# spyglass-search/memex

Hardware: AMD Instinct MI355X
Metric: queries/sec, exact cosine top-10 (recall@10 = 1.0) on 10M x 384-d f32 (higher is better)
Workload: dtype f32 corpus; int8 MFMA filter (exact integer sums, measured-residual certificate) -> f32 rescoring -> f64 DistCosine on the survivors (results bit-identical to all-f64)

## Files before the change

memex_amd/csrc/index.hip:

```cpp
#include <dlfcn.h>
#include <sys/stat.h>
#include <unistd.h>

#include <algorithm>
#include <atomic>
#include <cmath>
#include <condition_variable>
#include <cstdlib>
#include <chrono>
#include <ctime>
#include <cstring>
#include <deque>
#include <map>
#include <memory>
#include <mutex>
#include <string>
#include <thread>
#include <vector>

#include "index_kernels.h"
#include "mx_common.h"
#include "mx_debug.h"
#include "mx_filter_bits.h"
#include "shard_pool.h"

namespace mx {

std::string &last_error_slot() {
    static thread_local std::string slot;
    return slot;
}

namespace {

constexpr int kFlagWords = 4 * kMaxBatch;
constexpr int kAutoI8MaxDim = 1024;
constexpr int kSumWords = 5;

struct Scratch {
    void *qfrag = nullptr;
    float *qpad = nullptr;
    double *qnorm2 = nullptr;
    float *theta = nullptr, *theta_retry = nullptr;
    uint32_t *todo = nullptr;
    uint32_t *dev_flags = nullptr;
    uint32_t *host_flags = nullptr;
    uint32_t *host_sum = nullptr;
    bool out_on_host = false;
    uint32_t *done_ctr = nullptr;
    uint32_t flag_seq = 0;
    uint32_t *overflow = nullptr, *cand_cnt = nullptr, *qflags = nullptr;
    float *e1 = nullptr;
    float *lane_rec = nullptr;
    uint32_t *lane_tile = nullptr;
    uint32_t *lane_cnt = nullptr;
    float *lane_max = nullptr;
    float *qstage = nullptr;
    float *qscale = nullptr;
    float *qa = nullptr, *qb = nullptr;
    float *qmean = nullptr;
    uint64_t *out_ids = nullptr;
    float *out_scores = nullptr;
    float *out_dists = nullptr;
    int32_t *out_nfound = nullptr;
    int kcap = 0;
    void *exact_scratch = nullptr;
    size_t exact_bytes = 0;
    float *max_err = nullptr;
    float *h_q = nullptr;
    uint64_t *h_ids = nullptr;
    float *h_scores = nullptr, *h_dists = nullptr;
    int32_t *h_nf = nullptr;
    uint32_t *rlim = nullptr;
    uint64_t *out_nrange = nullptr;
    uint64_t *h_nr = nullptr;
    bool ready = false;
};

struct LaneBufs {
    float *rec = nullptr;
    uint32_t *tile = nullptr, *cnt = nullptr;
    float *max = nullptr;
    int nwg = 0;
    int groups = 1;
};
constexpr int kMaxDevices = 64;
struct LanePool {
    std::mutex mu;
    std::vector<LaneBufs> idle;
    int open_indexes = 0;
};
LanePool g_lanes[kMaxDevices];

void lane_free(LaneBufs &b) {
    if (b.rec) (void)hipFree(b.rec);
    if (b.tile) (void)hipFree(b.tile);
    if (b.cnt) (void)hipFree(b.cnt);
    if (b.max) (void)hipFree(b.max);
    b = LaneBufs{};
}

struct Rccl {
    void *lib = nullptr;
    int (*CommInitAll)(void **, int, const int *) = nullptr;
    int (*CommDestroy)(void *) = nullptr;
    int (*AllGather)(const void *, void *, size_t, int, void *, hipStream_t) = nullptr;
    int (*GroupStart)() = nullptr;
    int (*GroupEnd)() = nullptr;
    const char *(*GetErrorString)(int) = nullptr;
    bool ok = false;
};

}
}

using namespace mx;

struct mx_filter;

struct SearchReq {
    const float *q;
    int B, k;
    uint64_t *ids;
    float *scores, *dists;
    int32_t *n_found;
    const std::vector<std::pair<uint64_t, uint64_t>> *filt = nullptr;
    mx_filter *res = nullptr;
    const uint32_t *dlim = nullptr;
    uint64_t *n_in_range = nullptr;
    int rc = MX_OK;
    std::string err;
    bool done = false;
};

struct mx_index {
    std::string key;
    int dim = 0, ds = 0, kc = 0, device = 0;
    int refs = 1;
    std::mutex mu;
    std::mutex cmu;
    std::condition_variable ccv;
    std::deque<SearchReq *> pending;
    bool leader = false;
    hipStream_t stream = nullptr;
    float *x = nullptr;
    float *scale = nullptr;
    void *xh = nullptr;
    bool want_filter = true;
    bool filter_i8 = false;
    bool filter_auto = true;
    bool pooled = false;
    uint32_t i8_batches = 0, i8_retry_batches = 0;
    uint64_t plain_bf16_rows = 0;
    uint64_t demoted_at_rows = 0;
    float *tsc = nullptr;
    float *amean = nullptr;
    float *mean = nullptr;
    float *msum = nullptr;
    bool centred = false;
    bool compressed = false;
    bool raw_ingest = false;
    float *xs = nullptr, *ss = nullptr;
    uint64_t xs_rows = 0;
    uint64_t n = 0, cap = 0;
    IdMap idmap{0, 0, 1, 0};
    uint32_t *flags = nullptr;
    uint64_t wild_rows = 0;
    uint32_t *zero_rows = nullptr;
    uint64_t n_zero = 0;
    uint32_t *wild_list = nullptr;
    uint64_t n_wild = 0;
    int mode = MX_SEARCH_AUTO;
    bool profiling = false;
    int n_cu = 0, nwg = 0;
    bool scan8_pair = true;
    Scratch s;
    mx_index_stats stats{};
    hipEvent_t ev0 = nullptr, ev1 = nullptr, ev_wait = nullptr;
    double wait_ema_us[4] = {0.0, 0.0, 0.0, 0.0};
    uint64_t *dead = nullptr;
    std::vector<uint64_t> dead_h;
    uint64_t n_dead = 0;
    std::vector<uint64_t> dead_log;
    uint64_t disk_dead = 0;
    uint64_t gen = 0;
    bool failed = false;
    uint64_t *filt = nullptr;
    size_t filt_words = 0;
    uint64_t *filt_ranges = nullptr;
    size_t filt_ranges_cap = 0;
    uint32_t *subset_rows = nullptr;
    bool last_subset = false;
    uint64_t row_epoch = 0;
    uint64_t dead_ver = 0;
    uint32_t *mmr_rows = nullptr;
    float *mmr_stage = nullptr;
    size_t mmr_stage_bytes = 0;
    uint64_t *mmr_ids = nullptr, *mmr_h_ids = nullptr;
    float *mmr_scores = nullptr, *mmr_dists = nullptr;
    int32_t *mmr_nf = nullptr, *mmr_h_nf = nullptr;
    uint32_t *mmr_pos = nullptr;
    int mmr_fcap = 0;
    uint32_t *byid_rows = nullptr;
    float *byid_stage = nullptr;
    float *byid_q = nullptr;
    uint64_t *byid_ids = nullptr, *byid_nr = nullptr, *byid_own = nullptr;
    float *byid_scores = nullptr, *byid_dists = nullptr;
    int32_t *byid_nf = nullptr;
    uint32_t *byid_src = nullptr, *byid_dlim = nullptr;
    int byid_cap = 0;
    std::string disk_dir;
    uint64_t disk_rows = 0;
    off_t disk_size = 0;
    struct timespec disk_mtime {};
    std::vector<mx_index *> shards;
    uint64_t block_rows = 0;
    uint64_t total = 0;
    bool use_rccl = false;
    std::vector<void *> comms;
    std::vector<void *> sh_block;
    std::vector<void *> sh_gather;
    std::vector<float *> sh_q, sh_scores;
    std::vector<int32_t *> sh_nf;
    int sh_kcap = 0;
    std::unique_ptr<ShardPool> pool;
    bool composite() const { return !shards.empty(); }
};

struct FilterShard {
    int device = 0;
    uint64_t *bits = nullptr;
    size_t words = 0;
    std::vector<uint64_t> bits_h;
    uint64_t *stage = nullptr;
    size_t stage_words = 0;
    uint32_t *list = nullptr;
    bool cached = false, list_ok = false;
    uint64_t cached_dead = 0;
    uint64_t n_allowed = 0, n_live = 0;
    uint64_t row_lo = 0, row_hi = 0;
};
struct mx_filter {
    mx_index *idx = nullptr;
    uint64_t epoch = 0;
    std::vector<FilterShard> sh;
};

namespace {

std::mutex g_reg_mu;
std::map<std::string, mx_index *> g_registry;
std::once_flag g_scan_once;
hipError_t g_scan_setup_err = hipSuccess;
std::mutex g_rccl_mu;
Rccl g_rccl;
std::atomic<bool> g_rccl_broken{false};

bool load_rccl() {
    std::lock_guard<std::mutex> lk(g_rccl_mu);
    if (g_rccl.lib) return g_rccl.ok;
    for (const char *name : {"librccl.so.1", "librccl.so", "/opt/rocm/lib/librccl.so.1"}) {
        g_rccl.lib = dlopen(name, RTLD_NOW | RTLD_GLOBAL);
        if (g_rccl.lib) break;
    }
    if (!g_rccl.lib) return false;
    auto sym = [&](const char *n) { return dlsym(g_rccl.lib, n); };
    g_rccl.CommInitAll = reinterpret_cast<int (*)(void **, int, const int *)>(sym("ncclCommInitAll"));
    g_rccl.CommDestroy = reinterpret_cast<int (*)(void *)>(sym("ncclCommDestroy"));
    g_rccl.AllGather = reinterpret_cast<int (*)(const void *, void *, size_t, int, void *, hipStream_t)>(sym("ncclAllGather"));
    g_rccl.GroupStart = reinterpret_cast<int (*)()>(sym("ncclGroupStart"));
    g_rccl.GroupEnd = reinterpret_cast<int (*)()>(sym("ncclGroupEnd"));
    g_rccl.GetErrorString = reinterpret_cast<const char *(*)(int)>(sym("ncclGetErrorString"));
    g_rccl.ok = g_rccl.CommInitAll && g_rccl.CommDestroy && g_rccl.AllGather && g_rccl.GroupStart && g_rccl.GroupEnd;
    return g_rccl.ok;
}

void free_composite_buffers(mx_index *idx) {
    for (size_t g = 0; g < idx->shards.size(); ++g) {
        DeviceGuard dg(idx->shards[g]->device);
        auto F = [](void *p) {
            if (p) (void)hipFree(p);
        };
        if (g < idx->sh_block.size()) F(idx->sh_block[g]);
        if (g < idx->sh_gather.size()) F(idx->sh_gather[g]);
        if (g < idx->sh_q.size()) F(idx->sh_q[g]);
        if (g < idx->sh_scores.size()) F(idx->sh_scores[g]);
        if (g < idx->sh_nf.size()) F(idx->sh_nf[g]);
    }
    idx->sh_block.clear(); idx->sh_gather.clear(); idx->sh_q.clear(); idx->sh_scores.clear(); idx->sh_nf.clear();
    idx->sh_kcap = 0;
}

int free_index(mx_index *idx) {
    {
        std::lock_guard<std::mutex> lk(idx->mu);
    }
    if (idx->composite()) {
        idx->pool.reset();
        for (mx_index *sh : idx->shards) {
            DeviceGuard dg(sh->device);
            if (sh->stream) (void)hipStreamSynchronize(sh->stream);
        }
        free_composite_buffers(idx);
        for (void *c : idx->comms)
            if (c && g_rccl.ok) (void)g_rccl.CommDestroy(c);
        for (mx_index *sh : idx->shards) free_index(sh);
        idx->shards.clear();
    }
    DeviceGuard g(idx->device);
    if (idx->stream) (void)hipStreamSynchronize(idx->stream);
    auto F = [](void *p) {
        if (p) (void)hipFree(p);
    };
    F(idx->x); F(idx->scale); F(idx->xh); F(idx->tsc); F(idx->flags); F(idx->xs); F(idx->ss); F(idx->zero_rows); F(idx->wild_list);
    F(idx->amean); F(idx->mean); F(idx->msum); F(idx->dead); F(idx->filt); F(idx->filt_ranges); F(idx->subset_rows);
    F(idx->mmr_rows); F(idx->mmr_stage); F(idx->mmr_ids); F(idx->mmr_scores); F(idx->mmr_dists); F(idx->mmr_nf); F(idx->mmr_pos);
    if (idx->mmr_h_ids) (void)hipHostFree(idx->mmr_h_ids);
    if (idx->mmr_h_nf) (void)hipHostFree(idx->mmr_h_nf);
    F(idx->byid_rows); F(idx->byid_stage); F(idx->byid_q); F(idx->byid_ids); F(idx->byid_nr); F(idx->byid_own); F(idx->byid_scores);
    F(idx->byid_dists); F(idx->byid_nf); F(idx->byid_src); F(idx->byid_dlim);
    Scratch &s = idx->s;
    F(s.qfrag); F(s.qpad); F(s.qnorm2); F(s.theta); F(s.theta_retry); F(s.todo); F(s.dev_flags); F(s.done_ctr);
    if (s.host_flags) (void)hipHostFree(s.host_flags);
    if (s.host_sum) (void)hipHostFree(s.host_sum);
    for (void *hp : {(void *)s.h_q, (void *)s.h_ids, (void *)s.h_scores, (void *)s.h_dists, (void *)s.h_nf, (void *)s.h_nr})
        if (hp) (void)hipHostFree(hp);
    F(s.rlim); F(s.out_nrange);
    F(s.qstage); F(s.qscale); F(s.qa); F(s.qb); F(s.qmean); F(s.out_ids); F(s.out_scores); F(s.out_dists); F(s.out_nfound);
    F(s.exact_scratch); F(s.max_err);
    if (idx->ev0) (void)hipEventDestroy(idx->ev0);
    if (idx->ev1) (void)hipEventDestroy(idx->ev1);
    if (idx->ev_wait) (void)hipEventDestroy(idx->ev_wait);
    if (idx->stream) (void)hipStreamDestroy(idx->stream);
    if (idx->pooled && idx->device >= 0 && idx->device < kMaxDevices) {
        LanePool &lp = g_lanes[idx->device];
        std::lock_guard<std::mutex> lk(lp.mu);
        if (--lp.open_indexes <= 0) {
            lp.open_indexes = 0;
            for (LaneBufs &b : lp.idle) lane_free(b);
            lp.idle.clear();
        }
    }
    delete idx;
    return MX_OK;
}

struct LaneLease {
    mx_index *idx = nullptr;
    LaneBufs b;
    int take(mx_index *i, int groups) {
        if (i->device < 0 || i->device >= kMaxDevices) return fail(MX_EDEVICE, "device %d out of range", i->device);
        idx = i;
        LanePool &lp = g_lanes[i->device];
        {
            std::lock_guard<std::mutex> lk(lp.mu);
            for (size_t j = 0; j < lp.idle.size(); ++j)
                if (lp.idle[j].nwg == i->nwg && lp.idle[j].groups == groups) {
                    b = lp.idle[j];
                    lp.idle.erase(lp.idle.begin() + (long)j);
                    break;
                }
        }
        if (!b.rec) {
            b.nwg = i->nwg;
            b.groups = groups;
            const size_t lanes = (size_t)i->nwg * kScanThreads * (size_t)groups;
            hipError_t e = hipMalloc(reinterpret_cast<void **>(&b.rec), lanes * kRecCap * 16 * sizeof(float));
            if (e == hipSuccess) e = hipMalloc(reinterpret_cast<void **>(&b.tile), lanes * kRecCap * sizeof(uint32_t));
            if (e == hipSuccess) e = hipMalloc(reinterpret_cast<void **>(&b.cnt), lanes * sizeof(uint32_t));
            if (e == hipSuccess) e = hipMalloc(reinterpret_cast<void **>(&b.max), lanes * sizeof(float));
            if (e != hipSuccess) {
                lane_free(b);
                idx = nullptr;
                return fail(MX_ENOMEM, "hipMalloc(lane buffers): %s", hipGetErrorString(e));
            }
        }
        Scratch &s = i->s;
        s.lane_rec = b.rec;
        s.lane_tile = b.tile;
        s.lane_cnt = b.cnt;
        s.lane_max = b.max;
        return MX_OK;
    }
    void drop() {
        if (!idx) return;
        Scratch &s = idx->s;
        s.lane_rec = nullptr;
        s.lane_tile = nullptr;
        s.lane_cnt = nullptr;
        s.lane_max = nullptr;
        LanePool &lp = g_lanes[idx->device];
        std::lock_guard<std::mutex> lk(lp.mu);
        if (lp.open_indexes > 0) lp.idle.push_back(b);
        else lane_free(b);
        idx = nullptr;
        b = LaneBufs{};
    }
    ~LaneLease() { drop(); }
};

int ensure_scratch(mx_index *idx) {
    Scratch &s = idx->s;
    if (s.ready) return MX_OK;
    const size_t ds = (size_t)idx->ds;
    MX_HIP(hipMalloc(&s.qfrag, (size_t)kMaxBatch * ds * 2));
    MX_HIP(hipMalloc(&s.qpad, (size_t)kMaxBatch * ds * 4));
    MX_HIP(hipMalloc(&s.qnorm2, kMaxBatch * sizeof(double)));
    MX_HIP(hipMalloc(&s.theta, kMaxBatch * sizeof(float)));
    MX_HIP(hipMalloc(&s.theta_retry, kMaxBatch * sizeof(float)));
    MX_HIP(hipMalloc(&s.todo, kMaxBatch * sizeof(uint32_t)));
    MX_HIP(hipMalloc(&s.dev_flags, kFlagWords * sizeof(uint32_t)));
    MX_HIP(hipMemsetAsync(s.dev_flags, 0, kFlagWords * sizeof(uint32_t), idx->stream));
    s.overflow = s.dev_flags;
    s.cand_cnt = s.dev_flags + kMaxBatch;
    s.e1 = reinterpret_cast<float *>(s.dev_flags + 2 * kMaxBatch);
    s.qflags = s.dev_flags + 3 * kMaxBatch;
    MX_HIP(hipHostMalloc(reinterpret_cast<void **>(&s.host_flags), kFlagWords * sizeof(uint32_t), hipHostMallocDefault));
    MX_HIP(hipHostMalloc(reinterpret_cast<void **>(&s.host_sum), kSumWords * sizeof(uint32_t), hipHostMallocMapped | hipHostMallocCoherent));
    memset(s.host_sum, 0, kSumWords * sizeof(uint32_t));
    MX_HIP(hipMalloc(&s.done_ctr, sizeof(uint32_t)));
    MX_HIP(hipMemsetAsync(s.done_ctr, 0, sizeof(uint32_t), idx->stream));
    MX_HIP(hipMalloc(&s.qstage, (size_t)kMaxBatch * idx->dim * sizeof(float)));
    MX_HIP(hipMalloc(&s.qscale, kMaxBatch * sizeof(float)));
    MX_HIP(hipMalloc(&s.qa, kMaxBatch * sizeof(float)));
    MX_HIP(hipMalloc(&s.qb, kMaxBatch * sizeof(float)));
    MX_HIP(hipMalloc(&s.qmean, kMaxBatch * sizeof(float)));
    MX_HIP(hipMemsetAsync(s.qmean, 0, kMaxBatch * sizeof(float), idx->stream));
    MX_HIP(hipHostMalloc(reinterpret_cast<void **>(&s.h_q), (size_t)kMaxBatch * idx->dim * sizeof(float), hipHostMallocMapped | hipHostMallocCoherent));
    MX_HIP(hipHostMalloc(reinterpret_cast<void **>(&s.h_nf), kMaxBatch * sizeof(int32_t), hipHostMallocMapped | hipHostMallocCoherent));
    MX_HIP(hipMalloc(&s.max_err, sizeof(float)));
    MX_HIP(hipMalloc(&s.rlim, kMaxBatch * sizeof(uint32_t)));
    MX_HIP(hipMalloc(&s.out_nrange, kMaxBatch * sizeof(uint64_t)));
    MX_HIP(hipHostMalloc(reinterpret_cast<void **>(&s.h_nr), kMaxBatch * sizeof(uint64_t), hipHostMallocMapped | hipHostMallocCoherent));
    MX_HIP(hipMemsetAsync(s.max_err, 0, sizeof(float), idx->stream));
    s.ready = true;
    return MX_OK;
}

int ensure_out(mx_index *idx, int k) {
    Scratch &s = idx->s;
    if (k <= s.kcap) return MX_OK;
    auto F = [](void *p) {
        if (p) (void)hipFree(p);
    };
    F(s.out_ids); F(s.out_scores); F(s.out_dists); F(s.out_nfound);
    s.out_ids = nullptr; s.out_scores = nullptr; s.out_dists = nullptr; s.out_nfound = nullptr;
    for (void *hp : {(void *)s.h_ids, (void *)s.h_scores, (void *)s.h_dists})
        if (hp) (void)hipHostFree(hp);
    s.h_ids = nullptr; s.h_scores = nullptr; s.h_dists = nullptr;
    s.kcap = 0;
    const int kc = std::max(k, 16);
    MX_HIP(hipMalloc(&s.out_ids, (size_t)kMaxBatch * kc * sizeof(uint64_t)));
    MX_HIP(hipMalloc(&s.out_scores, (size_t)kMaxBatch * kc * sizeof(float)));
    MX_HIP(hipMalloc(&s.out_dists, (size_t)kMaxBatch * kc * sizeof(float)));
    MX_HIP(hipMalloc(&s.out_nfound, kMaxBatch * sizeof(int32_t)));
    MX_HIP(hipHostMalloc(reinterpret_cast<void **>(&s.h_ids), (size_t)kMaxBatch * kc * sizeof(uint64_t), hipHostMallocMapped | hipHostMallocCoherent));
    MX_HIP(hipHostMalloc(reinterpret_cast<void **>(&s.h_scores), (size_t)kMaxBatch * kc * sizeof(float), hipHostMallocMapped | hipHostMallocCoherent));
    MX_HIP(hipHostMalloc(reinterpret_cast<void **>(&s.h_dists), (size_t)kMaxBatch * kc * sizeof(float), hipHostMallocMapped | hipHostMallocCoherent));
    s.kcap = kc;
    return MX_OK;
}

int ensure_exact(mx_index *idx, int k, int *gcap) {
    Scratch &s = idx->s;
    for (int g = *gcap;; g /= 2) {
        const size_t need = exact_group_scratch_bytes(idx->n, k, g);
        if (s.exact_bytes >= need) {
            *gcap = g;
            return MX_OK;
        }
        if (s.exact_scratch) {
            MX_HIP(hipStreamSynchronize(idx->stream));
            (void)hipFree(s.exact_scratch);
        }
        s.exact_scratch = nullptr;
        s.exact_bytes = 0;
        const size_t want = need + need / 4;
        if (hipMalloc(&s.exact_scratch, want) == hipSuccess) {
            s.exact_bytes = want;
        } else {
            (void)hipGetLastError();
            if (hipMalloc(&s.exact_scratch, need) == hipSuccess) s.exact_bytes = need;
            else (void)hipGetLastError();
        }
        if (s.exact_bytes >= need) {
            *gcap = g;
            return MX_OK;
        }
        if (g <= 4) return fail(MX_ENOMEM, "hipMalloc(EXACT-path scratch, %zu bytes) failed", need);
    }
}

struct DevBuf {
    void *p = nullptr;
    ~DevBuf() {
        if (p) (void)hipFree(p);
    }
    void *release() {
        void *r = p;
        p = nullptr;
        return r;
    }
};

int grow_dead(mx_index *idx, uint64_t cap) {
    if (!idx->dead) return MX_OK;
    const size_t words = (size_t)(cap / kTile8Rows), have = idx->dead_h.size();
    if (words <= have) return MX_OK;
    DevBuf nd;
    MX_HIP(hipMalloc(&nd.p, words * sizeof(uint64_t)));
    MX_HIP(hipMemcpyAsync(nd.p, idx->dead, have * sizeof(uint64_t), hipMemcpyDeviceToDevice, idx->stream));
    MX_HIP(hipMemsetAsync(static_cast<uint64_t *>(nd.p) + have, 0, (words - have) * sizeof(uint64_t), idx->stream));
    MX_HIP(hipStreamSynchronize(idx->stream));
    (void)hipFree(idx->dead);
    idx->dead = static_cast<uint64_t *>(nd.release());
    idx->dead_h.resize(words, 0);
    return MX_OK;
}

int ensure_capacity(mx_index *idx, uint64_t rows) {
    if (rows <= idx->cap) return MX_OK;
    uint64_t want = std::max<uint64_t>(rows, idx->cap + idx->cap / 2);
    want = round_up(std::max<uint64_t>(want, 1024), kTile8Rows);
    if (int rc = grow_dead(idx, want); rc != MX_OK) return rc;
    if (idx->compressed) {
        DevBuf nh2;
        const size_t hb = (size_t)want * idx->ds * 2;
        MX_HIP(hipMalloc(&nh2.p, hb));
        const size_t used = idx->xh ? (size_t)round_up(idx->n, kTileRows) * idx->ds * 2 : 0;
        if (used) MX_HIP(hipMemcpyAsync(nh2.p, idx->xh, used, hipMemcpyDeviceToDevice, idx->stream));
        MX_HIP(hipMemsetAsync(static_cast<char *>(nh2.p) + used, 0, hb - used, idx->stream));
        MX_HIP(hipStreamSynchronize(idx->stream));
        if (idx->xh) (void)hipFree(idx->xh);
        idx->xh = nh2.release();
        idx->cap = want;
        return MX_OK;
    }
    DevBuf nx, nsc, nh, nts, nam;
    const size_t rowb = (size_t)idx->ds * sizeof(float);
    MX_HIP(hipMalloc(&nx.p, want * rowb));
    MX_HIP(hipMalloc(&nsc.p, want * sizeof(float)));
    float *fx = static_cast<float *>(nx.p), *fsc = static_cast<float *>(nsc.p);
    if (idx->n) {
        MX_HIP(hipMemcpyAsync(fx, idx->x, idx->n * rowb, hipMemcpyDeviceToDevice, idx->stream));
        MX_HIP(hipMemcpyAsync(fsc, idx->scale, idx->n * sizeof(float), hipMemcpyDeviceToDevice, idx->stream));
    }
    MX_HIP(hipMemsetAsync(fx + idx->n * (size_t)idx->ds, 0, (want - idx->n) * rowb, idx->stream));
    MX_HIP(hipMemsetAsync(fsc + idx->n, 0, (want - idx->n) * sizeof(float), idx->stream));
    if (idx->want_filter && idx->kc <= kMaxKC16) {
        const size_t eb = idx->filter_i8 ? 1 : 2;
        const size_t hb = (size_t)want * idx->ds * eb, tb = (size_t)(want / kTile8Rows) * kTscaleFloats * sizeof(float);
        if (hipMalloc(&nh.p, hb) != hipSuccess || (idx->filter_i8 && hipMalloc(&nts.p, tb) != hipSuccess)) {
            (void)hipGetLastError();
            if (nh.p) (void)hipFree(nh.release());
            nh.p = nullptr;
        } else {
            const uint64_t used_rows = idx->xh ? round_up(idx->n, kTile8Rows) : 0;
            const size_t used = (size_t)used_rows * idx->ds * eb;
            if (used) MX_HIP(hipMemcpyAsync(nh.p, idx->xh, used, hipMemcpyDeviceToDevice, idx->stream));
            MX_HIP(hipMemsetAsync(static_cast<char *>(nh.p) + used, 0, hb - used, idx->stream));
            if (idx->filter_i8) {
                const size_t tused = (size_t)(used_rows / kTile8Rows) * kTscaleFloats * sizeof(float);
                if (tused) MX_HIP(hipMemcpyAsync(nts.p, idx->tsc, tused, hipMemcpyDeviceToDevice, idx->stream));
                MX_HIP(hipMemsetAsync(static_cast<char *>(nts.p) + tused, 0, tb - tused, idx->stream));
                if (idx->centred && idx->xh && idx->amean) {
                    if (hipMalloc(&nam.p, want * sizeof(float)) == hipSuccess) {
                        const size_t aused = (size_t)used_rows * sizeof(float);
                        MX_HIP(hipMemcpyAsync(nam.p, idx->amean, std::min(aused, (size_t)idx->cap * sizeof(float)), hipMemcpyDeviceToDevice, idx->stream));
                        if (want * sizeof(float) > aused) MX_HIP(hipMemsetAsync(static_cast<char *>(nam.p) + aused, 0, want * sizeof(float) - aused, idx->stream));
                    } else {
                        (void)hipGetLastError();
                        if (idx->n) {
// ... 297 lines not shown
int build_filter_mask(mx_index *idx, const Ranges &r, std::vector<uint64_t> &flat) {
    const size_t words = (size_t)(idx->cap / kTile8Rows);
    if (int rc = ensure_mask_words(idx, words); rc != MX_OK) return rc;
    if (idx->filt_ranges_cap < std::max<size_t>(r.size(), 1)) {
        if (idx->filt_ranges) (void)hipFree(idx->filt_ranges);
        idx->filt_ranges = nullptr;
        idx->filt_ranges_cap = 0;
        const size_t want = std::max<size_t>(r.size() + r.size() / 2, 64);
        MX_HIP(hipMalloc(reinterpret_cast<void **>(&idx->filt_ranges), want * 2 * sizeof(uint64_t)));
        idx->filt_ranges_cap = want;
    }
    flat.resize(2 * r.size());
    for (size_t i = 0; i < r.size(); ++i) {
        flat[2 * i] = r[i].first;
        flat[2 * i + 1] = r[i].second;
    }
    if (!flat.empty())
        MX_HIP(hipMemcpyAsync(idx->filt_ranges, flat.data(), flat.size() * sizeof(uint64_t), hipMemcpyHostToDevice, idx->stream));
    MX_HIP(launch_filter_mask(idx->stream, idx->n_dead ? idx->dead : nullptr, idx->filt_ranges, (uint32_t)r.size(), words, idx->filt));
    return MX_OK;
}

bool subset_pays(const mx_index *idx, int B, uint64_t m, uint64_t span_rows, int bytes_per_elem) {
    if (m > (uint64_t)kSubsetCap || idx->ds > kMaxKC16 * kChunkFloats) return false;
    const int force = debug_flag("filt_subset", -1);
    if (force == 0 || force == 1) return force == 1;
    const double w = (double)idx->ds / 384.0;
    const double subset_us = (double)((B + kPassBatch - 1) / kPassBatch) * (43.0 + 0.053 * w * (double)m);
    const double masked_us = 75.0 + (double)span_rows * w * bytes_per_elem * (B <= 128 ? 0.065e-3 : 0.10e-3);
    return subset_us <= masked_us;
}

struct FilterArg {
    const Ranges *ranges = nullptr;
    mx_filter *res = nullptr;
    int shard = 0;
};

void refresh_filter_shard(const mx_index *t, FilterShard &fs) {
    if (fs.cached && fs.cached_dead == t->dead_ver) return;
    fs.n_allowed = fs.n_live = 0;
    fs.row_lo = fs.row_hi = 0;
    const bool dead = t->n_dead != 0;
    for (size_t w = 0; w < fs.bits_h.size(); ++w) {
        const uint64_t b = fs.bits_h[w];
        if (!b) continue;
        if (!fs.n_allowed) fs.row_lo = (uint64_t)w * 64 + (uint64_t)__builtin_ctzll(b);
        fs.row_hi = (uint64_t)w * 64 + 64 - (uint64_t)__builtin_clzll(b);
        fs.n_allowed += (uint64_t)__builtin_popcountll(b);
        fs.n_live += (uint64_t)__builtin_popcountll(dead && w < t->dead_h.size() ? b & ~t->dead_h[w] : b);
    }
    fs.cached = true;
    fs.cached_dead = t->dead_ver;
    fs.list_ok = false;
}

int ensure_mask_words(mx_index *idx, size_t words) {
    if (idx->filt_words >= words) return MX_OK;
    if (idx->filt) (void)hipFree(idx->filt);
    idx->filt = nullptr;
    idx->filt_words = 0;
    MX_HIP(hipMalloc(reinterpret_cast<void **>(&idx->filt), words * sizeof(uint64_t)));
    idx->filt_words = words;
    return MX_OK;
}

int apply_filter_mask(mx_index *idx, const FilterShard &fs) {
    const size_t words = (size_t)(idx->cap / kTile8Rows);
    if (int rc = ensure_mask_words(idx, words); rc != MX_OK) return rc;
    MX_HIP(launch_filter_apply(idx->stream, idx->n_dead ? idx->dead : nullptr, fs.bits, std::min(fs.words, words), words, idx->filt));
    return MX_OK;
}

int await_finish(mx_index *idx, int B, uint32_t seq) {
    Scratch &s = idx->s;
    static const bool no_spin = [] {
        const char *sp = getenv("MEMEX_HIP_SPIN");
        return !(sp && sp[0] == '1');
    }();
    const auto t0 = std::chrono::steady_clock::now();
    double &ema = idx->wait_ema_us[B <= 32 ? 0 : B <= 128 ? 1 : B <= 256 ? 2 : 3];
    bool overslept = false;
    if (no_spin && ema > 150.0) {
        const double nap_us = 0.8 * ema - 60.0;
        if (nap_us > 50.0) {
            struct timespec ts;
            ts.tv_sec = (time_t)(nap_us / 1e6);
            ts.tv_nsec = (long)((nap_us - (double)ts.tv_sec * 1e6) * 1e3);
            (void)clock_nanosleep(CLOCK_MONOTONIC, 0, &ts, nullptr);
            overslept = __atomic_load_n(&s.host_sum[4], __ATOMIC_ACQUIRE) == seq;
        }
    }
    bool done = false;
    for (unsigned spins = 1;; ++spins) {
        if (__atomic_load_n(&s.host_sum[4], __ATOMIC_ACQUIRE) == seq) {
            done = true;
            break;
        }
        if ((spins & 0xfff) == 0 && std::chrono::steady_clock::now() - t0 > std::chrono::seconds(2)) break;
        __builtin_ia32_pause();
    }
    if (done) {
        const double us = std::chrono::duration<double, std::micro>(std::chrono::steady_clock::now() - t0).count();
        ema = overslept ? 0.5 * ema : ema > 0.0 ? 0.75 * ema + 0.25 * us : us;
        return MX_OK;
    }
    MX_HIP(hipStreamSynchronize(idx->stream));
    if (__atomic_load_n(&s.host_sum[4], __ATOMIC_ACQUIRE) == seq) return MX_OK;
    return fail(MX_EDEVICE, "finish_kernel did not signal completion");
}

enum class BatchKind { kTopK, kRange };
struct BatchPlan {
    bool filt8;
    bool wide;
    bool fast;
    bool centred8;
    bool centred;
    bool x2;
    bool pair;
    int nwg;
    int lanes;
    Scan8Geom geom;
    int split;
    uint64_t trows;
    int bytes_per_elem;
};

BatchPlan plan_batch(const mx_index *idx, int B, int k_or_cap, BatchKind kind, bool trivial) {
    BatchPlan pl;
    pl.filt8 = idx->xh != nullptr && idx->filter_i8 && !idx->compressed;
    pl.wide = idx->kc > kMaxKC && !pl.filt8;
    pl.fast = !trivial && idx->mode == MX_SEARCH_AUTO && (idx->kc > kMaxKC ? idx->xh != nullptr && idx->kc <= kMaxKC16 : true) &&
              (!idx->compressed || idx->wild_rows == 0) && (kind == BatchKind::kRange || k_or_cap <= 256) &&
              idx->n_zero <= (uint64_t)kZeroCap && idx->n_wild <= (uint64_t)kWildCap;
    pl.centred8 = idx->centred && pl.filt8 && idx->amean && idx->mean && idx->kc <= kMaxKC;
    const bool two_groups = pl.fast && pl.filt8 && !pl.centred8 && idx->kc <= kMaxKC8x2;
    pl.x2 = two_groups && B > kPassBatch;
    pl.pair = two_groups && B > kPassBatch / 2 && B <= kPassBatch && idx->scan8_pair;
    pl.centred = pl.centred8 || (idx->centred && idx->xh && !pl.filt8 && !pl.wide && !idx->compressed && idx->amean && idx->mean && idx->kc <= kMaxKC);
    pl.nwg = pl.pair ? 2 * idx->nwg : idx->nwg;
    pl.lanes = pl.x2 || pl.pair ? 2 : 1;
    pl.geom = pl.pair ? Scan8Geom::kPair : pl.x2 ? Scan8Geom::k512 : Scan8Geom::k256;
    pl.split = B > kPassBatch && !pl.x2 && !(pl.fast && pl.wide) ? kPassBatch : pl.fast && pl.wide && B > kWideBatch ? kWideBatch : 0;
    pl.trows = pl.filt8 ? kTile8Rows : kTileRows;
    pl.bytes_per_elem = pl.filt8 ? 1 : idx->xh ? 2 : 4;
    return pl;
}

int prep_queries(mx_index *idx, const BatchPlan &pl, const float *d_q, int B) {
    Scratch &s = idx->s;
    MX_HIP(launch_prep_queries(idx->stream, d_q, B, idx->dim, idx->ds, s.qfrag, s.qpad, s.qnorm2, s.theta, s.e1,
                               idx->xh ? idx->flags + 2 : nullptr, s.overflow, s.qflags, s.qa, s.qb, pl.filt8, s.qscale,
                               pl.centred ? idx->mean : nullptr, s.qmean, pl.centred8 ? idx->flags + 5 : nullptr));
    return MX_OK;
}

void fill_scan_params(ScanParams &p, const mx_index *idx, const BatchPlan &pl, int B, const uint64_t *mask) {
    const Scratch &s = idx->s;
    p.x = idx->x;
    p.xh = idx->xh;
    p.scale = idx->scale;
    p.qfrag = s.qfrag;
    p.theta = s.theta;
    p.n_rows = idx->n;
    p.ds = (uint32_t)idx->ds;
    p.wave_mask = (1u << ((B + 31) / 32)) - 1u;
    p.lane_rec = s.lane_rec;
    p.lane_tile = s.lane_tile;
    p.lane_cnt = s.lane_cnt;
    p.lane_max = s.lane_max;
    p.overflow = s.overflow;
    p.tscale = idx->tsc;
    p.qscale = s.qscale;
    p.qa = s.qa;
    p.qb = s.qb;
    p.amean = pl.centred ? idx->amean : nullptr;
    p.qmean = s.qmean;
    p.dead = mask;
}

hipError_t launch_scan_for(const mx_index *idx, const BatchPlan &pl, bool collect, const ScanParams &p) {
    if (pl.filt8) return launch_scan8(idx->stream, idx->kc, collect, pl.nwg, p, pl.geom);
    if (pl.wide) return launch_scan16w(idx->stream, idx->kc, collect, pl.nwg, p);
    return idx->xh ? launch_scan16(idx->stream, idx->kc, collect, pl.nwg, p) : launch_scan(idx->stream, idx->kc, collect, pl.nwg, p);
}

void fill_finish_params(FinishParams &fp, const mx_index *idx, const BatchPlan &pl, int B, int k, const uint64_t *mask, uint64_t n_live,
                        uint64_t *d_ids, float *d_scores, float *d_dists, int32_t *d_nfound) {
    const Scratch &s = idx->s;
    fp.k = k;
    fp.ds = idx->ds;
    fp.nwg = pl.nwg;
    fp.x = idx->compressed ? nullptr : idx->x;
    fp.xh = idx->xh;
    fp.scale = idx->scale;
    fp.n_rows = idx->n;
    fp.idmap = idx->idmap;
    fp.qpad = s.qpad;
    fp.qnorm2 = s.qnorm2;
    fp.e1 = s.e1;
    fp.qa = s.qa;
    fp.qb = s.qb;
    fp.terr = pl.filt8 ? idx->tsc : nullptr;
    fp.e2 = (float)(idx->ds + 8) * 5.9604645e-8f + 1e-6f;
    fp.lane_rec = s.lane_rec;
    fp.lane_tile = s.lane_tile;
    fp.lane_cnt = s.lane_cnt;
    fp.theta = s.theta;
    fp.zero_rows = idx->zero_rows;
    fp.n_zero = (uint32_t)std::min<uint64_t>(idx->n_zero, kZeroCap);
    fp.wild_rows = idx->wild_list;
    fp.n_wild = (uint32_t)std::min<uint64_t>(idx->n_wild, kWildCap);
    fp.dead = mask;
    fp.n_live = n_live;
    fp.overflow = s.overflow;
    fp.todo = nullptr;
    fp.theta_retry = s.theta_retry;
    fp.cand_cnt = s.cand_cnt;
    fp.ids = d_ids;
    fp.scores = d_scores;
    fp.dists = d_dists;
    fp.n_found = d_nfound;
    fp.max_err = nullptr;
    fp.done_ctr = s.done_ctr;
    fp.dev_flags = s.dev_flags;
    fp.host_flags = s.host_sum;
    fp.n_queries = B;
    fp.host_out = s.out_on_host ? 1 : 0;
}

int fetch_flags(mx_index *idx) {
    MX_HIP(hipMemcpyAsync(idx->s.host_flags, idx->s.dev_flags, kFlagWords * sizeof(uint32_t), hipMemcpyDeviceToHost, idx->stream));
    MX_HIP(hipStreamSynchronize(idx->stream));
    return MX_OK;
}

void drop_large_exact_scratch(mx_index *idx) {
    if (idx->mode != MX_SEARCH_AUTO || idx->s.exact_bytes <= kExactKeepBytes) return;
    (void)hipFree(idx->s.exact_scratch);
    idx->s.exact_scratch = nullptr;
    idx->s.exact_bytes = 0;
}

int search_batch(mx_index *idx, const float *d_q, int B, int k, uint64_t *d_ids, float *d_scores, float *d_dists,
                 int32_t *d_nfound, const FilterArg *filt = nullptr) {
    int rc = ensure_scratch(idx);
    if (rc != MX_OK) return rc;
    Scratch &s = idx->s;
    hipStream_t st = idx->stream;
    Ranges fr;
    uint64_t n_allow = 0, span_lo = 0, span_hi = 0;
    FilterShard *res = filt && filt->res ? &filt->res->sh[(size_t)filt->shard] : nullptr;
    if (res) {
        refresh_filter_shard(idx, *res);
        n_allow = res->n_live;
        span_lo = res->row_lo;
        span_hi = res->row_hi;
    } else if (filt) {
        for (const auto &x : *filt->ranges)
            if (x.first < std::min(x.second, idx->n)) fr.emplace_back(x.first, std::min(x.second, idx->n));
        n_allow = count_allowed(idx, fr);
        if (!fr.empty()) {
            span_lo = fr.front().first;
            span_hi = fr.back().second;
        }
    }
    idx->last_subset = false;
    const bool trivial = idx->n == 0 || k == 0 || (filt && n_allow == 0);
    if (idx->compressed && idx->kc > kMaxKC16 && !trivial)
        return fail(MX_EUNSUPPORTED, "a compressed corpus supports dim <= %d", kMaxKC16 * kChunkFloats);
    const BatchPlan pl = plan_batch(idx, B, k, BatchKind::kTopK, trivial);
    if (pl.split) {
        rc = search_batch(idx, d_q, pl.split, k, d_ids, d_scores, d_dists, d_nfound, filt);
        if (rc != MX_OK) return rc;
        const size_t o = (size_t)pl.split * k;
        return search_batch(idx, d_q + (size_t)pl.split * idx->dim, B - pl.split, k, d_ids + o, d_scores + o,
                            d_dists ? d_dists + o : nullptr, d_nfound + pl.split, filt);
    }
    const uint32_t *h_ovf = s.host_flags, *h_qfl = s.host_flags + 3 * kMaxBatch;
    auto any_bad_query = [&] {
        uint32_t bad = 0;
        for (int b = 0; b < B; ++b) bad |= h_qfl[b];
        return bad != 0;
    };
    if (filt && !trivial && subset_pays(idx, B, n_allow, span_hi - span_lo, pl.bytes_per_elem)) {
        std::vector<uint32_t> list;
        const uint32_t *rows_list = nullptr;
        if (res) {
            if (!res->list) MX_HIP(hipMalloc(reinterpret_cast<void **>(&res->list), (size_t)kSubsetCap * sizeof(uint32_t)));
            if (!res->list_ok) {
                MX_HIP(hipMemsetAsync(res->list, 0, (size_t)kSubsetCap * sizeof(uint32_t), st));
                MX_HIP(launch_filter_list(st, idx->n_dead ? idx->dead : nullptr, res->bits, span_lo >> 6, (span_hi + 63) >> 6, res->list,
                                          (uint32_t)kSubsetCap));
                res->list_ok = true;
            }
            rows_list = res->list;
        } else {
            list.reserve((size_t)n_allow);
            for (const auto &x : fr)
                for (uint64_t r = x.first; r < x.second; ++r)
                    if (!idx->n_dead || !((idx->dead_h[r >> 6] >> (r & 63)) & 1ull)) list.push_back((uint32_t)r);
            if (!idx->subset_rows) MX_HIP(hipMalloc(reinterpret_cast<void **>(&idx->subset_rows), (size_t)kSubsetCap * sizeof(uint32_t)));
            MX_HIP(hipMemcpyAsync(idx->subset_rows, list.data(), list.size() * sizeof(uint32_t), hipMemcpyHostToDevice, st));
            rows_list = idx->subset_rows;
        }
        if ((rc = prep_queries(idx, pl, d_q, B)) != MX_OK) return rc;
        MX_HIP(launch_subset_topk(st, B, k, idx->ds, idx->compressed ? nullptr : idx->x, idx->xh, rows_list, (uint32_t)n_allow,
                                  idx->idmap, s.qpad, s.qnorm2, d_ids, d_scores, d_dists, d_nfound));
        if ((rc = fetch_flags(idx)) != MX_OK) return rc;
        if (any_bad_query()) return fail(MX_EINVAL, "a query contains non-finite values");
        idx->last_subset = true;
        idx->stats.searches += 1;
        idx->stats.queries += (uint64_t)B;
        idx->stats.filtered_queries += (uint64_t)B;
        idx->stats.subset_queries += (uint64_t)B;
        return MX_OK;
    }
    std::vector<uint64_t> flat_ranges;
    if (filt && !trivial && (rc = res ? apply_filter_mask(idx, *res) : build_filter_mask(idx, fr, flat_ranges)) != MX_OK) return rc;
    const uint64_t *mask = filt ? idx->filt : idx->n_dead ? idx->dead : nullptr;
    const uint64_t n_live = filt ? n_allow : idx->n - idx->n_dead;
    LaneLease lease;
    if ((rc = lease.take(idx, pl.lanes)) != MX_OK) return rc;
    if ((rc = prep_queries(idx, pl, d_q, B)) != MX_OK) return rc;
    bool timed = false;

    FinishParams fp;
    fill_finish_params(fp, idx, pl, B, k, mask, n_live, d_ids, d_scores, d_dists, d_nfound);
    if (trivial) fp.n_rows = fp.n_live = 0;
    fp.max_err = idx->profiling ? s.max_err : nullptr;
    auto finish_and_wait = [&]() -> int {
        fp.seq = ++s.flag_seq;
        MX_HIP(launch_finish(st, B, fp));
        return await_finish(idx, B, fp.seq);
    };
    std::vector<int> exact;
    if (trivial) {
        fp.seq = ++s.flag_seq;
        MX_HIP(launch_finish(st, B, fp));
    } else if (pl.fast) {
        const uint64_t tiles = (idx->n + pl.trows - 1) / pl.trows, full = idx->n / pl.trows;
        const uint64_t ts0 = filt ? span_lo / pl.trows : 0, ts1 = filt ? (span_hi + pl.trows - 1) / pl.trows : tiles;
        const uint64_t full1 = std::min(ts1, full);
        ScanParams p;
        fill_scan_params(p, idx, pl, B, mask);
        auto collect = [&](bool first) -> int {
            p.tile_begin = (uint32_t)ts0;
            p.tile_end = (uint32_t)ts1;
            p.tile_stride = 1;
            if (first && idx->profiling) MX_HIP(hipEventRecord(idx->ev0, st));
            MX_HIP(launch_scan_for(idx, pl, true, p));
            if (first && idx->profiling) {
                MX_HIP(hipEventRecord(idx->ev1, st));
                timed = true;
            }
            if (first) {
                idx->stats.scan_launches += 1;
                idx->stats.scan_bytes += (ts1 - ts0) * pl.trows * idx->ds * (uint64_t)pl.bytes_per_elem;
            }
            return MX_OK;
        };
        if (ts1 - ts0 > 2ull * idx->nwg) {
            p.tile_begin = (uint32_t)ts0;
            p.tile_end = (uint32_t)full1;
            p.tile_stride = sample_stride(full1 - ts0, pl.nwg, k, pl.filt8, idx->ds, pl.centred8);
            MX_HIP(launch_scan_for(idx, pl, false, p));
            MX_HIP(launch_theta(st, B, k, pl.nwg, s.lane_max, s.qa, !pl.filt8, s.theta));
        }
        if ((rc = collect(true)) != MX_OK) return rc;
        if ((rc = finish_and_wait()) != MX_OK) return rc;
        if (timed) {
            float ms = 0.f;
            MX_HIP(hipEventElapsedTime(&ms, idx->ev0, idx->ev1));
            idx->stats.scan_ms += ms;
            timed = false;
        }
        if (s.host_sum[2]) return fail(MX_EINVAL, "a query contains non-finite values");
        idx->stats.candidates += s.host_sum[1];
        if (s.host_sum[0]) {
            if ((rc = fetch_flags(idx)) != MX_OK) return rc;
            int retry = 0;
            for (int b = 0; b < B; ++b) {
                if (h_ovf[b] == 1) ++retry;
                else if (h_ovf[b] >= 2) exact.push_back(b);
            }
            if (pl.filt8 && !filt) idx->i8_retry_batches += 1;
            const bool habitual = pl.filt8 && idx->i8_batches >= 8 && idx->i8_retry_batches * 4 > idx->i8_batches;
            if (pl.filt8 && !filt && idx->filter_auto && ((size_t)(retry + (int)exact.size()) * 16 > (size_t)std::max(B, 16) || habitual)) {
                if (!idx->centred && idx->kc <= kMaxKC && idx->n >= 256) {
                    const std::string keep = last_error_slot();
                    if (build_filter_copy(idx, true) == MX_OK && idx->centred) {
                        lease.drop();
                        return search_batch(idx, d_q, B, k, d_ids, d_scores, d_dists, d_nfound);
                    }
                    last_error_slot() = keep;
                }
                const int drc = demote_filter(idx);
                if (drc == MX_OK) {
                    idx->stats.filter_demotions += 1;
                    lease.drop();
                    return search_batch(idx, d_q, B, k, d_ids, d_scores, d_dists, d_nfound);
                }
                if (drc != MX_ENOMEM) return drc;
            }
            if (retry) {
                idx->stats.retry_queries += (uint64_t)retry;
                p.wave_mask = 0;
                for (int b = 0; b < B; ++b)
                    if (h_ovf[b] == 1) p.wave_mask |= 1u << (b >> 5);
                MX_HIP(launch_retry_setup(st, s.theta, s.theta_retry, s.overflow, s.todo));
                if ((rc = collect(false)) != MX_OK) return rc;
                fp.todo = s.todo;
                if ((rc = finish_and_wait()) != MX_OK) return rc;
                exact.clear();
                if (s.host_sum[0]) {
                    if ((rc = fetch_flags(idx)) != MX_OK) return rc;
                    for (int b = 0; b < B; ++b)
                        if (h_ovf[b] != 0) exact.push_back(b);
                }
            }
        }
        idx->stats.fallback_queries += exact.size();
    } else {
        if ((rc = fetch_flags(idx)) != MX_OK) return rc;
        if (any_bad_query()) return fail(MX_EINVAL, "a query contains non-finite values");
        for (int b = 0; b < B; ++b) exact.push_back(b);
    }
    if (!exact.empty() || trivial || !pl.fast) {
        rc = run_exact(idx, exact, k, d_ids, d_scores, d_dists, d_nfound, mask, n_live);
        if (rc != MX_OK) return rc;
        MX_HIP(hipStreamSynchronize(st));
        drop_large_exact_scratch(idx);
    }
    idx->stats.searches += 1;
    idx->stats.queries += (uint64_t)B;
    if (filt) idx->stats.filtered_queries += (uint64_t)B;
    if (pl.filt8 && pl.fast && !filt) idx->i8_batches += 1;
    return MX_OK;
}

float host_score_from_dist(float d) {
    const volatile float t = 1.0f / d;
    const volatile float u = 1.0f / t;
    return 1.0f - u;
}

uint32_t range_dist_limit(float t) {
    if (!(t <= 1.0f)) return 0;
    uint32_t lo = 0, hi = 0x40800000u;
    if (host_score_from_dist(4.0f) >= t) return hi + 1;
    while (hi - lo > 1) {
        const uint32_t mid = lo + (hi - lo) / 2;
        float d;
        memcpy(&d, &mid, sizeof d);
        if (host_score_from_dist(d) >= t) lo = mid;
        else hi = mid;
    }
    return lo + 1;
}

constexpr float kRangeEps = 9.5367431640625e-7f;

int run_exact_range(mx_index *idx, const std::vector<int> &qs, int cap, uint64_t *d_ids, float *d_scores, float *d_dists,
                    int32_t *d_nfound, uint64_t *d_nrange, const uint64_t *mask, uint64_t n_live) {
    if (qs.empty()) return MX_OK;
    int gcap = qs.size() <= 4 ? 4 : qs.size() <= 8 ? 8 : qs.size() <= 16 ? 16 : kExactGroup;
    int rc = ensure_exact(idx, cap, &gcap);
    if (rc != MX_OK) return rc;
    Scratch &s = idx->s;
    for (size_t g0 = 0; g0 < qs.size(); g0 += (size_t)gcap) {
        ExactGroup grp{};
        grp.n = (int)std::min<size_t>((size_t)gcap, qs.size() - g0);
        for (int j = 0; j < grp.n; ++j) grp.q[j] = qs[g0 + j];
        MX_HIP(launch_exact_range_group(idx->stream, cap, idx->ds, idx->compressed ? nullptr : idx->x, idx->xh, idx->n, idx->idmap, s.qpad,
                                        s.qnorm2, grp, s.exact_scratch, s.rlim, d_ids, d_scores, d_dists, d_nfound, d_nrange, mask, n_live));
    }
    return MX_OK;
}

int range_batch(mx_index *idx, const float *d_q, int B, int cap, const uint32_t *dlim, uint64_t *d_ids, float *d_scores, float *d_dists,
                int32_t *d_nfound, uint64_t *d_nrange) {
    int rc = ensure_scratch(idx);
    if (rc != MX_OK) return rc;
    Scratch &s = idx->s;
    hipStream_t st = idx->stream;
    const uint64_t n_live = idx->n - idx->n_dead;
    const bool trivial = idx->n == 0 || n_live == 0;
    if (idx->compressed && idx->kc > kMaxKC16 && !trivial)
        return fail(MX_EUNSUPPORTED, "a compressed corpus supports dim <= %d", kMaxKC16 * kChunkFloats);
    const BatchPlan pl = plan_batch(idx, B, cap, BatchKind::kRange, trivial);
    if (pl.split) {
        rc = range_batch(idx, d_q, pl.split, cap, dlim, d_ids, d_scores, d_dists, d_nfound, d_nrange);
        if (rc != MX_OK) return rc;
        const size_t o = (size_t)pl.split * cap;
        return range_batch(idx, d_q + (size_t)pl.split * idx->dim, B - pl.split, cap, dlim + pl.split, d_ids + o, d_scores + o,
                           d_dists ? d_dists + o : nullptr, d_nfound + pl.split, d_nrange + pl.split);
    }
    const uint32_t *h_ovf = s.host_flags, *h_qfl = s.host_flags + 3 * kMaxBatch;
    const uint64_t *mask = idx->n_dead ? idx->dead : nullptr;
    LaneLease lease;
    if (pl.fast && (rc = lease.take(idx, pl.lanes)) != MX_OK) return rc;
    MX_HIP(hipMemcpyAsync(s.rlim, dlim, (size_t)B * sizeof(uint32_t), hipMemcpyHostToDevice, st));
    if ((rc = prep_queries(idx, pl, d_q, B)) != MX_OK) return rc;
    std::vector<int> exact;
    if (pl.fast) {
        MX_HIP(launch_range_theta(st, B, s.rlim, kRangeEps, s.qa, s.theta));
        const uint64_t tiles = (idx->n + pl.trows - 1) / pl.trows;
        ScanParams p;
        fill_scan_params(p, idx, pl, B, mask);
        p.tile_begin = 0;
        p.tile_end = (uint32_t)tiles;
        p.tile_stride = 1;
        MX_HIP(launch_scan_for(idx, pl, true, p));
        idx->stats.scan_launches += 1;
        idx->stats.scan_bytes += tiles * pl.trows * idx->ds * (uint64_t)pl.bytes_per_elem;

        RangeParams rp;
        FinishParams &fp = rp.f;
        fill_finish_params(fp, idx, pl, B, cap, mask, n_live, d_ids, d_scores, d_dists, d_nfound);
        fp.seq = ++s.flag_seq;
        rp.dlim = s.rlim;
        rp.eps = kRangeEps;
        rp.n_in_range = d_nrange;
        MX_HIP(launch_range_finish(st, B, rp));
        if ((rc = await_finish(idx, B, fp.seq)) != MX_OK) return rc;
        if (s.host_sum[2]) return fail(MX_EINVAL, "a query contains non-finite values");
        idx->stats.candidates += s.host_sum[1];
        if (s.host_sum[0]) {
            if ((rc = fetch_flags(idx)) != MX_OK) return rc;
            for (int b = 0; b < B; ++b)
                if (h_ovf[b] != 0) exact.push_back(b);
        }
        idx->stats.fallback_queries += exact.size();
    } else {
        if ((rc = fetch_flags(idx)) != MX_OK) return rc;
        for (int b = 0; b < B; ++b)
            if (h_qfl[b]) return fail(MX_EINVAL, "a query contains non-finite values");
        for (int b = 0; b < B && !trivial; ++b) exact.push_back(b);
        if (trivial) {
            MX_HIP(hipMemsetAsync(s.rlim, 0, (size_t)B * sizeof(uint32_t), st));
            RangeParams rp{};
            rp.f.k = cap;
            rp.f.ds = idx->ds;
            rp.f.x = idx->x;
            rp.f.ids = d_ids;
            rp.f.scores = d_scores;
            rp.f.dists = d_dists;
            rp.f.n_found = d_nfound;
            rp.f.cand_cnt = s.cand_cnt;
            rp.dlim = s.rlim;
            rp.n_in_range = d_nrange;
            MX_HIP(launch_range_finish(st, B, rp));
        }
    }
    if (!exact.empty() || trivial) {
        rc = run_exact_range(idx, exact, cap, d_ids, d_scores, d_dists, d_nfound, d_nrange, mask, n_live);
        if (rc != MX_OK) return rc;
        MX_HIP(hipStreamSynchronize(st));
        drop_large_exact_scratch(idx);
    }
    idx->stats.searches += 1;
    idx->stats.queries += (uint64_t)B;
    return MX_OK;
}

void sync_shard_streams(mx_index *idx) {
    for (mx_index *sh : idx->shards) {
        DeviceGuard dg(sh->device);
        if (sh->stream) (void)hipStreamSynchronize(sh->stream);
    }
}

bool sync_shard_streams_within(mx_index *idx, double seconds) {
    const auto t_end = std::chrono::steady_clock::now() + std::chrono::duration<double>(seconds);
    for (mx_index *sh : idx->shards) {
        DeviceGuard dg(sh->device);
        if (!sh->stream) continue;
        for (;;) {
            const hipError_t e = hipStreamQuery(sh->stream);
            if (e == hipSuccess) break;
            if (e != hipErrorNotReady) {
                (void)hipGetLastError();
                return false;
            }
            if (std::chrono::steady_clock::now() > t_end) return false;
            std::this_thread::sleep_for(std::chrono::microseconds(200));
        }
    }
    return true;
}

int ensure_composite_buffers(mx_index *idx, int k) {
    if (k <= idx->sh_kcap) return MX_OK;
    sync_shard_streams(idx);
    free_composite_buffers(idx);
    const int kc = std::max(k, 16);
    const size_t G = idx->shards.size();
    const size_t blk = (size_t)kMaxBatch * kc * 12 + kMaxBatch * sizeof(uint64_t);
    idx->sh_block.assign(G, nullptr); idx->sh_gather.assign(G, nullptr); idx->sh_q.assign(G, nullptr);
    idx->sh_scores.assign(G, nullptr); idx->sh_nf.assign(G, nullptr);
    for (size_t g = 0; g < G; ++g) {
        DeviceGuard dg(idx->shards[g]->device);
        MX_HIP(hipMalloc(&idx->sh_block[g], blk));
        if (g == 0 || idx->use_rccl) MX_HIP(hipMalloc(&idx->sh_gather[g], blk * G));
        MX_HIP(hipMalloc(reinterpret_cast<void **>(&idx->sh_q[g]), (size_t)kMaxBatch * idx->dim * sizeof(float)));
        MX_HIP(hipMalloc(reinterpret_cast<void **>(&idx->sh_scores[g]), (size_t)kMaxBatch * kc * sizeof(float)));
        MX_HIP(hipMalloc(reinterpret_cast<void **>(&idx->sh_nf[g]), kMaxBatch * sizeof(int32_t)));
    }
    idx->sh_kcap = kc;
    return MX_OK;
}

uint64_t shard_rows(uint64_t total, uint64_t R, uint64_t G, uint64_t g) {
    const uint64_t full_blocks = total / R, tail = total % R;
    uint64_t rows = (full_blocks / G) * R + (g < full_blocks % G ? R : 0);
    if (full_blocks % G == g) rows += tail;
    return rows;
}

void enable_peer_access(mx_index *idx) {
    for (size_t g = 1; g < idx->shards.size(); ++g) {
        if (idx->shards[g]->device == idx->shards[0]->device) continue;
        int can = 0;
        (void)hipDeviceCanAccessPeer(&can, idx->shards[0]->device, idx->shards[g]->device);
        if (can) {
            DeviceGuard dg(idx->shards[0]->device);
            (void)hipDeviceEnablePeerAccess(idx->shards[g]->device, 0);
            (void)hipGetLastError();
            DeviceGuard d2(idx->shards[g]->device);
            (void)hipDeviceEnablePeerAccess(idx->shards[0]->device, 0);
            (void)hipGetLastError();
        }
    }
}

bool rccl_selftest(mx_index *idx, double seconds) {
    const int G = (int)idx->shards.size();
    std::vector<hipStream_t> st(G, nullptr);
    std::vector<unsigned char *> snd(G, nullptr), rcv(G, nullptr);
    bool ok = true;
    for (int g = 0; g < G && ok; ++g) {
        DeviceGuard dg(idx->shards[g]->device);
        ok = hipStreamCreateWithFlags(&st[g], hipStreamNonBlocking) == hipSuccess && hipMalloc(&snd[g], 64) == hipSuccess &&
             hipMalloc(&rcv[g], 64 * (size_t)G) == hipSuccess && hipMemsetAsync(snd[g], g + 1, 64, st[g]) == hipSuccess &&
             hipMemsetAsync(rcv[g], 0, 64 * (size_t)G, st[g]) == hipSuccess;
    }
    bool hung = false;
    if (ok) {
        int e = g_rccl.GroupStart();
        for (int g = 0; g < G && e == 0; ++g) e = g_rccl.AllGather(snd[g], rcv[g], 64, 1 , idx->comms[g], st[g]);
        const int e2 = g_rccl.GroupEnd();
        ok = e == 0 && e2 == 0;
        const auto t0 = std::chrono::steady_clock::now();
        for (int g = 0; g < G && ok && !hung; ++g) {
            DeviceGuard dg(idx->shards[g]->device);
            for (;;) {
                const hipError_t q = hipStreamQuery(st[g]);
                if (q == hipSuccess) break;
                if (q != hipErrorNotReady) {
                    ok = false;
                    break;
                }
                if (std::chrono::duration<double>(std::chrono::steady_clock::now() - t0).count() > seconds) {
                    hung = true;
                    break;
                }
                struct timespec ts = {0, 200 * 1000};
                (void)clock_nanosleep(CLOCK_MONOTONIC, 0, &ts, nullptr);
            }
        }
        if (ok && !hung) {
            std::vector<unsigned char> h(64 * (size_t)G);
            DeviceGuard dg(idx->shards[0]->device);
            ok = hipMemcpy(h.data(), rcv[0], h.size(), hipMemcpyDeviceToHost) == hipSuccess;
            for (int g = 0; g < G && ok; ++g) ok = h[64 * (size_t)g] == (unsigned char)(g + 1) && h[64 * (size_t)g + 63] == (unsigned char)(g + 1);
        }
// ... 707 lines not shown
            rc = fail(MX_EIO, "%s: entry %zu names row %llu of a store of %llu rows", path.c_str(), i, (unsigned long long)(*rows)[i],
                      (unsigned long long)n_rows);
    if (rc != MX_OK) rows->clear();
    return rc;
}

int save_dead_file(mx_index *idx, const char *dir, bool in_sync) {
    const std::string path = dead_file(dir);
    const uint64_t total = idx->dead_log.size();
    struct stat sb;
    const bool exists = stat(path.c_str(), &sb) == 0;
    if (total == 0) {
        if (exists && unlink(path.c_str()) != 0) return fail(MX_EIO, "cannot remove %s", path.c_str());
        idx->disk_dead = 0;
        return MX_OK;
    }
    const long hb = dead_header_bytes(idx->gen);
    if (in_sync && exists && idx->disk_dead <= total && (uint64_t)sb.st_size == (uint64_t)hb + 8 * idx->disk_dead) {
        if (idx->disk_dead == total) return MX_OK;
        FILE *f = fopen(path.c_str(), "r+b");
        if (!f) return fail(MX_EIO, "cannot open %s for appending", path.c_str());
        const size_t m = (size_t)(total - idx->disk_dead);
        int rc = fseek(f, hb + (long)(8 * idx->disk_dead), SEEK_SET) == 0 &&
                         fwrite(idx->dead_log.data() + idx->disk_dead, sizeof(uint64_t), m, f) == m
                     ? MX_OK : fail(MX_EIO, "write to %s failed", path.c_str());
        if (rc == MX_OK && (fflush(f) != 0 || fseek(f, 8, SEEK_SET) != 0 || fwrite(&total, sizeof(total), 1, f) != 1))
            rc = fail(MX_EIO, "write to %s failed", path.c_str());
        if (fclose(f) != 0 && rc == MX_OK) rc = fail(MX_EIO, "write to %s failed", path.c_str());
        if (rc == MX_OK) idx->disk_dead = total;
        return rc;
    }
    const std::string tmp = path + ".tmp";
    FILE *f = fopen(tmp.c_str(), "wb");
    if (!f) return fail(MX_EIO, "cannot open %s for writing", tmp.c_str());
    int rc = fwrite(idx->gen ? kDeadMagic2 : kDeadMagic, 1, 8, f) == 8 && fwrite(&total, sizeof(total), 1, f) == 1 &&
                     (!idx->gen || fwrite(&idx->gen, sizeof(idx->gen), 1, f) == 1) &&
                     fwrite(idx->dead_log.data(), sizeof(uint64_t), (size_t)total, f) == (size_t)total
                 ? MX_OK : fail(MX_EIO, "write to %s failed", tmp.c_str());
    if (fclose(f) != 0 && rc == MX_OK) rc = fail(MX_EIO, "write to %s failed", tmp.c_str());
    if (rc == MX_OK && rename(tmp.c_str(), path.c_str()) != 0) rc = fail(MX_EIO, "cannot rename %s", tmp.c_str());
    if (rc != MX_OK) {
        unlink(tmp.c_str());
        return rc;
    }
    idx->disk_dead = total;
    return MX_OK;
}

int clear_locked(mx_index *idx) {
    if (idx->composite()) {
        for (mx_index *sh : idx->shards) {
            std::lock_guard<std::mutex> lk(sh->mu);
            clear_locked(sh);
        }
        idx->total = 0;
    } else {
        idx->n = 0;
        idx->centred = false;
        idx->plain_bf16_rows = 0;
        idx->wild_rows = 0;
        idx->n_zero = 0;
        idx->n_wild = 0;
        if (idx->dead) {
            DeviceGuard dg(idx->device);
            (void)hipMemsetAsync(idx->dead, 0, idx->dead_h.size() * sizeof(uint64_t), idx->stream);
            std::fill(idx->dead_h.begin(), idx->dead_h.end(), 0);
        }
        for (double &w : idx->wait_ema_us) w = 0.0;
        if (idx->flags) {
            DeviceGuard dg(idx->device);
            (void)hipMemsetAsync(idx->flags + 2, 0, 4 * sizeof(uint32_t), idx->stream);
        }
    }
    idx->n_dead = 0;
    idx->dead_ver += 1;
    idx->row_epoch += 1;
    idx->dead_log.clear();
    idx->disk_dead = 0;
    idx->disk_dir.clear();
    idx->failed = false;
    return MX_OK;
}

int add_host_locked(mx_index *idx, const float *rows, uint64_t n, uint64_t *first_id) {
    if (idx->composite()) return composite_add(idx, rows, n, first_id, false);
    DeviceGuard g(idx->device);
    if (n == 0) return add_device_locked(idx, nullptr, 0, first_id);
    const size_t total = (size_t)n * idx->dim;
    for (size_t i = 0; i < total; ++i)
        if (!std::isfinite(rows[i])) return fail(MX_EINVAL, "row %zu contains a non-finite value; nothing inserted", i / idx->dim);
    const uint64_t chunk_rows = std::max<uint64_t>(1, (64ull << 20) / ((uint64_t)idx->dim * 4));
    float *stage = nullptr;
    MX_HIP(hipMalloc(&stage, (size_t)std::min(chunk_rows, n) * idx->dim * sizeof(float)));
    int rc = MX_OK;
    uint64_t first = 0;
    const RowMark mark = mark_rows(idx);
    for (uint64_t done = 0; done < n && rc == MX_OK; done += chunk_rows) {
        const uint64_t m = std::min(chunk_rows, n - done);
        hipError_t e = hipMemcpyAsync(stage, rows + (size_t)done * idx->dim, (size_t)m * idx->dim * sizeof(float),
                                      hipMemcpyHostToDevice, idx->stream);
        if (e != hipSuccess) {
            rc = fail(MX_EDEVICE, "hipMemcpy H2D: %s", hipGetErrorString(e));
            break;
        }
        uint64_t f = 0;
        rc = add_device_locked(idx, stage, m, &f);
        if (done == 0) first = f;
    }
    (void)hipFree(stage);
    if (rc != MX_OK) rollback_rows(idx, mark);
    if (rc == MX_OK && first_id) *first_id = first;
    return rc;
}

int open_plain(const std::string &k, int dim, int device, mx_index **out) {
    int ndev = 0;
    hipError_t e = hipGetDeviceCount(&ndev);
    if (e != hipSuccess || ndev <= 0)
        return fail(MX_EDEVICE, "no HIP device available (%s)", e == hipSuccess ? "count 0" : hipGetErrorString(e));
    if (device < 0 || device >= ndev) return fail(MX_EDEVICE, "device %d out of range (have %d)", device, ndev);
    if (device >= kMaxDevices) return fail(MX_EUNSUPPORTED, "device %d: at most %d devices per process", device, kMaxDevices);
    DeviceGuard g(device);
    if (!g.ok) return fail(MX_EDEVICE, "hipSetDevice(%d) failed", device);
    std::call_once(g_scan_once, [] {
        g_scan_setup_err = scan_setup();
        if (g_scan_setup_err == hipSuccess) g_scan_setup_err = scan16_setup();
        if (g_scan_setup_err == hipSuccess) g_scan_setup_err = scan16w_setup();
        if (g_scan_setup_err == hipSuccess) g_scan_setup_err = scan8_setup();
        if (g_scan_setup_err == hipSuccess) g_scan_setup_err = finish_setup();
        if (g_scan_setup_err == hipSuccess) g_scan_setup_err = subset_setup();
        if (g_scan_setup_err == hipSuccess) g_scan_setup_err = range_setup();
    });
    if (g_scan_setup_err != hipSuccess)
        return fail(MX_EDEVICE, "scan kernel setup failed: %s (is this a gfx950 device?)", hipGetErrorString(g_scan_setup_err));
    std::unique_ptr<mx_index> idx(new mx_index());
    idx->key = k;
    idx->dim = dim;
    idx->ds = (int)round_up((uint64_t)dim, dim > kMaxKC * kChunkFloats ? 2 * kChunkFloats : kChunkFloats);
    idx->kc = idx->ds / kChunkFloats;
    {
        const char *fk = getenv("MEMEX_HIP_FILTER");
        idx->filter_auto = !(fk && fk[0]);
        idx->filter_i8 = idx->filter_auto ? idx->ds <= kAutoI8MaxDim : (fk[0] == 'i' || fk[0] == '8');
    }
    idx->device = device;
    hipDeviceProp_t prop;
    MX_HIP(hipGetDeviceProperties(&prop, device));
    idx->n_cu = prop.multiProcessorCount;
    idx->nwg = std::max(1, std::min(idx->n_cu, kMaxScanCUs));
    {
        const char *pv = getenv("MEMEX_HIP_SCAN8_PAIR");
        idx->scan8_pair = !(pv && pv[0] == '0');
    }
    MX_HIP(hipStreamCreateWithFlags(&idx->stream, hipStreamNonBlocking));
    MX_HIP(hipEventCreate(&idx->ev0));
    MX_HIP(hipEventCreate(&idx->ev1));
    MX_HIP(hipEventCreateWithFlags(&idx->ev_wait, hipEventDisableTiming));
    MX_HIP(hipMalloc(&idx->flags, 6 * sizeof(uint32_t)));
    MX_HIP(hipMemset(idx->flags, 0, 6 * sizeof(uint32_t)));
    MX_HIP(hipMalloc(&idx->zero_rows, kZeroCap * sizeof(uint32_t)));
    MX_HIP(hipMalloc(&idx->wild_list, kWildCap * sizeof(uint32_t)));
    if (device < kMaxDevices) {
        std::lock_guard<std::mutex> lk(g_lanes[device].mu);
        g_lanes[device].open_indexes += 1;
        idx->pooled = true;
    }
    *out = idx.release();
    return MX_OK;
}

bool row_removed(const mx_index *t, uint64_t r) {
    return t->dead && (r >> 6) < t->dead_h.size() && ((t->dead_h[r >> 6] >> (r & 63)) & 1ull);
}
bool global_removed(const mx_index *idx, uint64_t r) {
    if (!idx->composite()) return row_removed(idx, r);
    const uint64_t R = idx->block_rows, G = idx->shards.size(), b = r / R;
    return row_removed(idx->shards[b % G], (b / G) * R + r % R);
}

int release_capacity(mx_index *idx) {
    const uint64_t want = round_up(std::max<uint64_t>(idx->n, 1024), kTile8Rows);
    if (want >= idx->cap) return MX_OK;
    const size_t ds = (size_t)idx->ds;
    const size_t eb = idx->compressed ? 2 : idx->filter_i8 ? 1 : 2;
    DevBuf nx, nsc, nh, nts, nam;
    auto get = [](DevBuf &b, size_t bytes) {
        if (hipMalloc(&b.p, bytes) == hipSuccess) return true;
        (void)hipGetLastError();
        b.p = nullptr;
        return false;
    };
    bool ok = idx->compressed || (get(nx, want * ds * 4) && get(nsc, want * sizeof(float)));
    if (ok && idx->xh) ok = get(nh, want * ds * eb);
    if (ok && idx->tsc) ok = get(nts, (want / kTile8Rows) * kTscaleFloats * sizeof(float));
    if (ok && idx->amean) ok = get(nam, want * sizeof(float));
    if (!ok) return MX_OK;
    const uint64_t used = round_up(idx->n, kTile8Rows);
    hipStream_t st = idx->stream;
    auto move = [&](DevBuf &b, const void *old, size_t used_bytes, size_t all_bytes) -> hipError_t {
        hipError_t e = used_bytes ? hipMemcpyAsync(b.p, old, used_bytes, hipMemcpyDeviceToDevice, st) : hipSuccess;
        if (e == hipSuccess && all_bytes > used_bytes) e = hipMemsetAsync(static_cast<char *>(b.p) + used_bytes, 0, all_bytes - used_bytes, st);
        return e;
    };
    if (!idx->compressed) {
        MX_HIP(move(nx, idx->x, used * ds * 4, want * ds * 4));
        MX_HIP(move(nsc, idx->scale, used * sizeof(float), want * sizeof(float)));
    }
    if (nh.p) MX_HIP(move(nh, idx->xh, used * ds * eb, want * ds * eb));
    if (nts.p) MX_HIP(move(nts, idx->tsc, (used / kTile8Rows) * kTscaleFloats * sizeof(float), (want / kTile8Rows) * kTscaleFloats * sizeof(float)));
    if (nam.p) MX_HIP(move(nam, idx->amean, used * sizeof(float), want * sizeof(float)));
    MX_HIP(hipStreamSynchronize(st));
    auto swap = [](auto *&dst, DevBuf &b) {
        if (!b.p) return;
        if (dst) (void)hipFree(dst);
        dst = static_cast<std::remove_reference_t<decltype(dst)>>(b.release());
    };
    swap(idx->x, nx);
    swap(idx->scale, nsc);
    if (nh.p) {
        (void)hipFree(idx->xh);
        idx->xh = nh.release();
    }
    swap(idx->tsc, nts);
    swap(idx->amean, nam);
    idx->cap = want;
    return MX_OK;
}

int compact_plain(mx_index *idx, bool *moved) {
    *moved = false;
    DeviceGuard dg(idx->device);
    hipStream_t st = idx->stream;
    const uint64_t n = idx->n, tiles = (n + kTile8Rows - 1) / kTile8Rows, ds = (uint64_t)idx->ds;
    if (!idx->dead || idx->dead_h.size() < tiles) return fail(MX_EDEVICE, "removal mask smaller than the index");
    std::vector<uint64_t> hp((size_t)tiles + 1, 0);
    uint64_t t_first = tiles;
    for (uint64_t t = 0; t < tiles; ++t) {
        const uint64_t r0 = t * kTile8Rows;
        const uint64_t valid = n - r0 >= (uint64_t)kTile8Rows ? ~0ull : (1ull << (n - r0)) - 1ull;
        const uint64_t live = ~idx->dead_h[t] & valid;
        if (live != valid && t_first == tiles) t_first = t;
        hp[t + 1] = hp[t] + (uint64_t)__builtin_popcountll(live);
    }
    const uint64_t n_live = hp[tiles];
    if (n_live != n - idx->n_dead) return fail(MX_EDEVICE, "removal bookkeeping out of step (%llu live rows counted, %llu expected)",
                                               (unsigned long long)n_live, (unsigned long long)(n - idx->n_dead));
    if (idx->compressed) t_first = 0;
    const uint32_t nb = compact_count_blocks(tiles);
    DevBuf tb, bo, stage, wa, wb;
    MX_HIP(hipMalloc(&tb.p, std::max<uint64_t>(tiles, 1) * sizeof(uint32_t)));
    MX_HIP(hipMalloc(&bo.p, ((size_t)nb + 1) * sizeof(uint32_t)));
    uint32_t *tile_base = static_cast<uint32_t *>(tb.p), *blk_off = static_cast<uint32_t *>(bo.p);
    const uint64_t stage_tiles = std::max<uint64_t>(1, (64ull << 20) / (kTile8Rows * ds * 4));
    constexpr uint64_t kWinTiles = 16384 / kTile8Rows;
    if (idx->compressed) {
        MX_HIP(hipMalloc(&wa.p, (size_t)kWinTiles * kTile8Rows * idx->dim * sizeof(float)));
        MX_HIP(hipMalloc(&wb.p, (size_t)kWinTiles * kTile8Rows * idx->dim * sizeof(float)));
        if (!idx->xs) {
            MX_HIP(hipMalloc(reinterpret_cast<void **>(&idx->xs), (size_t)(65536 + kTileRows) * idx->ds * sizeof(float)));
            MX_HIP(hipMalloc(reinterpret_cast<void **>(&idx->ss), (size_t)(65536 + kTileRows) * sizeof(float)));
            idx->xs_rows = 65536 + kTileRows;
        }
    } else {
        MX_HIP(hipMalloc(&stage.p, (size_t)stage_tiles * kTile8Rows * (ds + 1) * sizeof(float)));
    }
    MX_HIP(launch_compact_prefix(st, idx->dead, n, tile_base, blk_off));
    uint32_t dev_live = 0;
    MX_HIP(hipMemcpyAsync(&dev_live, blk_off + nb, sizeof(dev_live), hipMemcpyDeviceToHost, st));
    MX_HIP(hipStreamSynchronize(st));
    if (dev_live != n_live) return fail(MX_EDEVICE, "device removal mask out of step (%u live rows, %llu expected)", dev_live,
                                        (unsigned long long)n_live);

    *moved = true;
    if (!idx->compressed) {
        float *sx = static_cast<float *>(stage.p), *ss = sx + stage_tiles * kTile8Rows * ds;
        for (uint64_t t = t_first; t < tiles;) {
            const uint64_t lag = t * kTile8Rows - hp[t];
            uint64_t c;
            if (lag >= stage_tiles * kTile8Rows) {
                c = std::min(tiles - t, lag / kTile8Rows);
                MX_HIP(launch_compact_gather(st, idx->dead, n, t, c, tile_base, blk_off, idx->x + t * kTile8Rows * ds, idx->scale + t * kTile8Rows,
                                             (int)ds, 0, idx->x, idx->scale));
            } else {
                c = std::min(tiles - t, stage_tiles);
                MX_HIP(launch_compact_gather(st, idx->dead, n, t, c, tile_base, blk_off, idx->x + t * kTile8Rows * ds, idx->scale + t * kTile8Rows,
                                             (int)ds, hp[t], sx, ss));
                const uint64_t m = hp[t + c] - hp[t];
                if (m) {
                    MX_HIP(hipMemcpyAsync(idx->x + hp[t] * ds, sx, m * ds * sizeof(float), hipMemcpyDeviceToDevice, st));
                    MX_HIP(hipMemcpyAsync(idx->scale + hp[t], ss, m * sizeof(float), hipMemcpyDeviceToDevice, st));
                }
            }
            t += c;
        }
        const uint64_t z1 = std::min<uint64_t>(round_up(n, kTile8Rows), idx->cap);
        MX_HIP(hipMemsetAsync(idx->x + n_live * ds, 0, (z1 - n_live) * ds * sizeof(float), st));
        MX_HIP(hipMemsetAsync(idx->scale + n_live, 0, (z1 - n_live) * sizeof(float), st));
        MX_HIP(hipMemsetAsync(idx->flags, 0, 2 * sizeof(uint32_t), st));
        MX_HIP(hipMemsetAsync(idx->flags + 3, 0, 2 * sizeof(uint32_t), st));
        MX_HIP(launch_relist(st, idx->x, idx->scale, n_live, idx->ds, idx->flags, idx->zero_rows, idx->wild_list));
        idx->n = n_live;
        idx->n_zero = 0;
        idx->n_wild = 0;
        uint32_t fl[5] = {0, 0, 0, 0, 0};
        if (int rc = commit_ingest(idx, fl); rc != MX_OK) return rc;
        if (idx->xh) {
            MX_HIP(hipMemsetAsync(idx->flags + 2, 0, sizeof(uint32_t), st));
            MX_HIP(hipMemsetAsync(idx->flags + 5, 0, sizeof(uint32_t), st));
            const bool ctr = idx->centred && idx->amean && idx->mean && idx->msum;
            if (ctr && n_live) MX_HIP(launch_mean_dir(st, idx->x, idx->scale, n_live, idx->ds, idx->msum, idx->mean));
            const uint32_t t1 = (uint32_t)((n_live + kTileRows - 1) / kTileRows);
            if (n_live) {
                if (idx->filter_i8)
                    MX_HIP(launch_shadow8(st, idx->x, idx->scale, idx->ds, 0, (uint32_t)round_up(t1, 2), n_live, idx->xh, idx->tsc, idx->flags + 2,
                                          ctr ? idx->mean : nullptr, ctr ? idx->amean : nullptr, ctr ? idx->flags + 5 : nullptr));
                else
                    MX_HIP(launch_shadow(st, idx->x, idx->scale, idx->ds, 0, t1, idx->xh, idx->flags + 2, 0, 0, ~0ull, ctr ? idx->mean : nullptr,
                                         ctr ? idx->amean : nullptr));
            }
        }
    } else {
        float *wa_f = static_cast<float *>(wa.p), *wb_f = static_cast<float *>(wb.p);
        MX_HIP(hipMemsetAsync(idx->flags + 2, 0, 3 * sizeof(uint32_t), st));
        idx->n = 0;
        idx->n_zero = 0;
        idx->n_wild = 0;
        idx->wild_rows = 0;
        idx->raw_ingest = true;
        int rc = MX_OK;
        for (uint64_t t = 0; t < tiles && rc == MX_OK; t += kWinTiles) {
            const uint64_t c = std::min(kWinTiles, tiles - t), r0 = t * kTile8Rows, rows = std::min(c * kTile8Rows, n - r0);
            hipError_t e = launch_unshadow(st, idx->xh, idx->ds, idx->dim, r0, rows, wa_f);
            if (e == hipSuccess) e = launch_compact_gather(st, idx->dead, n, t, c, tile_base, blk_off, wa_f, nullptr, idx->dim, hp[t], wb_f, nullptr);
            if (e != hipSuccess) rc = fail(MX_EDEVICE, "compaction of the bf16 rows: %s", hipGetErrorString(e));
            else rc = add_device_locked(idx, wb_f, hp[t + c] - hp[t], nullptr);
        }
        idx->raw_ingest = false;
        if (rc != MX_OK) return rc;
        const uint64_t z1 = round_up(n_live, kTileRows);
        if (z1 > n_live) {
            MX_HIP(hipMemsetAsync(idx->xs, 0, (size_t)kTileRows * ds * sizeof(float), st));
            MX_HIP(hipMemsetAsync(idx->ss, 0, (size_t)kTileRows * sizeof(float), st));
            const uint32_t tl = (uint32_t)(n_live / kTileRows);
            MX_HIP(launch_shadow(st, idx->xs, idx->ss, idx->ds, tl, tl + 1, idx->xh, idx->flags + 2, tl, n_live, z1));
        }
    }
    MX_HIP(hipStreamSynchronize(st));
    (void)hipFree(idx->dead);
    idx->dead = nullptr;
    idx->dead_h.clear();
    idx->dead_h.shrink_to_fit();
    idx->n_dead = 0;
    auto rescale = [&](uint64_t &v) {
        if (v) v = std::max<uint64_t>(1, (uint64_t)((double)v * (double)n_live / (double)std::max<uint64_t>(n, 1)));
    };
    rescale(idx->demoted_at_rows);
    rescale(idx->plain_bf16_rows);
    return release_capacity(idx);
}

int compact_composite(mx_index *idx) {
    const uint64_t R = idx->block_rows, G = idx->shards.size(), total = idx->total;
    std::unique_ptr<mx_index> fresh(new mx_index());
    fresh->dim = idx->dim;
    fresh->block_rows = R;
    auto drop_fresh = [&] {
        for (mx_index *sh : fresh->shards) free_index(sh);
        fresh->shards.clear();
    };
    for (uint64_t g = 0; g < G; ++g) {
        mx_index *old = idx->shards[g], *sh = nullptr;
        int rc = open_plain("", idx->dim, old->device, &sh);
        if (rc != MX_OK) {
            drop_fresh();
            return rc;
        }
        sh->idmap = old->idmap;
        sh->mode = old->mode;
        sh->profiling = old->profiling;
        sh->scan8_pair = old->scan8_pair;
        sh->want_filter = old->want_filter;
        sh->filter_i8 = old->filter_i8;
        sh->filter_auto = old->filter_auto;
        sh->compressed = old->compressed;
        sh->raw_ingest = old->compressed;
        fresh->shards.push_back(sh);
    }
    const uint64_t chunk = std::max<uint64_t>(kTile8Rows, (32ull << 20) / ((uint64_t)idx->dim * 4));
    std::vector<float> buf((size_t)std::min<uint64_t>(chunk, std::max<uint64_t>(total, 1)) * idx->dim), tmpv;
    int rc = MX_OK;
    for (uint64_t r0 = 0; r0 < total && rc == MX_OK; r0 += chunk) {
        const uint64_t m = std::min(chunk, total - r0);
        rc = fetch_rows(idx, r0, m, buf.data(), tmpv);
        uint64_t k = 0;
        for (uint64_t i = 0; i < m && rc == MX_OK; ++i) {
            if (global_removed(idx, r0 + i)) continue;
            if (k != i) memmove(buf.data() + k * idx->dim, buf.data() + i * idx->dim, (size_t)idx->dim * sizeof(float));
            ++k;
        }
        if (rc == MX_OK && k) rc = composite_add(fresh.get(), buf.data(), k, nullptr, false);
    }
    for (mx_index *sh : fresh->shards) sh->raw_ingest = false;
    if (rc != MX_OK) {
        drop_fresh();
        return rc;
    }
    std::swap(idx->shards, fresh->shards);
    drop_fresh();
    idx->total = fresh->total;
    idx->n_dead = 0;
    return MX_OK;
}

int usable(mx_index *idx) {
    if (!idx->failed) return MX_OK;
    return fail(MX_EDEVICE, "this index is unusable: a compaction failed after rows had moved (mx_index_clear or mx_index_load resets it)");
}

}

extern "C" {

const char *mx_last_error(void) { return last_error_slot().c_str(); }
const char *mx_version(void) { return "memex-hip 0.6.0 (gfx950)"; }
size_t mx_index_stats_size(void) { return sizeof(mx_index_stats); }

int mx_device_count(int *n) try {
    if (!n) return fail(MX_EINVAL, "null argument");
    int c = 0;
    hipError_t e = hipGetDeviceCount(&c);
    if (e != hipSuccess) {
        *n = 0;
        return fail(MX_EDEVICE, "hipGetDeviceCount: %s", hipGetErrorString(e));
    }
    *n = c;
    return MX_OK;
} catch (...) {
    return guard_exception();
}

int mx_index_open(const char *key, int dim, int device, mx_index **out) try {
    if (!out) return fail(MX_EINVAL, "out is null");
    *out = nullptr;
    if (dim < 1 || dim > (1 << 16)) return fail(MX_EINVAL, "dim %d out of range", dim);
    const std::string k = key ? key : "";
    std::lock_guard<std::mutex> lk(g_reg_mu);
    if (!k.empty()) {
        auto it = g_registry.find(k);
        if (it != g_registry.end()) {
            mx_index *idx = it->second;
            if (idx->dim != dim) return fail(MX_EINVAL, "index '%s' is open with dim %d, not %d", k.c_str(), idx->dim, dim);
            if (!idx->composite() && idx->device != device)
                return fail(MX_EINVAL, "index '%s' lives on device %d, not %d", k.c_str(), idx->device, device);
            idx->refs += 1;
            *out = idx;
            return MX_OK;
        }
    }
    mx_index *raw = nullptr;
    int rc = open_plain(k, dim, device, &raw);
    if (rc != MX_OK) return rc;
    if (!k.empty()) g_registry[k] = raw;
    *out = raw;
    return MX_OK;
} catch (...) {
    return guard_exception();
}

int mx_index_open_sharded(const char *key, int dim, int n_dev, const int *devices, uint64_t block_rows, mx_index **out) try {
    if (!out) return fail(MX_EINVAL, "out is null");
    *out = nullptr;
    if (dim < 1 || dim > (1 << 16)) return fail(MX_EINVAL, "dim %d out of range", dim);
    if (n_dev < 1 || n_dev > 64) return fail(MX_EINVAL, "n_dev %d out of range", n_dev);
    const std::string k = key ? key : "";
    std::lock_guard<std::mutex> lk(g_reg_mu);
    if (!k.empty()) {
        auto it = g_registry.find(k);
        if (it != g_registry.end()) {
            mx_index *idx = it->second;
            if (idx->dim != dim) return fail(MX_EINVAL, "index '%s' is open with dim %d, not %d", k.c_str(), idx->dim, dim);
            if ((int)idx->shards.size() != n_dev) return fail(MX_EINVAL, "index '%s' is open with %zu shards, not %d", k.c_str(), idx->shards.size(), n_dev);
            idx->refs += 1;
            *out = idx;
            return MX_OK;
        }
    }
    std::unique_ptr<mx_index> idx(new mx_index());
    idx->key = k;
    idx->dim = dim;
    idx->block_rows = round_up(block_rows ? block_rows : 65536, kTileRows);
    bool distinct = n_dev > 1;
    for (int g = 0; g < n_dev; ++g) {
        const int dev = devices ? devices[g] : g;
        mx_index *sh = nullptr;
        int rc = open_plain("", dim, dev, &sh);
        if (rc != MX_OK) {
            for (mx_index *s2 : idx->shards) free_index(s2);
            return rc;
        }
        sh->idmap = IdMap{0, (uint32_t)idx->block_rows, (uint32_t)n_dev, (uint32_t)g};
        idx->shards.push_back(sh);
        for (int h = 0; h < g; ++h) distinct = distinct && idx->shards[h]->device != dev;
    }
    idx->device = idx->shards[0]->device;
    const char *ex = getenv("MEMEX_HIP_EXCHANGE");
    const bool want_rccl = ex ? strcmp(ex, "rccl") == 0 : distinct;
    const bool forbid_rccl = ex && strcmp(ex, "p2p") == 0;
    if (want_rccl && !forbid_rccl && (distinct || n_dev == 1)) {
        std::string why;
        if (g_rccl_broken) {
            why = "an earlier RCCL initialisation of this process hung";
        } else if (!load_rccl()) {
            why = "librccl.so.1 cannot be loaded";
        } else {
            struct Init {
                std::mutex mu;
                std::condition_variable cv;
                bool done = false;
                int rc = -1;
                std::vector<void *> comms;
                std::vector<int> devs;
            };
            auto init = std::make_shared<Init>();
            for (mx_index *sh : idx->shards) init->devs.push_back(sh->device);
            init->comms.assign(n_dev, nullptr);
            std::thread([init, n_dev] {
                const int rc = g_rccl.CommInitAll(init->comms.data(), n_dev, init->devs.data());
                std::lock_guard<std::mutex> l2(init->mu);
                init->rc = rc;
                init->done = true;
                init->cv.notify_all();
            }).detach();
            const char *tv = getenv("MEMEX_HIP_RCCL_TIMEOUT");
// ... 1410 lines not shown
```

memex_amd/csrc/index_kernels.h:

```cpp
#pragma once
#include <hip/hip_runtime.h>

#include <cstdint>

namespace mx {

constexpr int kScanThreads = 512;
constexpr int kScanWaves = 8;
constexpr int kTileRows = 32;
constexpr int kChunkFloats = 128;
constexpr int kSlotBytes = kTileRows * kChunkFloats * 4;
constexpr int kNumSlots = 8;
constexpr int kPrefetch = 8;
constexpr int kScaleRing = 16;
constexpr int kScanLdsBytes = kNumSlots * kSlotBytes + 2 * kTileRows * (kChunkFloats * 2 + 16) + kScaleRing * kTileRows * 4;
constexpr int kMaxKC = 6;

constexpr int kSlot16Bytes = kTileRows * kChunkFloats * 2;
constexpr int kRing16 = 16;
constexpr int kMeanRing16 = 32;
constexpr int kScan16LdsBytes = kRing16 * kSlot16Bytes + kMeanRing16 * 256 + 1024;
constexpr int kMaxKC16 = 12;
constexpr int kWideBatch = 128;
constexpr int kScan16WideLdsBytes = kRing16 * kSlot16Bytes + 4 * 64 * 16 * 4;

constexpr int kPassBatch = 256;
constexpr int kMaxBatch = 512;
constexpr int kMaxKC8x2 = 4;
constexpr int kRecCap = 64;
constexpr int kMaxScanCUs = 256;
constexpr int kMaxScanWGs = 2 * kMaxScanCUs;
constexpr int kCandCap = 16384;
constexpr int kZeroCap = 1024;
constexpr int kWildCap = 64;

constexpr float kApproxErr = 0.0081f;
constexpr float kAccSlack = 2.7e-4f;

struct Cand {
    float score;
    uint32_t row;
};

struct IdMap {
    uint64_t id_offset;
    uint32_t block_rows, n_shards, shard;
    __host__ __device__ uint64_t id_of(uint32_t row) const {
        const uint64_t r = block_rows ? ((uint64_t)(row / block_rows) * n_shards + shard) * block_rows + row % block_rows
                                      : (uint64_t)row;
        return id_offset + r + 1;
    }
};

struct ScanParams {
    const float *x;
    const void *xh;
    const float *scale;
    const void *qfrag;
    const float *theta;
    uint64_t n_rows;
    uint32_t tile_begin;
    uint32_t tile_end;
    uint32_t tile_stride;
    uint32_t ds;
    uint32_t wave_mask = 0xff;
    float *lane_rec;
    uint32_t *lane_tile;
    uint32_t *lane_cnt;
    float *lane_max;
    uint32_t *overflow;
    const float *tscale = nullptr;
    const float *qscale = nullptr;
    const float *qa = nullptr, *qb = nullptr;
    const float *amean = nullptr;
    const float *qmean = nullptr;
    const uint64_t *dead = nullptr;
};

__device__ __forceinline__ uint32_t lane_dead16(uint32_t half, uint32_t h) {
    const uint32_t w = half >> (4u * h);
    return (w & 0xfu) | ((w >> 4) & 0xf0u) | ((w >> 8) & 0xf00u) | ((w >> 12) & 0xf000u);
}
__device__ __forceinline__ uint32_t dead_half(const uint64_t *dead, uint32_t t) { return (uint32_t)(dead[t >> 1] >> (32u * (t & 1u))); }

hipError_t scan_setup();
hipError_t scan16_setup();
hipError_t launch_scan(hipStream_t s, int kc, bool collect, int nwg, const ScanParams &p);
hipError_t launch_scan16(hipStream_t s, int kc, bool collect, int nwg, const ScanParams &p);
constexpr int kTile8Rows = 64;
constexpr int kTscaleFloats = 8;
constexpr float kMinStep8 = 1.0f / 32768.0f;
constexpr int kScaleRing8 = 32;
constexpr int kScale8Entry = 512;
constexpr int kScan8LdsBytes = kRing16 * kSlot16Bytes + kScaleRing8 * kScale8Entry + 256;
constexpr int kScan8PairWaves = 4;
constexpr int kScan8PairRing = 8;
constexpr int kScan8PairScaleRing = 16;
constexpr int kScan8PairEntry = 256;
constexpr int kScan8PairLdsBytes = kScan8PairRing * kSlot16Bytes + kScan8PairScaleRing * kScan8PairEntry;
static_assert(2 * kScan8PairLdsBytes <= 160 * 1024, "two workgroups of the pair form must fit one CU's LDS");
enum class Scan8Geom {
    k256,
    k512,
    kPair,
};
hipError_t scan8_setup();
hipError_t launch_scan8(hipStream_t s, int kc, bool collect, int nwg, const ScanParams &p, Scan8Geom geom = Scan8Geom::k256);
hipError_t launch_shadow8(hipStream_t s, const float *x, const float *scale, int ds, uint32_t half0, uint32_t half1,
                          uint64_t row_hi, void *x8, float *tscale, uint32_t *ec_max, const float *mean = nullptr,
                          float *amean = nullptr, uint32_t *rc_max = nullptr);
hipError_t scan16w_setup();
hipError_t launch_scan16w(hipStream_t s, int kc, bool collect, int nwg, const ScanParams &p);

hipError_t launch_shadow(hipStream_t s, const float *x, const float *scale, int ds, uint32_t tile0, uint32_t tile1,
                         void *xh, uint32_t *ec_max, uint32_t src_tile0 = 0, uint64_t row_lo = 0, uint64_t row_hi = ~0ull,
                         const float *mean = nullptr, float *amean = nullptr);
hipError_t launch_mean_dir(hipStream_t s, const float *x, const float *scale, uint64_t n, int ds, float *msum, float *mean);
hipError_t launch_unshadow(hipStream_t s, const void *xh, int ds, int d, uint64_t row0, uint64_t n, float *out);

hipError_t launch_ingest(hipStream_t s, const float *src, uint64_t n, int d, float *x, float *scale,
                         uint64_t first, int ds, uint32_t *flags, int raw, uint32_t *zero_rows, uint32_t *wild_rows, uint64_t row_base);

hipError_t launch_prep_queries(hipStream_t s, const float *q, int B, int d, int ds, void *qfrag,
                               float *qpad, double *qnorm2, float *theta, float *e1, const uint32_t *ec_max,
                               uint32_t *overflow, uint32_t *flags, float *qa, float *qb, bool filt8 = false,
                               float *qscale = nullptr, const float *mean = nullptr, float *qmean = nullptr,
                               const uint32_t *rc_max = nullptr);

hipError_t launch_theta(hipStream_t s, int B, int k, int nwg, const float *lane_max, const float *qa, bool raw, float *theta);

struct FinishParams {
    int k, ds, nwg;
    const float *x;
    const void *xh;
    const float *scale;
    uint64_t n_rows;
    IdMap idmap;
    const float *qpad;
    const double *qnorm2;
    const float *e1;
    const float *qa, *qb;
    const float *terr;
    float e2;
    const float *lane_rec;
    const uint32_t *lane_tile;
    const uint32_t *lane_cnt;
    const float *theta;
    const uint32_t *zero_rows;
    uint32_t n_zero;
    const uint32_t *wild_rows;
    uint32_t n_wild;
    const uint64_t *dead;
    uint64_t n_live;
    uint32_t *overflow;
    const uint32_t *todo;
    float *theta_retry;
    uint32_t *cand_cnt;
    uint64_t *ids;
    float *scores, *dists;
    int32_t *n_found;
    float *max_err;
    uint32_t *done_ctr;
    const uint32_t *dev_flags;
    uint32_t *host_flags;
    int n_queries;
    int host_out;
    uint32_t seq;
};
hipError_t finish_setup();
hipError_t launch_finish(hipStream_t s, int B, const FinishParams &p);
hipError_t launch_retry_setup(hipStream_t s, float *theta, const float *theta_retry, uint32_t *overflow, uint32_t *todo);

hipError_t launch_range_theta(hipStream_t s, int B, const uint32_t *dlim, float eps, const float *qa, float *theta);
struct RangeParams {
    FinishParams f;
    const uint32_t *dlim;
    float eps;
    uint64_t *n_in_range;
};
hipError_t range_setup();
hipError_t launch_range_finish(hipStream_t s, int B, const RangeParams &rp);

constexpr int kExactGroup = 32;
constexpr int kExactSlices = 256;
struct ExactGroup {
    int n;
    int q[kExactGroup];
};
size_t exact_group_scratch_bytes(uint64_t n_rows, int k, int gcap);
hipError_t launch_exact_group(hipStream_t s, int k, int ds, const float *x, const void *xh, uint64_t n_rows, const IdMap &idmap,
                              const float *qpad, const double *qnorm2, const ExactGroup &grp, void *scratch, uint64_t *ids,
                              float *scores, float *dists, int32_t *n_found, const uint64_t *dead = nullptr, uint64_t n_live = ~0ull);

constexpr int kCompactTilesPerBlock = 1024;
uint32_t compact_count_blocks(uint64_t tiles);
hipError_t launch_compact_prefix(hipStream_t s, const uint64_t *dead, uint64_t n, uint32_t *tile_base, uint32_t *blk_off);
hipError_t launch_compact_gather(hipStream_t s, const uint64_t *dead, uint64_t n, uint64_t tile0, uint64_t tiles, const uint32_t *tile_base,
                                 const uint32_t *blk_off, const float *src, const float *src_scale, int W, uint64_t dst0, float *dst,
                                 float *dst_scale);
hipError_t launch_relist(hipStream_t s, const float *x, const float *scale, uint64_t n, int ds, uint32_t *flags, uint32_t *zero_rows,
                         uint32_t *wild_rows);

hipError_t launch_filter_mask(hipStream_t s, const uint64_t *dead, const uint64_t *ranges, uint32_t n_ranges, uint64_t words,
                              uint64_t *mask);
constexpr int kSubsetCap = 16384;
hipError_t subset_setup();
hipError_t launch_subset_topk(hipStream_t s, int B, int k, int ds, const float *x, const void *xh, const uint32_t *rows, uint32_t m,
                              const IdMap &idmap, const float *qpad, const double *qnorm2, uint64_t *ids, float *scores, float *dists,
                              int32_t *n_found);

hipError_t launch_filter_range_edit(hipStream_t s, const uint64_t *ranges, uint32_t n_ranges, uint64_t w0, uint64_t w1, bool allow,
                                    uint64_t *bits);
hipError_t launch_filter_id_edit(hipStream_t s, const uint64_t *ids, uint64_t n_ids, uint64_t total, const IdMap &idmap, bool allow,
                                 uint64_t *bits, uint64_t bit_words);
hipError_t launch_filter_apply(hipStream_t s, const uint64_t *dead, const uint64_t *bits, uint64_t bit_words, uint64_t words,
                               uint64_t *mask);
hipError_t launch_filter_list(hipStream_t s, const uint64_t *dead, const uint64_t *bits, uint64_t w0, uint64_t w1, uint32_t *rows,
                              uint32_t cap);

hipError_t launch_fill_nfound(hipStream_t s, int32_t *nf, int B, int32_t v);
hipError_t launch_exact_range_group(hipStream_t s, int cap, int ds, const float *x, const void *xh, uint64_t n_rows, const IdMap &idmap,
                                    const float *qpad, const double *qnorm2, const ExactGroup &grp, void *scratch, const uint32_t *dlim,
                                    uint64_t *ids, float *scores, float *dists, int32_t *n_found, uint64_t *n_in_range,
                                    const uint64_t *dead = nullptr, uint64_t n_live = ~0ull);
hipError_t launch_range_sum(hipStream_t s, const void *counts, size_t stride, int G, int B, int cap, uint64_t *n_in_range, int32_t *n_found);
hipError_t launch_merge(hipStream_t s, const void *ids, size_t ids_stride, const void *dists, size_t dists_stride,
                        int G, int B, int k, uint64_t *out_ids, float *out_dists, float *out_scores);

constexpr int kMmrMaxFetch = 1024;
constexpr int kMmrMaxDs = 8192;
constexpr size_t kMmrStageBytes = 64u << 20;
hipError_t launch_mmr_gather(hipStream_t s, int ds, const float *x, const void *xh, const uint32_t *rows, uint32_t n, float *stage);
hipError_t launch_mmr_select(hipStream_t s, int B, int k, int fetch, int ds, float lambda, const float *stage, const uint32_t *pos,
                             const uint64_t *cand_ids, const float *cand_scores, const float *cand_dists, const int32_t *cand_nf,
                             uint64_t *ids, float *scores, float *dists, int32_t *n_found);

constexpr uint32_t kByIdNone = 0xffffffffu;
hipError_t launch_byid_gather(hipStream_t s, int dim, int ds, const float *x, const void *xh, const uint32_t *rows, uint32_t n, float *q);
struct ByIdDrop {
    int B, k, kk, exclude, dim;
    const uint32_t *src;
    const uint64_t *own;
    const uint64_t *in_ids;
    const float *in_scores, *in_dists;
    const int32_t *in_nfound;
    const uint64_t *in_nrange;
    const uint32_t *dlim;
    const float *q;
    uint64_t *ids;
    float *scores, *dists;
    int32_t *n_found;
    uint64_t *n_in_range;
};
hipError_t launch_byid_drop_self(hipStream_t s, const ByIdDrop &p);

}
```

memex_amd/csrc/index_kernels.hip:

```cpp
#include <cmath>

#include "index_kernels.h"
#include "mx_rotate.h"

namespace mx {

typedef __attribute__((ext_vector_type(4))) float f32x4;

__device__ __forceinline__ uint32_t f32_key(float f) {
    const uint32_t u = __float_as_uint(f);
    return (u & 0x80000000u) ? ~u : (u | 0x80000000u);
}
__device__ __forceinline__ float key_f32(uint32_t k) {
    const uint32_t u = (k & 0x80000000u) ? (k & 0x7fffffffu) : ~k;
    return __uint_as_float(u);
}
__device__ __forceinline__ float score_from_dist(float d) {
    const float t = __fdiv_rn(1.0f, d);
    const float u = __fdiv_rn(1.0f, t);
    return __fsub_rn(1.0f, u);
}
__device__ __forceinline__ float dist_from_sums(double dot, double na, double nb) {
    if (na > 0.0 && nb > 0.0) {
        double d = __dsub_rn(1.0, __ddiv_rn(dot, __dsqrt_rn(__dmul_rn(na, nb))));
        if (d < 0.0) d = 0.0;
        return (float)d;
    }
    return 0.0f;
}

__device__ __forceinline__ uint32_t block_sum_256(uint32_t v, uint32_t *lds4) {
#pragma unroll
    for (int o = 32; o > 0; o >>= 1) v += __shfl_xor(v, o);
    __syncthreads();
    if ((threadIdx.x & 63) == 0) lds4[threadIdx.x >> 6] = v;
    __syncthreads();
    return lds4[0] + lds4[1] + lds4[2] + lds4[3];
}


template <int PER>
__device__ __forceinline__ uint32_t block_kth_largest(const uint32_t (&key)[PER], const bool (&valid)[PER], uint32_t k,
                                                      uint32_t *hist, uint32_t *s_pick) {
    const int tid = threadIdx.x;
    uint32_t kmax = 0, kmin = 0xffffffffu;
#pragma unroll
    for (int e = 0; e < PER; ++e)
        if (valid[e]) {
            kmax = key[e] > kmax ? key[e] : kmax;
            kmin = key[e] < kmin ? key[e] : kmin;
        }
#pragma unroll
    for (int o = 32; o > 0; o >>= 1) {
        const uint32_t a = __shfl_xor(kmax, o), b = __shfl_xor(kmin, o);
        kmax = a > kmax ? a : kmax;
        kmin = b < kmin ? b : kmin;
    }
    __syncthreads();
    if ((tid & 63) == 0) {
        hist[tid >> 6] = kmax;
        hist[16 + (tid >> 6)] = kmin;
    }
    __syncthreads();
    const int nw = (int)(blockDim.x >> 6);
    for (int w = 0; w < nw; ++w) {
        kmax = hist[w] > kmax ? hist[w] : kmax;
        kmin = hist[16 + w] < kmin ? hist[16 + w] : kmin;
    }
    const uint32_t diff = kmax ^ kmin;
    if (diff == 0) return kmax;
    int hi = 31 - __clz((int)diff);
    uint32_t mask = hi == 31 ? 0u : ~((2u << hi) - 1u);
    uint32_t prefix = kmax & mask;
#pragma unroll 1
    while (hi >= 0) {
        const int lo = hi >= 7 ? hi - 7 : 0;
        const uint32_t dmask = (1u << (hi - lo + 1)) - 1u;
        __syncthreads();
        for (int i = tid; i < 256; i += blockDim.x) hist[i] = 0;
        __syncthreads();
#pragma unroll
        for (int e = 0; e < PER; ++e)
            if (valid[e] && (key[e] & mask) == prefix) atomicAdd(&hist[(key[e] >> lo) & dmask], 1u);
        __syncthreads();
        if (tid < 64) {
            const uint32_t b0 = hist[4 * tid], b1 = hist[4 * tid + 1], b2 = hist[4 * tid + 2], b3 = hist[4 * tid + 3];
            const uint32_t mine = b0 + b1 + b2 + b3;
            uint32_t inc = mine;
#pragma unroll
            for (int o = 1; o < 64; o <<= 1) {
                const uint32_t t = __shfl_down(inc, o);
                if (tid + o < 64) inc += t;
            }
            const uint32_t above = inc - mine;
            if (above < k && k <= inc) {
                uint32_t a = above;
                int dg;
                if (a + b3 >= k) dg = 3;
                else if ((a += b3) + b2 >= k) dg = 2;
                else if ((a += b2) + b1 >= k) dg = 1;
                else { a += b1; dg = 0; }
                s_pick[0] = (uint32_t)(4 * tid + dg);
                s_pick[1] = k - a;
            }
        }
        __syncthreads();
        prefix |= s_pick[0] << lo;
        mask |= dmask << lo;
        k = s_pick[1];
        hi = lo - 1;
    }
    return prefix;
}

__global__ __launch_bounds__(256) void ingest_kernel(const float *__restrict__ src, uint64_t n, int d,
                                                     float *__restrict__ x, float *__restrict__ scale,
                                                     uint64_t first, int ds, uint32_t *flags, int raw,
                                                     uint32_t *__restrict__ zero_rows, uint32_t *__restrict__ wild_rows,
                                                     uint64_t row_base) {
    const int lane = threadIdx.x & 63;
    const uint64_t wave0 = (uint64_t)blockIdx.x * 4 + (threadIdx.x >> 6);
    const uint64_t nwaves = (uint64_t)gridDim.x * 4;
    for (uint64_t r = wave0; r < n; r += nwaves) {
        const float *s = src + r * (uint64_t)d;
        float *o = x + (first + r) * (uint64_t)ds;
        double acc = 0.0;
        bool bad = false;
        for (int c = lane; c < ds; c += 64) {
            const float v = c < d ? s[c] : 0.0f;
            o[c] = v;
            bad |= !isfinite(v);
            acc += (double)v * (double)v;
        }
#pragma unroll
        for (int off = 32; off > 0; off >>= 1) acc += __shfl_xor(acc, off);
        const bool anybad = __builtin_amdgcn_ballot_w64(bad) != 0;
        if (lane == 0) {
            float sc;
            const bool wild = acc > 0.0 && (acc < 1e-30 || acc > 1e30) && isfinite(acc);
            if (wild) atomicAdd(&flags[1], 1u);
            if (wild && (raw & 2) && !anybad) {
                sc = 0.0f;
                const uint32_t at = atomicAdd(&flags[4], 1u);
                if (at < (uint32_t)kWildCap) wild_rows[at] = (uint32_t)(row_base + r);
            } else if (acc > 0.0) {
                sc = (raw & 1) ? 1.0f : (float)(1.0 / sqrt(acc));
            } else {
                sc = 0.0f;
                if (!anybad && acc == 0.0) {
                    const uint32_t at = atomicAdd(&flags[3], 1u);
                    if (at < (uint32_t)kZeroCap) zero_rows[at] = (uint32_t)(row_base + r);
                }
            }
            if (anybad || !isfinite(acc)) atomicAdd(&flags[0], 1u);
            scale[first + r] = sc;
        }
    }
}

hipError_t launch_ingest(hipStream_t s, const float *src, uint64_t n, int d, float *x, float *scale,
                         uint64_t first, int ds, uint32_t *flags, int raw, uint32_t *zero_rows, uint32_t *wild_rows, uint64_t row_base) {
    if (n == 0) return hipSuccess;
    uint64_t blocks = (n + 3) / 4;
    if (blocks > 8192) blocks = 8192;
    hipLaunchKernelGGL(ingest_kernel, dim3((unsigned)blocks), dim3(256), 0, s, src, n, d, x, scale, first, ds, flags, raw, zero_rows, wild_rows, row_base);
    return hipGetLastError();
}

__global__ __launch_bounds__(256) void prep_queries_kernel(const float *__restrict__ q, int B, int d, int ds,
                                                           __bf16 *__restrict__ qfrag, float *__restrict__ qpad,
                                                           double *__restrict__ qnorm2, float *__restrict__ theta,
                                                           float *__restrict__ e1, const uint32_t *__restrict__ ec_max,
                                                           uint32_t *__restrict__ overflow, uint32_t *__restrict__ flags,
                                                           int filt8, float *__restrict__ qscale,
                                                           float *__restrict__ qa, float *__restrict__ qb,
                                                           const float *__restrict__ mean, float *__restrict__ qmean,
                                                           const uint32_t *__restrict__ rc_max) {
    extern __shared__ __attribute__((aligned(16))) char psm[];
    float *s_row = reinterpret_cast<float *>(psm);
    __shared__ float s_inv;
    __shared__ uint32_t s_red[4];
    __shared__ uint32_t s_bad[4];
    __shared__ double s_dot[4];
    __shared__ float s_rq[4];
    const int b = blockIdx.x;
    const int tid = threadIdx.x;
    const bool live = b < B;
    bool bad = false;
    for (int i = tid; i < d; i += 256) {
        const float v = live ? q[(size_t)b * d + i] : 0.0f;
        s_row[i] = v;
        bad |= !isfinite(v);
    }
    __syncthreads();
    if (tid == 0) {
        double na = 0.0;
        for (int i = 0; i < d; ++i) {
            const float v = s_row[i];
            na += (double)__fmul_rn(v, v);
        }
        qnorm2[b] = na;
        const bool usable = live && na > 0.0 && isfinite(na);
        s_inv = usable ? (float)(1.0 / sqrt(na)) : 0.0f;
        theta[b] = usable ? -INFINITY : INFINITY;
        overflow[b] = 0;
    }
    __syncthreads();
    const float inv = s_inv;
    const int w = b >> 5, col = b & 31;
    float r2 = 0.0f;
    if (filt8) {
        float *rin = s_row + d, *rot = rin + ds, *mixq = rot + ds;
        float aq8 = 0.0f, rq2 = 0.0f;
        if (mean) {
            double dp = 0.0;
            for (int dim = tid; dim < d; dim += 256) dp += (double)(s_row[dim] * inv) * (double)mean[dim];
#pragma unroll
            for (int o = 32; o > 0; o >>= 1) dp += __shfl_xor(dp, o);
            if ((tid & 63) == 0) s_dot[tid >> 6] = dp;
            __syncthreads();
            aq8 = (float)(s_dot[0] + s_dot[1] + s_dot[2] + s_dot[3]);
            if (tid == 0) qmean[b] = aq8;
        }
        for (int dim = tid; dim < ds; dim += 256) {
            float vn = dim < d ? s_row[dim] * inv : 0.0f;
            if (mean && dim < d) vn = __builtin_fmaf(-aq8, mean[dim], vn);
            rin[dim] = vn;
            rq2 += vn * vn;
        }
        if (mean) {
#pragma unroll
            for (int o = 32; o > 0; o >>= 1) rq2 += __shfl_xor(rq2, o);
            if ((tid & 63) == 0) s_rq[tid >> 6] = rq2;
        }
        rot_fill_mix(mixq, ds >> 7, tid, 256);
        __syncthreads();
        if (tid < 64) rot_wave(rin, rot, ds >> 7, tid, mixq);
        __syncthreads();
        float mx = 0.0f;
        for (int dim = tid; dim < ds; dim += 256) mx = fmaxf(mx, fabsf(rot[dim]));
#pragma unroll
        for (int o = 32; o > 0; o >>= 1) mx = fmaxf(mx, __shfl_xor(mx, o));
        if ((tid & 63) == 0) s_red[tid >> 6] = __float_as_uint(mx);
        __syncthreads();
        mx = fmaxf(fmaxf(__uint_as_float(s_red[0]), __uint_as_float(s_red[1])), fmaxf(__uint_as_float(s_red[2]), __uint_as_float(s_red[3])));
        __syncthreads();
        const bool floored = mean && inv > 0.0f;
        const float sq = floored ? fmaxf(mx / 127.0f, kMinStep8) : mx / 127.0f;
        const float qinv = floored ? 1.0f / sq : (mx > 0.0f ? 127.0f / mx : 0.0f);
        if (tid == 0) qscale[b] = sq;
        const int ksteps = ds / 32;
        int8_t *q8 = reinterpret_cast<int8_t *>(qfrag);
        for (int dim = tid; dim < ds; dim += 256) {
            const float v = dim < d ? s_row[dim] : 0.0f;
            qpad[(size_t)b * ds + dim] = v;
            const int ks = dim >> 5, hh = (dim >> 4) & 1, i = dim & 15;
            const int lane = hh * 32 + col;
            const float vn = rot[dim];
            const float qv = fminf(fmaxf(rintf(vn * qinv), -127.0f), 127.0f);
            q8[(((size_t)w * ksteps + ks) * 64 + lane) * 16 + i] = (int8_t)(int)qv;
            const float r = qv * sq - vn;
            r2 += r * r;
        }
    } else {
        float aq = 0.0f;
        if (mean) {
            double dp = 0.0;
            for (int dim = tid; dim < d; dim += 256) dp += (double)(s_row[dim] * inv) * (double)mean[dim];
#pragma unroll
            for (int o = 32; o > 0; o >>= 1) dp += __shfl_xor(dp, o);
            if ((tid & 63) == 0) s_dot[tid >> 6] = dp;
            __syncthreads();
            aq = (float)(s_dot[0] + s_dot[1] + s_dot[2] + s_dot[3]);
            if (tid == 0) qmean[b] = aq;
        }
        const int ksteps = ds / 16;
        float rq2 = 0.0f;
        for (int dim = tid; dim < ds; dim += 256) {
            const float v = dim < d ? s_row[dim] : 0.0f;
            qpad[(size_t)b * ds + dim] = v;
            const int ks = dim >> 4, hh = (dim >> 3) & 1, i = dim & 7;
            const int lane = hh * 32 + col;
            float vn = v * inv;
            if (mean && dim < d) vn = __builtin_fmaf(-aq, mean[dim], vn);
            const __bf16 vb = (__bf16)vn;
            qfrag[(((size_t)w * ksteps + ks) * 64 + lane) * 8 + i] = vb;
            const float r = (float)vb - vn;
            r2 += r * r;
            rq2 += vn * vn;
        }
        if (mean) {
#pragma unroll
            for (int o = 32; o > 0; o >>= 1) rq2 += __shfl_xor(rq2, o);
            if ((tid & 63) == 0) s_rq[tid >> 6] = rq2;
        }
    }
#pragma unroll
    for (int o = 32; o > 0; o >>= 1) r2 += __shfl_xor(r2, o);
    const bool anybad = __builtin_amdgcn_ballot_w64(bad) != 0;
    if ((tid & 63) == 0) {
        s_red[tid >> 6] = __float_as_uint(r2);
        s_bad[tid >> 6] = anybad ? 1u : 0u;
    }
    __syncthreads();
    if (tid == 0) {
        flags[b] = live ? (s_bad[0] | s_bad[1] | s_bad[2] | s_bad[3]) : 0u;
        const float eq = sqrtf(__uint_as_float(s_red[0]) + __uint_as_float(s_red[1]) + __uint_as_float(s_red[2]) +
                               __uint_as_float(s_red[3])) * 1.01f + 1e-6f;
        float e = kApproxErr;
        if (ec_max) {
            const float ec = __uint_as_float(*ec_max) * 1.01f + 1e-6f;
            e = ec + eq + ec * eq + kAccSlack;
            if (!filt8) e = fminf(kApproxErr + ec * ec, e);
            if (mean && !filt8) {
                const float rq = sqrtf(s_rq[0] + s_rq[1] + s_rq[2] + s_rq[3]) * 1.001f + 1e-6f;
                e = fminf(e, rq * ec + eq * 1.0001f + ec * eq + kAccSlack);
            }
        }
        float a8 = eq + kAccSlack, b8 = 1.0f + eq;
        if (mean && filt8) {
            const float rq = sqrtf(s_rq[0] + s_rq[1] + s_rq[2] + s_rq[3]) * 1.001f + 1e-6f;
            const float rc = rc_max ? fminf(__uint_as_float(*rc_max) * 1.001f + 1e-6f, 1.0f + 1e-6f) : 1.0f + 1e-6f;
            a8 = eq * rc * 1.0001f + kAccSlack;
            b8 = rq + eq;
            if (ec_max) e = a8 + b8 * (__uint_as_float(*ec_max) * 1.01f + 1e-6f);
        }
        e1[b] = e;
        qa[b] = filt8 ? a8 : e;
        qb[b] = filt8 ? b8 : 0.0f;
    }
}

hipError_t launch_prep_queries(hipStream_t s, const float *q, int B, int d, int ds, void *qfrag, float *qpad,
                               double *qnorm2, float *theta, float *e1, const uint32_t *ec_max, uint32_t *overflow,
                               uint32_t *flags, float *qa, float *qb, bool filt8, float *qscale, const float *mean, float *qmean,
                               const uint32_t *rc_max) {
    if (!qmean) mean = nullptr;
    hipLaunchKernelGGL(prep_queries_kernel, dim3(B > kPassBatch ? kMaxBatch : kPassBatch), dim3(256),
                       sizeof(float) * ((size_t)d + (filt8 ? 2 * (size_t)ds + kRotMaxBlocks * kRotMaxBlocks : 0)), s, q, B, d, ds,
                       (__bf16 *)qfrag, qpad, qnorm2, theta, e1, ec_max, overflow, flags, filt8 ? 1 : 0, qscale, qa, qb, mean, qmean, rc_max);
    return hipGetLastError();
}

__global__ __launch_bounds__(256) void mean_sum_kernel(const float *__restrict__ x, const float *__restrict__ scale, uint64_t n, int ds,
                                                       float *__restrict__ msum) {
    const uint64_t per = (n + gridDim.x - 1) / gridDim.x;
    const uint64_t r0 = (uint64_t)blockIdx.x * per, r1 = r0 + per < n ? r0 + per : n;
    for (int c = threadIdx.x; c < ds; c += 256) {
        float acc = 0.0f;
        for (uint64_t r = r0; r < r1; ++r) acc = __builtin_fmaf(x[r * (uint64_t)ds + c], scale[r], acc);
        atomicAdd(&msum[c], acc);
    }
}

__global__ __launch_bounds__(256) void mean_norm_kernel(float *__restrict__ msum, int ds, float *__restrict__ mean) {
    __shared__ double s_p[4];
    double p = 0.0;
    for (int c = threadIdx.x; c < ds; c += 256) p += (double)msum[c] * (double)msum[c];
#pragma unroll
    for (int o = 32; o > 0; o >>= 1) p += __shfl_xor(p, o);
    if ((threadIdx.x & 63) == 0) s_p[threadIdx.x >> 6] = p;
    __syncthreads();
    const double n2 = s_p[0] + s_p[1] + s_p[2] + s_p[3];
    const double inv = n2 > 1e-30 && n2 < 1e30 ? 1.0 / sqrt(n2) : 0.0;
    for (int c = threadIdx.x; c < ds; c += 256) mean[c] = (float)((double)msum[c] * inv);
    __syncthreads();
    if (threadIdx.x == 0) msum[ds] = (float)sqrt(n2);
}

hipError_t launch_mean_dir(hipStream_t s, const float *x, const float *scale, uint64_t n, int ds, float *msum, float *mean) {
    hipError_t e = hipMemsetAsync(msum, 0, (size_t)ds * sizeof(float), s);
    if (e != hipSuccess) return e;
    if (n > 0) {
        const unsigned blocks = (unsigned)(n < 2048 ? n : 2048);
        hipLaunchKernelGGL(mean_sum_kernel, dim3(blocks), dim3(256), 0, s, x, scale, n, ds, msum);
    }
    hipLaunchKernelGGL(mean_norm_kernel, dim3(1), dim3(256), 0, s, msum, ds, mean);
    return hipGetLastError();
}

template <int PER>
__global__ __launch_bounds__(256) void theta_kernel(int k, int nwg, const float *__restrict__ lane_max,
                                                    const float *__restrict__ qa, int raw, float *__restrict__ theta) {
    __shared__ uint32_t s_hist[256];
    __shared__ uint32_t s_pick[2];
    __shared__ uint32_t s_nvalid[4];
    const int q = blockIdx.x;
    const int tid = threadIdx.x;
    const int n = 2 * nwg;
    const uint32_t t0 = (uint32_t)(q >> 5) * 64 + (uint32_t)(q & 31);
    uint32_t key[PER];
    bool valid[PER];
#pragma unroll
    for (int e = 0; e < PER; ++e) {
        const int i = e * 256 + tid;
        float v = -INFINITY;
        if (i < n) {
            const int hh = i / nwg, w = i - hh * nwg;
            v = lane_max[(size_t)(t0 + 32 * hh) * nwg + w];
        }
        valid[e] = v > -INFINITY;
        key[e] = f32_key(v);
    }
    uint32_t nv = 0;
#pragma unroll
    for (int e = 0; e < PER; ++e) nv += (uint32_t)__popcll(__builtin_amdgcn_ballot_w64(valid[e]));
    if ((tid & 63) == 0) s_nvalid[tid >> 6] = nv;
    __syncthreads();
    nv = s_nvalid[0] + s_nvalid[1] + s_nvalid[2] + s_nvalid[3];
    float kth = -8.0f;
    if (nv >= (uint32_t)k && k > 0) kth = key_f32(block_kth_largest<PER>(key, valid, (uint32_t)k, s_hist, s_pick));
    if (tid == 0 && theta[q] != INFINITY) theta[q] = kth - (raw ? 2.0f : 1.0f) * qa[q];
}

hipError_t launch_theta(hipStream_t s, int B, int k, int nwg, const float *lane_max, const float *qa, bool raw, float *theta) {
    if (B <= 0) return hipSuccess;
    if (nwg > kMaxScanWGs) return hipErrorInvalidValue;
    if (nwg <= 256)
        hipLaunchKernelGGL(theta_kernel<2>, dim3(B), dim3(256), 0, s, k, nwg, lane_max, qa, raw ? 1 : 0, theta);
    else
        hipLaunchKernelGGL(theta_kernel<4>, dim3(B), dim3(256), 0, s, k, nwg, lane_max, qa, raw ? 1 : 0, theta);
    return hipGetLastError();
}

__global__ void retry_setup_kernel(float *theta, const float *theta_retry, uint32_t *overflow, uint32_t *todo) {
    const int q = threadIdx.x;
    const bool again = overflow[q] == 1;
    todo[q] = again ? 1u : 0u;
    theta[q] = again ? theta_retry[q] : INFINITY;
    if (again) overflow[q] = 0;
}

hipError_t launch_retry_setup(hipStream_t s, float *theta, const float *theta_retry, uint32_t *overflow, uint32_t *todo) {
    hipLaunchKernelGGL(retry_setup_kernel, dim3(1), dim3(kMaxBatch), 0, s, theta, theta_retry, overflow, todo);
    return hipGetLastError();
}

template <bool CMP>
__device__ __forceinline__ float4 row_load4(const float *__restrict__ x, const void *__restrict__ xh, int ds, uint32_t row,
                                            int c4) {
    if (!CMP) return reinterpret_cast<const float4 *>(x + (size_t)row * ds)[c4];
    const uint32_t t = row >> 5, ks = (uint32_t)c4 >> 2, hh = ((uint32_t)c4 >> 1) & 1u, l = (row & 31u) + 32u * hh;
    const uint2 v = reinterpret_cast<const uint2 *>(xh)[(((size_t)t * (uint32_t)(ds >> 4) + ks) * 64 + l) * 2 + (c4 & 1)];
    float4 f;
    f.x = __uint_as_float(v.x << 16);
    f.y = __uint_as_float(v.x & 0xffff0000u);
    f.z = __uint_as_float(v.y << 16);
    f.w = __uint_as_float(v.y & 0xffff0000u);
    f.x = f.x == f.x ? f.x : 0.0f;
    f.y = f.y == f.y ? f.y : 0.0f;
    f.z = f.z == f.z ? f.z : 0.0f;
    f.w = f.w == f.w ? f.w : 0.0f;
    return f;
}

template <bool CMP>
__device__ __forceinline__ float exact_dist_stored(const float *__restrict__ qv, const float *__restrict__ x,
                                                   const void *__restrict__ xh, int ds, uint32_t row, double na) {
    double dot = 0.0, nb = 0.0;
#pragma unroll 8
    for (int i = 0; i < ds / 4; ++i) {
        const float4 c = row_load4<CMP>(x, xh, ds, row, i);
        const float4 a = *reinterpret_cast<const float4 *>(qv + 4 * i);
        dot += (double)__fmul_rn(a.x, c.x); nb += (double)__fmul_rn(c.x, c.x);
        dot += (double)__fmul_rn(a.y, c.y); nb += (double)__fmul_rn(c.y, c.y);
        dot += (double)__fmul_rn(a.z, c.z); nb += (double)__fmul_rn(c.z, c.z);
        dot += (double)__fmul_rn(a.w, c.w); nb += (double)__fmul_rn(c.w, c.w);
    }
    return dist_from_sums(dot, na, nb);
}

__device__ __forceinline__ float exact_dist_row(const float *__restrict__ qv, const float *__restrict__ row, int ds,
                                                double na, double *cos_out) {
    double dot = 0.0, nb = 0.0;
    const float4 *r4 = reinterpret_cast<const float4 *>(row);
#pragma unroll 8
    for (int i = 0; i < ds / 4; ++i) {
        const float4 c = r4[i];
        const float4 a = *reinterpret_cast<const float4 *>(qv + 4 * i);
        dot += (double)__fmul_rn(a.x, c.x); nb += (double)__fmul_rn(c.x, c.x);
        dot += (double)__fmul_rn(a.y, c.y); nb += (double)__fmul_rn(c.y, c.y);
        dot += (double)__fmul_rn(a.z, c.z); nb += (double)__fmul_rn(c.z, c.z);
        dot += (double)__fmul_rn(a.w, c.w); nb += (double)__fmul_rn(c.w, c.w);
    }
    if (cos_out) *cos_out = (na > 0.0 && nb > 0.0) ? dot / sqrt(na * nb) : 1.0;
    return dist_from_sums(dot, na, nb);
}

constexpr int kFinThreads = 1024;
constexpr int kFinishTailBytes = 128 + (2 * kMaxScanWGs + 1 + 3) * 4;
constexpr int kFinWaves = kFinThreads / 64;
constexpr int kFinPer = kCandCap / kFinThreads;
static_assert(kCandCap % kFinThreads == 0, "candidate capacity must divide over the block");

__device__ __forceinline__ uint32_t block_scan_1024(uint32_t v, uint32_t *lds_w, uint32_t *total) {
    const int lane = threadIdx.x & 63, wave = threadIdx.x >> 6;
    uint32_t inc = v;
#pragma unroll
    for (int o = 1; o < 64; o <<= 1) {
        const uint32_t t = __shfl_up(inc, o);
        if (lane >= o) inc += t;
    }
    __syncthreads();
    if (lane == 63) lds_w[wave] = inc;
    __syncthreads();
    uint32_t base = 0, tot = 0;
#pragma unroll
    for (int w = 0; w < kFinWaves; ++w) {
        const uint32_t c = lds_w[w];
        base += w < wave ? c : 0u;
        tot += c;
    }
    *total = tot;
    return base + inc - v;
}

template <bool CMP>
__device__ __forceinline__ void finish_query(const FinishParams &p) {
    extern __shared__ __attribute__((aligned(16))) char fsm[];
    Cand *ent = reinterpret_cast<Cand *>(fsm);
    uint64_t *keys = reinterpret_cast<uint64_t *>(fsm);
    float *qv = reinterpret_cast<float *>(fsm + sizeof(Cand) * (size_t)kCandCap);
    __shared__ uint32_t s_w[kFinWaves];
    __shared__ uint32_t s_sel[2][kFinWaves];
    __shared__ uint32_t s_hist[256];
    __shared__ uint32_t s_pick[2];
    __shared__ uint32_t s_cnt;

    const int q = blockIdx.x;
    const int tid = threadIdx.x;
    const int lane = tid & 63, wave = tid >> 6;
    if (p.todo && !p.todo[q]) return;
    const int k = p.k, ds = p.ds;
    const uint64_t want64 = p.n_live < (uint64_t)k ? p.n_live : (uint64_t)k;
    const int want = (int)want64;
    uint64_t *oid = p.ids + (size_t)q * k;
    float *osc = p.scores + (size_t)q * k;
    float *odi = p.dists ? p.dists + (size_t)q * k : nullptr;
    if (tid == 0) {
        p.n_found[q] = want;
        p.cand_cnt[q] = 0;
    }
    for (int j = tid; j < k; j += kFinThreads) {
        oid[j] = 0;
        osc[j] = 0.0f;
        if (odi) odi[j] = INFINITY;
    }
    if (want == 0) return;
    const double na = p.qnorm2[q];
    if (!(na > 0.0)) {
        if (!p.dead) {
            for (int j = tid; j < want; j += kFinThreads) {
                oid[j] = p.idmap.id_of((uint32_t)j);
                osc[j] = 1.0f;
                if (odi) odi[j] = 0.0f;
            }
        } else {
            uint32_t found = 0;
            for (uint64_t w0 = 0; found < (uint32_t)want && w0 * 64 < p.n_rows; w0 += kFinThreads) {
                const uint64_t w = w0 + (uint64_t)tid;
                uint64_t live = 0;
                if (w * 64 < p.n_rows) {
                    live = ~p.dead[w];
                    const uint64_t rem = p.n_rows - w * 64;
                    if (rem < 64) live &= (1ull << rem) - 1ull;
                }
                uint32_t tot;
                uint32_t j = found + block_scan_1024((uint32_t)__popcll(live), s_w, &tot);
                for (; live && j < (uint32_t)want; ++j) {
                    const uint64_t row = w * 64 + (uint64_t)__builtin_ctzll(live);
                    live &= live - 1;
                    oid[j] = p.idmap.id_of((uint32_t)row);
                    osc[j] = 1.0f;
                    if (odi) odi[j] = 0.0f;
                }
                found += tot;
            }
        }
        return;
    }
    const uint32_t lane_ovf = p.overflow[q];
    const float qa = p.qa[q], qb = p.qb[q];
    auto resid = [&](uint32_t row) { return p.terr ? p.terr[kTscaleFloats * (size_t)(row >> 6) + 2 + ((row >> 5) & 1u)] : 0.0f; };
    for (int i = tid; i < ds; i += kFinThreads) qv[i] = p.qpad[(size_t)q * ds + i];

    const int nwg = p.nwg;
    const float th = p.theta[q];
    const uint32_t nz = p.n_zero;
    const uint32_t nw = p.n_wild;
    auto in_list = [&](const uint32_t *list, uint32_t n, uint32_t row) {
        uint32_t lo = 0, hi = n;
        while (lo < hi) {
            const uint32_t mid = (lo + hi) >> 1;
            if (list[mid] < row) lo = mid + 1;
            else hi = mid;
        }
        return lo < n && list[lo] == row;
    };
    auto is_zero_row = [&](uint32_t row) { return (nz && in_list(p.zero_rows, nz, row)) || (nw && in_list(p.wild_rows, nw, row)); };
    auto is_dead = [&](uint32_t row) { return p.dead && ((p.dead[row >> 6] >> (row & 63u)) & 1ull) != 0; };
    uint32_t *s_off = reinterpret_cast<uint32_t *>(qv + ds) + 32;
    uint32_t nrec = 0;
    if (tid < 2 * nwg) {
        const uint32_t hh0 = (uint32_t)(tid / nwg);
        const int w = tid - (int)hh0 * nwg;
        nrec = p.lane_cnt[(size_t)((uint32_t)(q >> 5) * 64 + (uint32_t)(q & 31) + 32u * hh0) * nwg + w];
        nrec = nrec > (uint32_t)kRecCap ? (uint32_t)kRecCap : nrec;
    }
    uint32_t R;
    const uint32_t roff = block_scan_1024(nrec, s_w, &R);
    if (tid < 2 * nwg) s_off[tid] = roff;
    if (tid == 0) s_off[2 * nwg] = R;
    if (tid == 0) s_cnt = 0;
    __syncthreads();
    auto put = [&](uint32_t at, float sc, uint32_t row) {
        if (at < (uint32_t)kCandCap) {
            Cand cd;
            cd.score = sc;
            cd.row = row;
            ent[at] = cd;
        }
    };
    for (uint32_t j0 = 0; j0 < R; j0 += kFinThreads) {
        const uint32_t j = j0 + tid;
        uint32_t mask = 0, rowb = 0;
        float v[16];
        if (j < R) {
            uint32_t lo = 0, hi = (uint32_t)(2 * nwg) - 1;
            while (lo < hi) {
                const uint32_t mid = (lo + hi + 1) >> 1;
                if (s_off[mid] <= j) lo = mid;
                else hi = mid - 1;
            }
            const uint32_t e = j - s_off[lo], hh = lo / (uint32_t)nwg, w = lo - hh * (uint32_t)nwg;
            const size_t l = (size_t)((uint32_t)(q >> 5) * 64 + (uint32_t)(q & 31) + 32u * hh) * nwg + w;
            const f32x4 *rec = reinterpret_cast<const f32x4 *>(p.lane_rec + l * (kRecCap * 16)) + e * 4;
            const uint32_t t32 = p.lane_tile[l * kRecCap + e];
            rowb = t32 * kTileRows + 4u * hh;
            const uint32_t dm = p.dead ? lane_dead16(dead_half(p.dead, t32), hh) : 0u;
            const f32x4 a = rec[0], b = rec[1], c = rec[2], d = rec[3];
#pragma unroll
            for (int r = 0; r < 4; ++r) v[r] = a[r], v[4 + r] = b[r], v[8 + r] = c[r], v[12 + r] = d[r];
            const float er = resid(rowb);
            const float thr = fmaf(-qb, er, th), eb = fmaf(qb, er, qa);
#pragma unroll
            for (int r = 0; r < 16; ++r) {
                const uint32_t row = rowb + (r & 3) + 8 * (r >> 2);
                const bool pass = v[r] >= thr && (uint64_t)row < p.n_rows && !(v[r] == 0.0f && (nz | nw) && is_zero_row(row)) && !((dm >> r) & 1u);
                mask |= pass ? (1u << r) : 0u;
                v[r] -= eb;
            }
        }
        const uint32_t cnt = (uint32_t)__popc(mask);
        uint32_t inc = cnt;
#pragma unroll
        for (int o = 1; o < 64; o <<= 1) {
            const uint32_t t = __shfl_up(inc, o);
            if (lane >= o) inc += t;
        }
        uint32_t wbase = 0;
        if (lane == 63 && inc) wbase = atomicAdd(&s_cnt, inc);
        wbase = __shfl(wbase, 63);
        uint32_t at = wbase + inc - cnt;
        if (mask) {
#pragma unroll
            for (int r = 0; r < 16; ++r)
                if (mask & (1u << r)) put(at++, v[r], rowb + (r & 3) + 8 * (r >> 2));
        }
    }
    for (uint32_t z = tid; z < nz; z += kFinThreads)
        if ((uint64_t)p.zero_rows[z] < p.n_rows && !is_dead(p.zero_rows[z])) put(atomicAdd(&s_cnt, 1u), 1.0f, p.zero_rows[z]);
    __syncthreads();
    uint32_t M = s_cnt;
    const bool too_many = M > (uint32_t)kCandCap;
    if (too_many) M = kCandCap;
    __syncthreads();
    if (M < (uint32_t)want) {
        if (tid == 0) p.overflow[q] = lane_ovf ? 3u : 2u;
        return;
    }

    uint32_t key[kFinPer], row[kFinPer];
    bool valid[kFinPer];
#pragma unroll
    for (int e = 0; e < kFinPer; ++e) {
        const uint32_t i = (uint32_t)e * kFinThreads + tid;
        valid[e] = i < M;
        if (valid[e]) {
            const Cand cd = ent[i];
            key[e] = f32_key(cd.score);
            row[e] = cd.row;
        } else {
            key[e] = 0;
            row[e] = 0xffffffffu;
        }
    }
    {
        const uint32_t kth = block_kth_largest<kFinPer>(key, valid, (uint32_t)want, s_hist, s_pick);
        const float L1 = key_f32(kth);
        if (tid == 0) s_cnt = 0;
        __syncthreads();
        uint32_t mine = 0;
        float eb[kFinPer];
#pragma unroll
        for (int e = 0; e < kFinPer; ++e) {
            eb[e] = valid[e] ? fmaf(qb, resid(row[e]), qa) : 0.0f;
            valid[e] = valid[e] && key_f32(key[e]) + 2.0f * eb[e] >= L1;
            mine += valid[e] ? 1u : 0u;
        }
        uint32_t at = mine ? atomicAdd(&s_cnt, mine) : 0;
#pragma unroll
        for (int e = 0; e < kFinPer; ++e)
            if (valid[e]) {
                Cand cd;
                cd.score = key_f32(key[e]) + eb[e];
                cd.row = row[e];
                ent[at++] = cd;
            }
        __syncthreads();
    }
    const uint32_t m1 = s_cnt;
    if (tid == 0) p.cand_cnt[q] = m1;

    const float invq = (float)(1.0 / sqrt(na));
    const int nc4 = ds >> 2;
    float err = 0.0f;
    for (uint32_t base = (uint32_t)wave * 4; base < m1; base += kFinWaves * 4) {
        float dot[4];
        float sc[4];
        uint32_t rr[4];
#pragma unroll
        for (int j = 0; j < 4; ++j) {
            const uint32_t i = base + j < m1 ? base + j : base;
            rr[j] = ent[i].row;
            sc[j] = CMP ? 0.0f : p.scale[rr[j]];
            dot[j] = 0.0f;
        }
        for (int tb = 0; tb * 64 < nc4; tb += kMaxKC / 2) {
            float4 x[4][kMaxKC / 2];
#pragma unroll
            for (int t = 0; t < kMaxKC / 2; ++t) {
                const int c4 = lane + 64 * (tb + t);
                if (c4 < nc4) {
#pragma unroll
                    for (int j = 0; j < 4; ++j) x[j][t] = row_load4<CMP>(p.x, p.xh, ds, rr[j], c4);
                }
            }
#pragma unroll
            for (int t = 0; t < kMaxKC / 2; ++t) {
                const int c4 = lane + 64 * (tb + t);
                if (c4 < nc4) {
                    const float4 a = *reinterpret_cast<const float4 *>(qv + 4 * c4);
#pragma unroll
                    for (int j = 0; j < 4; ++j) {
                        const float m = CMP ? 1.0f : sc[j];
                        dot[j] = fmaf(a.x * invq, x[j][t].x * m, dot[j]);
                        dot[j] = fmaf(a.y * invq, x[j][t].y * m, dot[j]);
                        dot[j] = fmaf(a.z * invq, x[j][t].z * m, dot[j]);
                        dot[j] = fmaf(a.w * invq, x[j][t].w * m, dot[j]);
                        if (CMP) sc[j] = fmaf(x[j][t].x, x[j][t].x, fmaf(x[j][t].y, x[j][t].y, fmaf(x[j][t].z, x[j][t].z, fmaf(x[j][t].w, x[j][t].w, sc[j]))));
                    }
                }
            }
        }
#pragma unroll
        for (int j = 0; j < 4; ++j) {
#pragma unroll
            for (int o = 32; o > 0; o >>= 1) {
                dot[j] += __shfl_xor(dot[j], o);
                if (CMP) sc[j] += __shfl_xor(sc[j], o);
            }
        }
        if (lane < 4 && base + lane < m1) {
            const float d0 = lane == 0 ? dot[0] : lane == 1 ? dot[1] : lane == 2 ? dot[2] : dot[3];
            const float s0 = lane == 0 ? sc[0] : lane == 1 ? sc[1] : lane == 2 ? sc[2] : sc[3];
            const bool zero_row = !(s0 > 0.0f);
            const float s2 = zero_row ? 1.0f : (CMP ? d0 * __frsqrt_rn(s0) : d0);
            if (p.max_err && !zero_row) err = fmaxf(err, fabsf(s2 - ent[base + lane].score));
            ent[base + lane].score = s2;
        }
    }
    if (p.max_err) {
#pragma unroll
        for (int o = 32; o > 0; o >>= 1) err = fmaxf(err, __shfl_xor(err, o));
        if (lane == 0 && err > 0.0f) atomicMax(reinterpret_cast<unsigned int *>(p.max_err), __float_as_uint(err));
    }
    __syncthreads();

#pragma unroll
    for (int e = 0; e < kFinPer; ++e) {
        const uint32_t i = (uint32_t)e * kFinThreads + tid;
        valid[e] = i < m1;
        if (valid[e]) {
            const Cand cd = ent[i];
            key[e] = f32_key(cd.score);
            row[e] = cd.row;
        } else {
            key[e] = 0;
            row[e] = 0xffffffffu;
        }
    }
    {
        uint32_t kth;
        if (m1 <= 64u) {
            if (wave == 0) {
                const uint32_t mk = key[0];
                uint32_t gt = 0, ge = 0;
                for (int j = 0; j < 64; ++j) {
                    const uint32_t o = __shfl(mk, j);
                    const bool ov = (uint32_t)j < m1;
                    gt += (ov && o > mk) ? 1u : 0u;
                    ge += (ov && o >= mk) ? 1u : 0u;
                }
                if (valid[0] && gt < (uint32_t)want && (uint32_t)want <= ge) s_pick[0] = mk;
            }
            __syncthreads();
            kth = s_pick[0];
        } else {
            kth = block_kth_largest<kFinPer>(key, valid, (uint32_t)want, s_hist, s_pick);
        }
        const float L = key_f32(kth);
        if (tid == 0) {
            p.theta_retry[q] = L - p.e2 - qa - 1e-6f;
            s_cnt = 0;
        }
        if (lane_ovf || too_many) {
// ... 653 lines not shown
    }
    __syncthreads();
    uint32_t mt = m;
    if (m > 2048u && m > want) {
        uint64_t prefix = 0;
        for (int bit = 63; bit >= 0; --bit) {
            if (bit < 32 && bit >= kSubsetPosBits) continue;
            const uint64_t trial = prefix | (1ull << bit);
            uint32_t cc = 0;
            for (uint32_t i = tid; i < m; i += kFinThreads) cc += keys[i] < trial ? 1u : 0u;
#pragma unroll
            for (int o = 32; o > 0; o >>= 1) cc += __shfl_xor(cc, o);
            uint32_t *slot = s_sel[bit & 1];
            if (lane == 0) slot[wave] = cc;
            __syncthreads();
            cc = 0;
#pragma unroll
            for (int w = 0; w < kFinWaves; ++w) cc += slot[w];
            if (cc < want) prefix = trial;
        }
        uint64_t v[kSubsetPer];
        bool sel[kSubsetPer];
#pragma unroll
        for (int e = 0; e < kSubsetPer; ++e) {
            const uint32_t i = (uint32_t)e * kFinThreads + tid;
            sel[e] = i < m && keys[i] <= prefix;
            v[e] = sel[e] ? keys[i] : 0ull;
        }
        if (tid == 0) s_cnt = 0;
        __syncthreads();
#pragma unroll
        for (int e = 0; e < kSubsetPer; ++e)
            if (sel[e]) keys[atomicAdd(&s_cnt, 1u)] = v[e];
        __syncthreads();
        mt = want;
    }
    for (uint32_t c = tid; c < mt; c += kFinThreads) {
        const uint64_t me = keys[c];
        uint32_t rank = 0;
        for (uint32_t j = 0; j < mt; ++j) rank += keys[j] < me ? 1u : 0u;
        if (rank < want) {
            const float d = __uint_as_float((uint32_t)(me >> 32));
            oid[rank] = idmap.id_of(rows[(uint32_t)me]);
            osc[rank] = score_from_dist(d);
            if (odi) odi[rank] = d;
        }
    }
}

static size_t subset_lds_bytes(int ds) { return sizeof(uint64_t) * (size_t)kSubsetCap + sizeof(float) * (size_t)ds; }

hipError_t subset_setup() {
    const int lds = (int)subset_lds_bytes(kMaxKC16 * kChunkFloats);
    hipError_t e = hipFuncSetAttribute(reinterpret_cast<const void *>(&subset_topk_kernel<false>), hipFuncAttributeMaxDynamicSharedMemorySize, lds);
    if (e != hipSuccess) return e;
    return hipFuncSetAttribute(reinterpret_cast<const void *>(&subset_topk_kernel<true>), hipFuncAttributeMaxDynamicSharedMemorySize, lds);
}

hipError_t launch_subset_topk(hipStream_t s, int B, int k, int ds, const float *x, const void *xh, const uint32_t *rows, uint32_t m,
                              const IdMap &idmap, const float *qpad, const double *qnorm2, uint64_t *ids, float *scores, float *dists,
                              int32_t *n_found) {
    if (B <= 0) return hipSuccess;
    if (m > (uint32_t)kSubsetCap || ds > kMaxKC16 * kChunkFloats) return hipErrorInvalidValue;
    const size_t lds = subset_lds_bytes(ds);
    if (x) hipLaunchKernelGGL(subset_topk_kernel<false>, dim3(B), dim3(kFinThreads), lds, s, k, ds, x, xh, rows, m, idmap, qpad, qnorm2, ids, scores, dists, n_found);
    else hipLaunchKernelGGL(subset_topk_kernel<true>, dim3(B), dim3(kFinThreads), lds, s, k, ds, x, xh, rows, m, idmap, qpad, qnorm2, ids, scores, dists, n_found);
    return hipGetLastError();
}


__global__ void range_theta_kernel(int B, const uint32_t *__restrict__ dlim, float eps, const float *__restrict__ qa,
                                   float *__restrict__ theta) {
    const int q = blockIdx.x * blockDim.x + threadIdx.x;
    if (q >= B || theta[q] == INFINITY) return;
    const uint32_t lim = dlim[q];
    theta[q] = lim == 0 ? INFINITY : 1.0f - __uint_as_float(lim - 1u) - eps - qa[q];
}

hipError_t launch_range_theta(hipStream_t s, int B, const uint32_t *dlim, float eps, const float *qa, float *theta) {
    if (B <= 0) return hipSuccess;
    hipLaunchKernelGGL(range_theta_kernel, dim3((B + 255) / 256), dim3(256), 0, s, B, dlim, eps, qa, theta);
    return hipGetLastError();
}

template <bool CMP>
__device__ __forceinline__ void range_query(const RangeParams &rp) {
    const FinishParams &p = rp.f;
    extern __shared__ __attribute__((aligned(16))) char fsm[];
    Cand *ent = reinterpret_cast<Cand *>(fsm);
    uint64_t *keys = reinterpret_cast<uint64_t *>(fsm);
    float *qv = reinterpret_cast<float *>(fsm + sizeof(Cand) * (size_t)kCandCap);
    __shared__ uint32_t s_w[kFinWaves];
    __shared__ uint32_t s_sel[2][kFinWaves];
    __shared__ uint32_t s_hist[256];
    __shared__ uint32_t s_pick[2];
    __shared__ uint32_t s_cnt;

    const int q = blockIdx.x;
    const int tid = threadIdx.x;
    const int lane = tid & 63, wave = tid >> 6;
    const int cap = p.k, ds = p.ds;
    const uint32_t dlim = rp.dlim[q];
    const float eps = rp.eps;
    uint64_t *oid = p.ids + (size_t)q * cap;
    float *osc = p.scores + (size_t)q * cap;
    float *odi = p.dists ? p.dists + (size_t)q * cap : nullptr;
    if (tid == 0) {
        p.n_found[q] = 0;
        rp.n_in_range[q] = 0;
        p.cand_cnt[q] = 0;
    }
    for (int j = tid; j < cap; j += kFinThreads) {
        oid[j] = 0;
        osc[j] = 0.0f;
        if (odi) odi[j] = INFINITY;
    }
    if (dlim == 0 || p.n_live == 0) return;
    const double na = p.qnorm2[q];
    if (!(na > 0.0)) {
        const uint32_t want = (uint32_t)(p.n_live < (uint64_t)cap ? p.n_live : (uint64_t)cap);
        if (tid == 0) {
            p.n_found[q] = (int32_t)want;
            rp.n_in_range[q] = p.n_live;
        }
        uint32_t found = 0;
        for (uint64_t w0 = 0; found < want && w0 * 64 < p.n_rows; w0 += kFinThreads) {
            const uint64_t w = w0 + (uint64_t)tid;
            uint64_t live = 0;
            if (w * 64 < p.n_rows) {
                live = p.dead ? ~p.dead[w] : ~0ull;
                const uint64_t rem = p.n_rows - w * 64;
                if (rem < 64) live &= (1ull << rem) - 1ull;
            }
            uint32_t tot;
            uint32_t j = found + block_scan_1024((uint32_t)__popcll(live), s_w, &tot);
            for (; live && j < want; ++j) {
                const uint64_t row = w * 64 + (uint64_t)__builtin_ctzll(live);
                live &= live - 1;
                oid[j] = p.idmap.id_of((uint32_t)row);
                osc[j] = 1.0f;
                if (odi) odi[j] = 0.0f;
            }
            found += tot;
        }
        return;
    }
    const float D = __uint_as_float(dlim - 1u);
    const float cin = 1.0f - D + eps, cout = 1.0f - D - eps;
    const uint32_t lane_ovf = p.overflow[q];
    const float qa = p.qa[q], qb = p.qb[q];
    auto resid = [&](uint32_t row) { return p.terr ? p.terr[kTscaleFloats * (size_t)(row >> 6) + 2 + ((row >> 5) & 1u)] : 0.0f; };
    for (int i = tid; i < ds; i += kFinThreads) qv[i] = p.qpad[(size_t)q * ds + i];

    const int nwg = p.nwg;
    const float th = p.theta[q];
    const uint32_t nz = p.n_zero, nw = p.n_wild;
    auto in_list = [&](const uint32_t *list, uint32_t n, uint32_t row) {
        uint32_t lo = 0, hi = n;
        while (lo < hi) {
            const uint32_t mid = (lo + hi) >> 1;
            if (list[mid] < row) lo = mid + 1;
            else hi = mid;
        }
        return lo < n && list[lo] == row;
    };
    auto is_zero_row = [&](uint32_t row) { return (nz && in_list(p.zero_rows, nz, row)) || (nw && in_list(p.wild_rows, nw, row)); };
    auto is_dead = [&](uint32_t row) { return p.dead && ((p.dead[row >> 6] >> (row & 63u)) & 1ull) != 0; };
    uint32_t *s_off = reinterpret_cast<uint32_t *>(qv + ds) + 32;
    uint32_t nrec = 0;
    if (tid < 2 * nwg) {
        const uint32_t hh0 = (uint32_t)(tid / nwg);
        const int w = tid - (int)hh0 * nwg;
        nrec = p.lane_cnt[(size_t)((uint32_t)(q >> 5) * 64 + (uint32_t)(q & 31) + 32u * hh0) * nwg + w];
        nrec = nrec > (uint32_t)kRecCap ? (uint32_t)kRecCap : nrec;
    }
    uint32_t R;
    const uint32_t roff = block_scan_1024(nrec, s_w, &R);
    if (tid < 2 * nwg) s_off[tid] = roff;
    if (tid == 0) s_off[2 * nwg] = R;
    if (tid == 0) s_cnt = 0;
    __syncthreads();
    auto put = [&](uint32_t at, float sc, uint32_t row) {
        if (at < (uint32_t)kCandCap) {
            Cand cd;
            cd.score = sc;
            cd.row = row;
            ent[at] = cd;
        }
    };
    for (uint32_t j0 = 0; j0 < R; j0 += kFinThreads) {
        const uint32_t j = j0 + tid;
        uint32_t mask = 0, rowb = 0;
        float v[16];
        if (j < R) {
            uint32_t lo = 0, hi = (uint32_t)(2 * nwg) - 1;
            while (lo < hi) {
                const uint32_t mid = (lo + hi + 1) >> 1;
                if (s_off[mid] <= j) lo = mid;
                else hi = mid - 1;
            }
            const uint32_t e = j - s_off[lo], hh = lo / (uint32_t)nwg, w = lo - hh * (uint32_t)nwg;
            const size_t l = (size_t)((uint32_t)(q >> 5) * 64 + (uint32_t)(q & 31) + 32u * hh) * nwg + w;
            const f32x4 *rec = reinterpret_cast<const f32x4 *>(p.lane_rec + l * (kRecCap * 16)) + e * 4;
            const uint32_t t32 = p.lane_tile[l * kRecCap + e];
            rowb = t32 * kTileRows + 4u * hh;
            const uint32_t dm = p.dead ? lane_dead16(dead_half(p.dead, t32), hh) : 0u;
            const f32x4 a = rec[0], b = rec[1], c = rec[2], d = rec[3];
#pragma unroll
            for (int r = 0; r < 4; ++r) v[r] = a[r], v[4 + r] = b[r], v[8 + r] = c[r], v[12 + r] = d[r];
            const float er = resid(rowb);
            const float thr = fmaf(-qb, er, th), eb = fmaf(qb, er, qa);
#pragma unroll
            for (int r = 0; r < 16; ++r) {
                const uint32_t row = rowb + (r & 3) + 8 * (r >> 2);
                const bool pass = v[r] >= thr && (uint64_t)row < p.n_rows && !(v[r] == 0.0f && (nz | nw) && is_zero_row(row)) && !((dm >> r) & 1u);
                mask |= pass ? (1u << r) : 0u;
                v[r] -= eb;
            }
        }
        const uint32_t cnt = (uint32_t)__popc(mask);
        uint32_t inc = cnt;
#pragma unroll
        for (int o = 1; o < 64; o <<= 1) {
            const uint32_t t = __shfl_up(inc, o);
            if (lane >= o) inc += t;
        }
        uint32_t wbase = 0;
        if (lane == 63 && inc) wbase = atomicAdd(&s_cnt, inc);
        wbase = __shfl(wbase, 63);
        uint32_t at = wbase + inc - cnt;
        if (mask) {
#pragma unroll
            for (int r = 0; r < 16; ++r)
                if (mask & (1u << r)) put(at++, v[r], rowb + (r & 3) + 8 * (r >> 2));
        }
    }
    for (uint32_t z = tid; z < nz; z += kFinThreads)
        if ((uint64_t)p.zero_rows[z] < p.n_rows && !is_dead(p.zero_rows[z])) put(atomicAdd(&s_cnt, 1u), 1.0f, p.zero_rows[z]);
    __syncthreads();
    const uint32_t M = s_cnt;
    uint32_t nwv = 0;
    for (uint32_t i = 0; i < nw; ++i) nwv += (uint64_t)p.wild_rows[i] < p.n_rows ? 1u : 0u;
    if (lane_ovf || M + nwv > (uint32_t)kCandCap) {
        if (tid == 0) p.overflow[q] = 2;
        return;
    }

    uint32_t row[kFinPer];
    float lb[kFinPer];
    uint32_t st[kFinPer];
    uint32_t mi = 0, mu = 0;
#pragma unroll
    for (int e = 0; e < kFinPer; ++e) {
        const uint32_t i = (uint32_t)e * kFinThreads + tid;
        st[e] = 0;
        row[e] = 0;
        lb[e] = 0.0f;
        if (i < M) {
            const Cand cd = ent[i];
            row[e] = cd.row;
            lb[e] = cd.score;
            st[e] = lb[e] >= cin ? 1u : lb[e] + 2.0f * fmaf(qb, resid(cd.row), qa) < cout ? 0u : 2u;
            mi += st[e] == 1u ? 1u : 0u;
            mu += st[e] == 2u ? 1u : 0u;
        }
    }
    uint32_t nA, nU;
    {
        uint32_t pi = block_scan_1024(mi, s_w, &nA);
        uint32_t pu = block_scan_1024(mu, s_w, &nU);
        pu += nA;
#pragma unroll
        for (int e = 0; e < kFinPer; ++e) {
            if (st[e] == 0u) continue;
            Cand cd;
            cd.score = lb[e];
            cd.row = row[e];
            ent[st[e] == 1u ? pi++ : pu++] = cd;
        }
        __syncthreads();
    }
    if (tid == 0) p.cand_cnt[q] = nU;

    const float invq = (float)(1.0 / sqrt(na));
    const int nc4 = ds >> 2;
    for (uint32_t base = (uint32_t)wave * 4; base < nU; base += kFinWaves * 4) {
        float dot[4];
        float sc[4];
        uint32_t rr[4];
#pragma unroll
        for (int j = 0; j < 4; ++j) {
            const uint32_t i = base + j < nU ? base + j : base;
            rr[j] = ent[nA + i].row;
            sc[j] = CMP ? 0.0f : p.scale[rr[j]];
            dot[j] = 0.0f;
        }
        for (int tb = 0; tb * 64 < nc4; tb += kMaxKC / 2) {
            float4 x[4][kMaxKC / 2];
#pragma unroll
            for (int t = 0; t < kMaxKC / 2; ++t) {
                const int c4 = lane + 64 * (tb + t);
                if (c4 < nc4) {
#pragma unroll
                    for (int j = 0; j < 4; ++j) x[j][t] = row_load4<CMP>(p.x, p.xh, ds, rr[j], c4);
                }
            }
#pragma unroll
            for (int t = 0; t < kMaxKC / 2; ++t) {
                const int c4 = lane + 64 * (tb + t);
                if (c4 < nc4) {
                    const float4 a = *reinterpret_cast<const float4 *>(qv + 4 * c4);
#pragma unroll
                    for (int j = 0; j < 4; ++j) {
                        const float m = CMP ? 1.0f : sc[j];
                        dot[j] = fmaf(a.x * invq, x[j][t].x * m, dot[j]);
                        dot[j] = fmaf(a.y * invq, x[j][t].y * m, dot[j]);
                        dot[j] = fmaf(a.z * invq, x[j][t].z * m, dot[j]);
                        dot[j] = fmaf(a.w * invq, x[j][t].w * m, dot[j]);
                        if (CMP) sc[j] = fmaf(x[j][t].x, x[j][t].x, fmaf(x[j][t].y, x[j][t].y, fmaf(x[j][t].z, x[j][t].z, fmaf(x[j][t].w, x[j][t].w, sc[j]))));
                    }
                }
            }
        }
#pragma unroll
        for (int j = 0; j < 4; ++j) {
#pragma unroll
            for (int o = 32; o > 0; o >>= 1) {
                dot[j] += __shfl_xor(dot[j], o);
                if (CMP) sc[j] += __shfl_xor(sc[j], o);
            }
        }
        if (lane < 4 && base + lane < nU) {
            const float d0 = lane == 0 ? dot[0] : lane == 1 ? dot[1] : lane == 2 ? dot[2] : dot[3];
            const float s0 = lane == 0 ? sc[0] : lane == 1 ? sc[1] : lane == 2 ? sc[2] : sc[3];
            const bool zero_row = !(s0 > 0.0f);
            ent[nA + base + lane].score = zero_row ? 1.0f : (CMP ? d0 * __frsqrt_rn(s0) : d0);
        }
    }
    __syncthreads();
    uint32_t nB, n2;
    {
        mi = mu = 0;
#pragma unroll
        for (int e = 0; e < kFinPer; ++e) {
            const uint32_t i = (uint32_t)e * kFinThreads + tid;
            st[e] = 0;
            if (i < nU) {
                const Cand cd = ent[nA + i];
                row[e] = cd.row;
                lb[e] = cd.score;
                st[e] = cd.score - p.e2 >= cin ? 1u : cd.score + p.e2 < cout ? 0u : 2u;
                mi += st[e] == 1u ? 1u : 0u;
                mu += st[e] == 2u ? 1u : 0u;
            }
        }
        uint32_t pi = block_scan_1024(mi, s_w, &nB);
        uint32_t pu = block_scan_1024(mu, s_w, &n2);
        pi += nA;
        pu += nA + nB;
#pragma unroll
        for (int e = 0; e < kFinPer; ++e) {
            if (st[e] == 0u) continue;
            Cand cd;
            cd.score = lb[e];
            cd.row = row[e];
            ent[st[e] == 1u ? pi++ : pu++] = cd;
        }
        __syncthreads();
    }

    const uint32_t c0 = nA + nB, nC = n2 + nwv;
    for (uint32_t i = tid; i < nC; i += kFinThreads) {
        const uint32_t r = i < n2 ? ent[c0 + i].row : p.wild_rows[i - n2];
        const float d = exact_dist_stored<CMP>(qv, p.x, p.xh, ds, r, na);
        Cand cd;
        cd.score = (i >= n2 && is_dead(r)) || __float_as_uint(d) >= dlim ? -1.0f : d;
        cd.row = r;
        ent[c0 + i] = cd;
    }
    __syncthreads();

    const uint32_t T = c0 + nC;
    uint32_t stm = 0, mine = 0;
#pragma unroll
    for (int e = 0; e < kFinPer; ++e) {
        const uint32_t i = (uint32_t)e * kFinThreads + tid;
        lb[e] = 0.0f;
        row[e] = 0;
        if (i < T) {
            const Cand cd = ent[i];
            row[e] = cd.row;
            uint32_t s = 0;
            if (i < nA) lb[e] = cd.score, s = 1;
// ... 438 lines not shown
```

Before: 235,500.

## Add a separate sift kernel to gather filter candidates across many blocks per query

Moves candidate gathering from lane record buffers out of the single-block-per-query finish kernel into a new sift kernel that uses a 2D grid of blocks per query and appends passing candidates to a global per-query list via atomics. The finish and range-finish kernels then load that precomputed list instead of scanning records themselves. This spreads the threshold test over many more workgroups to remove a serial per-query bottleneck, at the cost of an extra launch, a global candidate buffer per lane pool, and counter resets in prep and retry. It is enabled by default and can be switched off with an environment variable.

```diff
diff --git a/memex_amd/csrc/index.hip b/memex_amd/csrc/index.hip
--- a/memex_amd/csrc/index.hip
+++ b/memex_amd/csrc/index.hip
@@ -55,6 +55,8 @@
     uint32_t *lane_tile = nullptr;
     uint32_t *lane_cnt = nullptr;
     float *lane_max = nullptr;
+    Cand *sift_list = nullptr;
+    uint32_t *sift_cnt = nullptr;
     float *qstage = nullptr;
     float *qscale = nullptr;
     float *qa = nullptr, *qb = nullptr;
@@ -81,6 +83,7 @@
     float *rec = nullptr;
     uint32_t *tile = nullptr, *cnt = nullptr;
     float *max = nullptr;
+    Cand *cand = nullptr;
     int nwg = 0;
     int groups = 1;
 };
@@ -97,6 +100,7 @@
     if (b.tile) (void)hipFree(b.tile);
     if (b.cnt) (void)hipFree(b.cnt);
     if (b.max) (void)hipFree(b.max);
+    if (b.cand) (void)hipFree(b.cand);
     b = LaneBufs{};
 }
 
@@ -173,6 +177,7 @@
     int mode = MX_SEARCH_AUTO;
     bool profiling = false;
     int n_cu = 0, nwg = 0;
+    bool sift = true;
     bool scan8_pair = true;
     Scratch s;
     mx_index_stats stats{};
@@ -320,7 +325,7 @@
     F(idx->byid_rows); F(idx->byid_stage); F(idx->byid_q); F(idx->byid_ids); F(idx->byid_nr); F(idx->byid_own); F(idx->byid_scores);
     F(idx->byid_dists); F(idx->byid_nf); F(idx->byid_src); F(idx->byid_dlim);
     Scratch &s = idx->s;
-    F(s.qfrag); F(s.qpad); F(s.qnorm2); F(s.theta); F(s.theta_retry); F(s.todo); F(s.dev_flags); F(s.done_ctr);
+    F(s.qfrag); F(s.qpad); F(s.qnorm2); F(s.theta); F(s.theta_retry); F(s.todo); F(s.dev_flags); F(s.done_ctr); F(s.sift_cnt);
     if (s.host_flags) (void)hipHostFree(s.host_flags);
     if (s.host_sum) (void)hipHostFree(s.host_sum);
     for (void *hp : {(void *)s.h_q, (void *)s.h_ids, (void *)s.h_scores, (void *)s.h_dists, (void *)s.h_nf, (void *)s.h_nr})
@@ -369,6 +374,7 @@
             if (e == hipSuccess) e = hipMalloc(reinterpret_cast<void **>(&b.tile), lanes * kRecCap * sizeof(uint32_t));
             if (e == hipSuccess) e = hipMalloc(reinterpret_cast<void **>(&b.cnt), lanes * sizeof(uint32_t));
             if (e == hipSuccess) e = hipMalloc(reinterpret_cast<void **>(&b.max), lanes * sizeof(float));
+            if (e == hipSuccess) e = hipMalloc(reinterpret_cast<void **>(&b.cand), (size_t)(groups > 1 ? kMaxBatch : kPassBatch) * kCandCap * sizeof(Cand));
             if (e != hipSuccess) {
                 lane_free(b);
                 idx = nullptr;
@@ -380,6 +386,7 @@
         s.lane_tile = b.tile;
         s.lane_cnt = b.cnt;
         s.lane_max = b.max;
+        s.sift_list = b.cand;
         return MX_OK;
     }
     void drop() {
@@ -389,6 +396,7 @@
         s.lane_tile = nullptr;
         s.lane_cnt = nullptr;
         s.lane_max = nullptr;
+        s.sift_list = nullptr;
         LanePool &lp = g_lanes[idx->device];
         std::lock_guard<std::mutex> lk(lp.mu);
         if (lp.open_indexes > 0) lp.idle.push_back(b);
@@ -418,6 +426,7 @@
     MX_HIP(hipHostMalloc(reinterpret_cast<void **>(&s.host_flags), kFlagWords * sizeof(uint32_t), hipHostMallocDefault));
     MX_HIP(hipHostMalloc(reinterpret_cast<void **>(&s.host_sum), kSumWords * sizeof(uint32_t), hipHostMallocMapped | hipHostMallocCoherent));
     memset(s.host_sum, 0, kSumWords * sizeof(uint32_t));
+    MX_HIP(hipMalloc(&s.sift_cnt, kMaxBatch * sizeof(uint32_t)));
     MX_HIP(hipMalloc(&s.done_ctr, sizeof(uint32_t)));
     MX_HIP(hipMemsetAsync(s.done_ctr, 0, sizeof(uint32_t), idx->stream));
     MX_HIP(hipMalloc(&s.qstage, (size_t)kMaxBatch * idx->dim * sizeof(float)));
@@ -1021,7 +1030,7 @@
     Scratch &s = idx->s;
     MX_HIP(launch_prep_queries(idx->stream, d_q, B, idx->dim, idx->ds, s.qfrag, s.qpad, s.qnorm2, s.theta, s.e1,
                                idx->xh ? idx->flags + 2 : nullptr, s.overflow, s.qflags, s.qa, s.qb, pl.filt8, s.qscale,
-                               pl.centred ? idx->mean : nullptr, s.qmean, pl.centred8 ? idx->flags + 5 : nullptr));
+                               pl.centred ? idx->mean : nullptr, s.qmean, pl.centred8 ? idx->flags + 5 : nullptr, s.sift_cnt));
     return MX_OK;
 }
 
@@ -1087,6 +1096,8 @@
     fp.todo = nullptr;
     fp.theta_retry = s.theta_retry;
     fp.cand_cnt = s.cand_cnt;
+    fp.sift_list = idx->sift ? s.sift_list : nullptr;
+    fp.sift_cnt = s.sift_cnt;
     fp.ids = d_ids;
     fp.scores = d_scores;
     fp.dists = d_dists;
@@ -1201,6 +1212,7 @@
     fp.max_err = idx->profiling ? s.max_err : nullptr;
     auto finish_and_wait = [&]() -> int {
         fp.seq = ++s.flag_seq;
+        MX_HIP(launch_sift(st, B, fp));
         MX_HIP(launch_finish(st, B, fp));
         return await_finish(idx, B, fp.seq);
     };
@@ -1278,7 +1290,7 @@
                 p.wave_mask = 0;
                 for (int b = 0; b < B; ++b)
                     if (h_ovf[b] == 1) p.wave_mask |= 1u << (b >> 5);
-                MX_HIP(launch_retry_setup(st, s.theta, s.theta_retry, s.overflow, s.todo));
+                MX_HIP(launch_retry_setup(st, s.theta, s.theta_retry, s.overflow, s.todo, s.sift_cnt));
                 if ((rc = collect(false)) != MX_OK) return rc;
                 fp.todo = s.todo;
                 if ((rc = finish_and_wait()) != MX_OK) return rc;
@@ -1392,6 +1404,7 @@
         rp.dlim = s.rlim;
         rp.eps = kRangeEps;
         rp.n_in_range = d_nrange;
+        MX_HIP(launch_sift(st, B, fp));
         MX_HIP(launch_range_finish(st, B, rp));
         if ((rc = await_finish(idx, B, fp.seq)) != MX_OK) return rc;
         if (s.host_sum[2]) return fail(MX_EINVAL, "a query contains non-finite values");
@@ -2405,6 +2418,10 @@
         const char *pv = getenv("MEMEX_HIP_SCAN8_PAIR");
         idx->scan8_pair = !(pv && pv[0] == '0');
     }
+    {
+        const char *sv = getenv("MEMEX_HIP_SIFT");
+        idx->sift = !(sv && sv[0] == '0');
+    }
     MX_HIP(hipStreamCreateWithFlags(&idx->stream, hipStreamNonBlocking));
     MX_HIP(hipEventCreate(&idx->ev0));
     MX_HIP(hipEventCreate(&idx->ev1));
@@ -2632,6 +2649,7 @@
         sh->mode = old->mode;
         sh->profiling = old->profiling;
         sh->scan8_pair = old->scan8_pair;
+        sh->sift = old->sift;
         sh->want_filter = old->want_filter;
         sh->filter_i8 = old->filter_i8;
         sh->filter_auto = old->filter_auto;
diff --git a/memex_amd/csrc/index_kernels.h b/memex_amd/csrc/index_kernels.h
--- a/memex_amd/csrc/index_kernels.h
+++ b/memex_amd/csrc/index_kernels.h
@@ -125,7 +125,7 @@
                                float *qpad, double *qnorm2, float *theta, float *e1, const uint32_t *ec_max,
                                uint32_t *overflow, uint32_t *flags, float *qa, float *qb, bool filt8 = false,
                                float *qscale = nullptr, const float *mean = nullptr, float *qmean = nullptr,
-                               const uint32_t *rc_max = nullptr);
+                               const uint32_t *rc_max = nullptr, uint32_t *sift_cnt = nullptr);
 
 hipError_t launch_theta(hipStream_t s, int B, int k, int nwg, const float *lane_max, const float *qa, bool raw, float *theta);
 
@@ -156,6 +156,8 @@
     const uint32_t *todo;
     float *theta_retry;
     uint32_t *cand_cnt;
+    Cand *sift_list;
+    uint32_t *sift_cnt;
     uint64_t *ids;
     float *scores, *dists;
     int32_t *n_found;
@@ -168,8 +170,10 @@
     uint32_t seq;
 };
 hipError_t finish_setup();
+hipError_t launch_sift(hipStream_t s, int B, const FinishParams &p);
 hipError_t launch_finish(hipStream_t s, int B, const FinishParams &p);
-hipError_t launch_retry_setup(hipStream_t s, float *theta, const float *theta_retry, uint32_t *overflow, uint32_t *todo);
+hipError_t launch_retry_setup(hipStream_t s, float *theta, const float *theta_retry, uint32_t *overflow, uint32_t *todo,
+                              uint32_t *sift_cnt = nullptr);
 
 hipError_t launch_range_theta(hipStream_t s, int B, const uint32_t *dlim, float eps, const float *qa, float *theta);
 struct RangeParams {
diff --git a/memex_amd/csrc/index_kernels.hip b/memex_amd/csrc/index_kernels.hip
--- a/memex_amd/csrc/index_kernels.hip
+++ b/memex_amd/csrc/index_kernels.hip
@@ -175,7 +175,7 @@
                                                            int filt8, float *__restrict__ qscale,
                                                            float *__restrict__ qa, float *__restrict__ qb,
                                                            const float *__restrict__ mean, float *__restrict__ qmean,
-                                                           const uint32_t *__restrict__ rc_max) {
+                                                           const uint32_t *__restrict__ rc_max, uint32_t *__restrict__ sift_cnt) {
     extern __shared__ __attribute__((aligned(16))) char psm[];
     float *s_row = reinterpret_cast<float *>(psm);
     __shared__ float s_inv;
@@ -204,6 +204,7 @@
         s_inv = usable ? (float)(1.0 / sqrt(na)) : 0.0f;
         theta[b] = usable ? -INFINITY : INFINITY;
         overflow[b] = 0;
+        if (sift_cnt) sift_cnt[b] = 0;
     }
     __syncthreads();
     const float inv = s_inv;
@@ -334,11 +335,11 @@
 hipError_t launch_prep_queries(hipStream_t s, const float *q, int B, int d, int ds, void *qfrag, float *qpad,
                                double *qnorm2, float *theta, float *e1, const uint32_t *ec_max, uint32_t *overflow,
                                uint32_t *flags, float *qa, float *qb, bool filt8, float *qscale, const float *mean, float *qmean,
-                               const uint32_t *rc_max) {
+                               const uint32_t *rc_max, uint32_t *sift_cnt) {
     if (!qmean) mean = nullptr;
     hipLaunchKernelGGL(prep_queries_kernel, dim3(B > kPassBatch ? kMaxBatch : kPassBatch), dim3(256),
                        sizeof(float) * ((size_t)d + (filt8 ? 2 * (size_t)ds + kRotMaxBlocks * kRotMaxBlocks : 0)), s, q, B, d, ds,
-                       (__bf16 *)qfrag, qpad, qnorm2, theta, e1, ec_max, overflow, flags, filt8 ? 1 : 0, qscale, qa, qb, mean, qmean, rc_max);
+                       (__bf16 *)qfrag, qpad, qnorm2, theta, e1, ec_max, overflow, flags, filt8 ? 1 : 0, qscale, qa, qb, mean, qmean, rc_max, sift_cnt);
     return hipGetLastError();
 }
 
@@ -423,16 +424,18 @@
     return hipGetLastError();
 }
 
-__global__ void retry_setup_kernel(float *theta, const float *theta_retry, uint32_t *overflow, uint32_t *todo) {
+__global__ void retry_setup_kernel(float *theta, const float *theta_retry, uint32_t *overflow, uint32_t *todo, uint32_t *sift_cnt) {
     const int q = threadIdx.x;
     const bool again = overflow[q] == 1;
     todo[q] = again ? 1u : 0u;
+    if (sift_cnt) sift_cnt[q] = 0;
     theta[q] = again ? theta_retry[q] : INFINITY;
     if (again) overflow[q] = 0;
 }
 
-hipError_t launch_retry_setup(hipStream_t s, float *theta, const float *theta_retry, uint32_t *overflow, uint32_t *todo) {
-    hipLaunchKernelGGL(retry_setup_kernel, dim3(1), dim3(kMaxBatch), 0, s, theta, theta_retry, overflow, todo);
+hipError_t launch_retry_setup(hipStream_t s, float *theta, const float *theta_retry, uint32_t *overflow, uint32_t *todo,
+                              uint32_t *sift_cnt) {
+    hipLaunchKernelGGL(retry_setup_kernel, dim3(1), dim3(kMaxBatch), 0, s, theta, theta_retry, overflow, todo, sift_cnt);
     return hipGetLastError();
 }
 
@@ -513,6 +516,193 @@
     }
     *total = tot;
     return base + inc - v;
+}
+
+__device__ __forceinline__ size_t lane_buffer_of(int q, uint32_t hh, uint32_t w, int nwg) {
+    return (size_t)((uint32_t)(q >> 5) * 64 + (uint32_t)(q & 31) + 32u * hh) * nwg + w;
+}
+
+__device__ __forceinline__ bool in_ascending_list(const uint32_t *list, uint32_t n, uint32_t row) {
+    uint32_t lo = 0, hi = n;
+    while (lo < hi) {
+        const uint32_t mid = (lo + hi) >> 1;
+        if (list[mid] < row) lo = mid + 1;
+        else hi = mid;
+    }
+    return lo < n && list[lo] == row;
+}
+
+__device__ __forceinline__ uint32_t record_test(const FinishParams &p, float th, float qa, float qb, size_t l, uint32_t e, uint32_t hh,
+                                                float (&v)[16], uint32_t &rowb) {
+    const uint32_t nz = p.n_zero, nw = p.n_wild;
+    const f32x4 *rec = reinterpret_cast<const f32x4 *>(p.lane_rec + l * (kRecCap * 16)) + e * 4;
+    const uint32_t t32 = p.lane_tile[l * kRecCap + e];
+    rowb = t32 * kTileRows + 4u * hh;
+    const uint32_t dm = p.dead ? lane_dead16(dead_half(p.dead, t32), hh) : 0u;
+    const f32x4 a = rec[0], b = rec[1], c = rec[2], d = rec[3];
+#pragma unroll
+    for (int r = 0; r < 4; ++r) v[r] = a[r], v[4 + r] = b[r], v[8 + r] = c[r], v[12 + r] = d[r];
+    const float er = p.terr ? p.terr[kTscaleFloats * (size_t)(rowb >> 6) + 2 + ((rowb >> 5) & 1u)] : 0.0f;
+    const float thr = fmaf(-qb, er, th), eb = fmaf(qb, er, qa);
+    uint32_t mask = 0;
+#pragma unroll
+    for (int r = 0; r < 16; ++r) {
+        const uint32_t row = rowb + (r & 3) + 8 * (r >> 2);
+        const bool listed = v[r] == 0.0f && (nz | nw) &&
+                            ((nz && in_ascending_list(p.zero_rows, nz, row)) || (nw && in_ascending_list(p.wild_rows, nw, row)));
+        const bool pass = v[r] >= thr && (uint64_t)row < p.n_rows && !listed && !((dm >> r) & 1u);
+        mask |= pass ? (1u << r) : 0u;
+        v[r] -= eb;
+    }
+    return mask;
+}
+
+__device__ __forceinline__ void append_passing(uint32_t mask, const float (&v)[16], uint32_t rowb, uint32_t *ctr, Cand *ent) {
+    const int lane = threadIdx.x & 63;
+    const uint32_t cnt = (uint32_t)__popc(mask);
+    uint32_t inc = cnt;
+#pragma unroll
+    for (int o = 1; o < 64; o <<= 1) {
+        const uint32_t t = __shfl_up(inc, o);
+        if (lane >= o) inc += t;
+    }
+    uint32_t wbase = 0;
+    if (lane == 63 && inc) wbase = atomicAdd(ctr, inc);
+    wbase = __shfl(wbase, 63);
+    uint32_t at = wbase + inc - cnt;
+    if (mask) {
+#pragma unroll
+        for (int r = 0; r < 16; ++r)
+            if (mask & (1u << r)) {
+                if (at < (uint32_t)kCandCap) {
+                    Cand cd;
+                    cd.score = v[r];
+                    cd.row = rowb + (r & 3) + 8 * (r >> 2);
+                    ent[at] = cd;
+                }
+                ++at;
+            }
+    }
+}
+
+__device__ __forceinline__ void append_zero_rows(const FinishParams &p, uint32_t t, uint32_t threads, uint32_t *ctr, Cand *ent) {
+    for (uint32_t z = t; z < p.n_zero; z += threads) {
+        const uint32_t row = p.zero_rows[z];
+        if ((uint64_t)row < p.n_rows && !(p.dead && ((p.dead[row >> 6] >> (row & 63u)) & 1ull) != 0)) {
+            const uint32_t at = atomicAdd(ctr, 1u);
+            if (at < (uint32_t)kCandCap) {
+                Cand cd;
+                cd.score = 1.0f;
+                cd.row = row;
+                ent[at] = cd;
+            }
+        }
+    }
+}
+
+__device__ __forceinline__ uint32_t gather_query(const FinishParams &p, int q, Cand *ent, uint32_t *s_off, uint32_t *s_w, uint32_t *s_cnt) {
+    const int tid = threadIdx.x;
+    const int nwg = p.nwg;
+    const float th = p.theta[q], qa = p.qa[q], qb = p.qb[q];
+    uint32_t nrec = 0;
+    if (tid < 2 * nwg) {
+        const uint32_t hh0 = (uint32_t)(tid / nwg);
+        nrec = p.lane_cnt[lane_buffer_of(q, hh0, (uint32_t)(tid - (int)hh0 * nwg), nwg)];
+        nrec = nrec > (uint32_t)kRecCap ? (uint32_t)kRecCap : nrec;
+    }
+    uint32_t R;
+    const uint32_t roff = block_scan_1024(nrec, s_w, &R);
+    if (tid < 2 * nwg) s_off[tid] = roff;
+    if (tid == 0) s_off[2 * nwg] = R;
+    if (tid == 0) *s_cnt = 0;
+    __syncthreads();
+    for (uint32_t j0 = 0; j0 < R; j0 += kFinThreads) {
+        const uint32_t j = j0 + tid;
+        uint32_t mask = 0, rowb = 0;
+        float v[16];
+        if (j < R) {
+            uint32_t lo = 0, hi = (uint32_t)(2 * nwg) - 1;
+            while (lo < hi) {
+                const uint32_t mid = (lo + hi + 1) >> 1;
+                if (s_off[mid] <= j) lo = mid;
+                else hi = mid - 1;
+            }
+            const uint32_t hh = lo / (uint32_t)nwg;
+            mask = record_test(p, th, qa, qb, lane_buffer_of(q, hh, lo - hh * (uint32_t)nwg, nwg), j - s_off[lo], hh, v, rowb);
+        }
+        append_passing(mask, v, rowb, s_cnt, ent);
+    }
+    append_zero_rows(p, (uint32_t)tid, kFinThreads, s_cnt, ent);
+    __syncthreads();
+    return *s_cnt;
+}
+
+__device__ __forceinline__ uint32_t load_sifted(const FinishParams &p, int q, Cand *ent) {
+    const uint32_t M = p.sift_cnt[q];
+    const uint32_t n = M < (uint32_t)kCandCap ? M : (uint32_t)kCandCap;
+    const Cand *src = p.sift_list + (size_t)q * kCandCap;
+    for (uint32_t i = threadIdx.x; i < n; i += kFinThreads) ent[i] = src[i];
+    __syncthreads();
+    return M;
+}
+
+constexpr int kSiftThreads = 256;
+constexpr int kSiftLanes = 128;
+static_assert(kSiftLanes == 128 && kSiftThreads >= kSiftLanes, "the count scan below is written for two waves");
+
+__global__ __launch_bounds__(kSiftThreads) void sift_kernel(const FinishParams p) {
+    __shared__ uint32_t s_off[kSiftLanes];
+    __shared__ uint32_t s_wsum[2];
+    const int q = blockIdx.y;
+    const int tid = threadIdx.x, lane = tid & 63;
+    if (p.todo && !p.todo[q]) return;
+    if (!(p.qnorm2[q] > 0.0)) return;
+    const int nwg = p.nwg;
+    const float th = p.theta[q], qa = p.qa[q], qb = p.qb[q];
+    uint32_t *ctr = p.sift_cnt + q;
+    Cand *list = p.sift_list + (size_t)q * kCandCap;
+    const uint32_t i = blockIdx.x * (uint32_t)kSiftLanes + (uint32_t)tid;
+    uint32_t nrec = 0;
+    if (tid < kSiftLanes && i < 2u * (uint32_t)nwg) {
+        const uint32_t hh0 = i / (uint32_t)nwg;
+        nrec = p.lane_cnt[lane_buffer_of(q, hh0, i - hh0 * (uint32_t)nwg, nwg)];
+        nrec = nrec > (uint32_t)kRecCap ? (uint32_t)kRecCap : nrec;
+    }
+    uint32_t inc = nrec;
+#pragma unroll
+    for (int o = 1; o < 64; o <<= 1) {
+        const uint32_t t = __shfl_up(inc, o);
+        if (lane >= o) inc += t;
+    }
+    if (tid < kSiftLanes && lane == 63) s_wsum[tid >> 6] = inc;
+    __syncthreads();
+    if (tid < kSiftLanes) s_off[tid] = inc - nrec + (tid >= 64 ? s_wsum[0] : 0u);
+    const uint32_t R = s_wsum[0] + s_wsum[1];
+    __syncthreads();
+    for (uint32_t j0 = 0; j0 < R; j0 += kSiftThreads) {
+        const uint32_t j = j0 + tid;
+        uint32_t mask = 0, rowb = 0;
+        float v[16];
+        if (j < R) {
+            uint32_t lo = 0, hi = (uint32_t)kSiftLanes - 1;
+            while (lo < hi) {
+                const uint32_t mid = (lo + hi + 1) >> 1;
+                if (s_off[mid] <= j) lo = mid;
+                else hi = mid - 1;
+            }
+            const uint32_t ib = blockIdx.x * (uint32_t)kSiftLanes + lo, hh = ib / (uint32_t)nwg;
+            mask = record_test(p, th, qa, qb, lane_buffer_of(q, hh, ib - hh * (uint32_t)nwg, nwg), j - s_off[lo], hh, v, rowb);
+        }
+        append_passing(mask, v, rowb, ctr, list);
+    }
+    if (blockIdx.x == 0) append_zero_rows(p, (uint32_t)tid, kSiftThreads, ctr, list);
+}
+
+hipError_t launch_sift(hipStream_t s, int B, const FinishParams &p) {
+    if (B <= 0 || !p.sift_list) return hipSuccess;
+    if (p.nwg <= 0 || p.nwg > kMaxScanWGs || !p.sift_cnt) return hipErrorInvalidValue;
+    hipLaunchKernelGGL(sift_kernel, dim3((2 * p.nwg + kSiftLanes - 1) / kSiftLanes, B), dim3(kSiftThreads), 0, s, p);
+    return hipGetLastError();
 }
 
 template <bool CMP>
@@ -584,94 +774,9 @@
     auto resid = [&](uint32_t row) { return p.terr ? p.terr[kTscaleFloats * (size_t)(row >> 6) + 2 + ((row >> 5) & 1u)] : 0.0f; };
     for (int i = tid; i < ds; i += kFinThreads) qv[i] = p.qpad[(size_t)q * ds + i];
 
-    const int nwg = p.nwg;
-    const float th = p.theta[q];
-    const uint32_t nz = p.n_zero;
     const uint32_t nw = p.n_wild;
-    auto in_list = [&](const uint32_t *list, uint32_t n, uint32_t row) {
-        uint32_t lo = 0, hi = n;
-        while (lo < hi) {
-            const uint32_t mid = (lo + hi) >> 1;
-            if (list[mid] < row) lo = mid + 1;
-            else hi = mid;
-        }
-        return lo < n && list[lo] == row;
-    };
-    auto is_zero_row = [&](uint32_t row) { return (nz && in_list(p.zero_rows, nz, row)) || (nw && in_list(p.wild_rows, nw, row)); };
     auto is_dead = [&](uint32_t row) { return p.dead && ((p.dead[row >> 6] >> (row & 63u)) & 1ull) != 0; };
-    uint32_t *s_off = reinterpret_cast<uint32_t *>(qv + ds) + 32;
-    uint32_t nrec = 0;
-    if (tid < 2 * nwg) {
-        const uint32_t hh0 = (uint32_t)(tid / nwg);
-        const int w = tid - (int)hh0 * nwg;
-        nrec = p.lane_cnt[(size_t)((uint32_t)(q >> 5) * 64 + (uint32_t)(q & 31) + 32u * hh0) * nwg + w];
-        nrec = nrec > (uint32_t)kRecCap ? (uint32_t)kRecCap : nrec;
-    }
-    uint32_t R;
-    const uint32_t roff = block_scan_1024(nrec, s_w, &R);
-    if (tid < 2 * nwg) s_off[tid] = roff;
-    if (tid == 0) s_off[2 * nwg] = R;
-    if (tid == 0) s_cnt = 0;
-    __syncthreads();
-    auto put = [&](uint32_t at, float sc, uint32_t row) {
-        if (at < (uint32_t)kCandCap) {
-            Cand cd;
-            cd.score = sc;
-            cd.row = row;
-            ent[at] = cd;
-        }
-    };
-    for (uint32_t j0 = 0; j0 < R; j0 += kFinThreads) {
-        const uint32_t j = j0 + tid;
-        uint32_t mask = 0, rowb = 0;
-        float v[16];
-        if (j < R) {
-            uint32_t lo = 0, hi = (uint32_t)(2 * nwg) - 1;
-            while (lo < hi) {
-                const uint32_t mid = (lo + hi + 1) >> 1;
-                if (s_off[mid] <= j) lo = mid;
-                else hi = mid - 1;
-            }
-            const uint32_t e = j - s_off[lo], hh = lo / (uint32_t)nwg, w = lo - hh * (uint32_t)nwg;
-            const size_t l = (size_t)((uint32_t)(q >> 5) * 64 + (uint32_t)(q & 31) + 32u * hh) * nwg + w;
-            const f32x4 *rec = reinterpret_cast<const f32x4 *>(p.lane_rec + l * (kRecCap * 16)) + e * 4;
-            const uint32_t t32 = p.lane_tile[l * kRecCap + e];
-            rowb = t32 * kTileRows + 4u * hh;
-            const uint32_t dm = p.dead ? lane_dead16(dead_half(p.dead, t32), hh) : 0u;
-            const f32x4 a = rec[0], b = rec[1], c = rec[2], d = rec[3];
-#pragma unroll
-            for (int r = 0; r < 4; ++r) v[r] = a[r], v[4 + r] = b[r], v[8 + r] = c[r], v[12 + r] = d[r];
-            const float er = resid(rowb);
-            const float thr = fmaf(-qb, er, th), eb = fmaf(qb, er, qa);
-#pragma unroll
-            for (int r = 0; r < 16; ++r) {
-                const uint32_t row = rowb + (r & 3) + 8 * (r >> 2);
-                const bool pass = v[r] >= thr && (uint64_t)row < p.n_rows && !(v[r] == 0.0f && (nz | nw) && is_zero_row(row)) && !((dm >> r) & 1u);
-                mask |= pass ? (1u << r) : 0u;
-                v[r] -= eb;
-            }
-        }
-        const uint32_t cnt = (uint32_t)__popc(mask);
-        uint32_t inc = cnt;
-#pragma unroll
-        for (int o = 1; o < 64; o <<= 1) {
-            const uint32_t t = __shfl_up(inc, o);
-            if (lane >= o) inc += t;
-        }
-        uint32_t wbase = 0;
-        if (lane == 63 && inc) wbase = atomicAdd(&s_cnt, inc);
-        wbase = __shfl(wbase, 63);
-        uint32_t at = wbase + inc - cnt;
-        if (mask) {
-#pragma unroll
-            for (int r = 0; r < 16; ++r)
-                if (mask & (1u << r)) put(at++, v[r], rowb + (r & 3) + 8 * (r >> 2));
-        }
-    }
-    for (uint32_t z = tid; z < nz; z += kFinThreads)
-        if ((uint64_t)p.zero_rows[z] < p.n_rows && !is_dead(p.zero_rows[z])) put(atomicAdd(&s_cnt, 1u), 1.0f, p.zero_rows[z]);
-    __syncthreads();
-    uint32_t M = s_cnt;
+    uint32_t M = p.sift_list ? load_sifted(p, q, ent) : gather_query(p, q, ent, reinterpret_cast<uint32_t *>(qv + ds) + 32, s_w, &s_cnt);
     const bool too_many = M > (uint32_t)kCandCap;
     if (too_many) M = kCandCap;
     __syncthreads();
@@ -1631,93 +1736,9 @@
     auto resid = [&](uint32_t row) { return p.terr ? p.terr[kTscaleFloats * (size_t)(row >> 6) + 2 + ((row >> 5) & 1u)] : 0.0f; };
     for (int i = tid; i < ds; i += kFinThreads) qv[i] = p.qpad[(size_t)q * ds + i];
 
-    const int nwg = p.nwg;
-    const float th = p.theta[q];
-    const uint32_t nz = p.n_zero, nw = p.n_wild;
-    auto in_list = [&](const uint32_t *list, uint32_t n, uint32_t row) {
-        uint32_t lo = 0, hi = n;
-        while (lo < hi) {
-            const uint32_t mid = (lo + hi) >> 1;
-            if (list[mid] < row) lo = mid + 1;
-            else hi = mid;
-        }
-        return lo < n && list[lo] == row;
-    };
-    auto is_zero_row = [&](uint32_t row) { return (nz && in_list(p.zero_rows, nz, row)) || (nw && in_list(p.wild_rows, nw, row)); };
+    const uint32_t nw = p.n_wild;
     auto is_dead = [&](uint32_t row) { return p.dead && ((p.dead[row >> 6] >> (row & 63u)) & 1ull) != 0; };
-    uint32_t *s_off = reinterpret_cast<uint32_t *>(qv + ds) + 32;
-    uint32_t nrec = 0;
-    if (tid < 2 * nwg) {
-        const uint32_t hh0 = (uint32_t)(tid / nwg);
-        const int w = tid - (int)hh0 * nwg;
-        nrec = p.lane_cnt[(size_t)((uint32_t)(q >> 5) * 64 + (uint32_t)(q & 31) + 32u * hh0) * nwg + w];
-        nrec = nrec > (uint32_t)kRecCap ? (uint32_t)kRecCap : nrec;
-    }
-    uint32_t R;
-    const uint32_t roff = block_scan_1024(nrec, s_w, &R);
-    if (tid < 2 * nwg) s_off[tid] = roff;
-    if (tid == 0) s_off[2 * nwg] = R;
-    if (tid == 0) s_cnt = 0;
-    __syncthreads();
-    auto put = [&](uint32_t at, float sc, uint32_t row) {
-        if (at < (uint32_t)kCandCap) {
-            Cand cd;
-            cd.score = sc;
-            cd.row = row;
-            ent[at] = cd;
-        }
-    };
-    for (uint32_t j0 = 0; j0 < R; j0 += kFinThreads) {
-        const uint32_t j = j0 + tid;
-        uint32_t mask = 0, rowb = 0;
-        float v[16];
-        if (j < R) {
-            uint32_t lo = 0, hi = (uint32_t)(2 * nwg) - 1;
-            while (lo < hi) {
-                const uint32_t mid = (lo + hi + 1) >> 1;
-                if (s_off[mid] <= j) lo = mid;
-                else hi = mid - 1;
-            }
-            const uint32_t e = j - s_off[lo], hh = lo / (uint32_t)nwg, w = lo - hh * (uint32_t)nwg;
-            const size_t l = (size_t)((uint32_t)(q >> 5) * 64 + (uint32_t)(q & 31) + 32u * hh) * nwg + w;
-            const f32x4 *rec = reinterpret_cast<const f32x4 *>(p.lane_rec + l * (kRecCap * 16)) + e * 4;
-            const uint32_t t32 = p.lane_tile[l * kRecCap + e];
-            rowb = t32 * kTileRows + 4u * hh;
-            const uint32_t dm = p.dead ? lane_dead16(dead_half(p.dead, t32), hh) : 0u;
-            const f32x4 a = rec[0], b = rec[1], c = rec[2], d = rec[3];
-#pragma unroll
-            for (int r = 0; r < 4; ++r) v[r] = a[r], v[4 + r] = b[r], v[8 + r] = c[r], v[12 + r] = d[r];
-            const float er = resid(rowb);
-            const float thr = fmaf(-qb, er, th), eb = fmaf(qb, er, qa);
-#pragma unroll
-            for (int r = 0; r < 16; ++r) {
-                const uint32_t row = rowb + (r & 3) + 8 * (r >> 2);
-                const bool pass = v[r] >= thr && (uint64_t)row < p.n_rows && !(v[r] == 0.0f && (nz | nw) && is_zero_row(row)) && !((dm >> r) & 1u);
-                mask |= pass ? (1u << r) : 0u;
-                v[r] -= eb;
-            }
-        }
-        const uint32_t cnt = (uint32_t)__popc(mask);
-        uint32_t inc = cnt;
-#pragma unroll
-        for (int o = 1; o < 64; o <<= 1) {
-            const uint32_t t = __shfl_up(inc, o);
-            if (lane >= o) inc += t;
-        }
-        uint32_t wbase = 0;
-        if (lane == 63 && inc) wbase = atomicAdd(&s_cnt, inc);
-        wbase = __shfl(wbase, 63);
-        uint32_t at = wbase + inc - cnt;
-        if (mask) {
-#pragma unroll
-            for (int r = 0; r < 16; ++r)
-                if (mask & (1u << r)) put(at++, v[r], rowb + (r & 3) + 8 * (r >> 2));
-        }
-    }
-    for (uint32_t z = tid; z < nz; z += kFinThreads)
-        if ((uint64_t)p.zero_rows[z] < p.n_rows && !is_dead(p.zero_rows[z])) put(atomicAdd(&s_cnt, 1u), 1.0f, p.zero_rows[z]);
-    __syncthreads();
-    const uint32_t M = s_cnt;
+    const uint32_t M = p.sift_list ? load_sifted(p, q, ent) : gather_query(p, q, ent, reinterpret_cast<uint32_t *>(qv + ds) + 32, s_w, &s_cnt);
     uint32_t nwv = 0;
     for (uint32_t i = 0; i < nw; ++i) nwv += (uint64_t)p.wild_rows[i] < p.n_rows ? 1u : 0u;
     if (lane_ovf || M + nwv > (uint32_t)kCandCap) {
```

After: 233,500. About the same (-0.8%).
